# jhuldr/BrainFM

Measured on AMD Instinct MI355X. Metric: voxels/sec whole-volume multi-task inference, 256^3 tiled, higher is better.
Workload: dtype f16x3-split (fp32-grade); 1 GPU; 256^3 volume, reference tiling win160/stride80 -> 27 tiles, UNet3D f64 x6 levels, 9 heads (69 ch), fused tail + deformed atlas + on-device stitch of 17 keys; stitched_keys=17, mfma_passes=3, submission=hipGraph replay per tile shape, parallelism=tiles sharded over 1 rank(s), gather to rank 0, tiles_in_flight_per_gpu=2

## Files before the change

brainfm_amd/_lib.py:

```python
import ctypes as C
import os

_HERE = os.path.dirname(os.path.abspath(__file__))
LIB_PATH = os.path.join(_HERE, "libbrainfm_hip.so")

ERR = {0: "BFM_OK", -1: "BFM_E_ARG", -2: "BFM_E_SHAPE", -3: "BFM_E_WORKSPACE", -4: "BFM_E_LAUNCH"}

ROLE_PLAIN, ROLE_CT, ROLE_BIAS_LOG, ROLE_SEG, ROLE_DIST, ROLE_SR, ROLE_PATHOL = range(7)
(EW_EXP, EW_AFFINE, EW_CLAMP, EW_CLAMP_MIN, EW_GAMMA, EW_SIGMOID, EW_DIV, EW_NONZERO, EW_SUB_DIV, EW_GE,
 EW_NAN_TO_NUM) = range(11)
(EW_ADD, EW_MUL, EW_MUL_EXP, EW_AXPY_CLAMP0, EW_AXPY, EW_DIV2, EW_ZERO_WHERE_ZERO) = range(7)


class BfmError(RuntimeError):
    pass


class Upsample(C.Structure):
    _fields_ = [("d", C.c_int), ("h", C.c_int), ("w", C.c_int),
                ("mapD", C.c_void_p), ("mapH", C.c_void_p), ("mapW", C.c_void_p),
                ("repD", C.c_void_p), ("repH", C.c_void_p), ("repW", C.c_void_p)]


CLASS_STATS_BLOCKS = 1024


class TailDesc(C.Structure):
    _fields_ = [("n_out", C.c_int), ("c_feat", C.c_int),
                ("head_w", C.c_void_p), ("head_b", C.c_void_p), ("roles", C.c_void_p), ("out_slot", C.c_void_p),
                ("seg_first", C.c_int), ("n_seg", C.c_int), ("seg_lut", C.c_void_p),
                ("n_dist", C.c_int), ("dist_first", C.c_int), ("max_dist", C.c_float),
                ("unit_feat", C.c_int), ("slot_high_res", C.c_int), ("slot_fake_cortical", C.c_int),
                ("n_maps", C.c_int), ("head_wmax", C.c_float), ("skip_zero_input", C.c_int)]


class ZoomAxis(C.Structure):
    _fields_ = [("f", C.c_void_p), ("c", C.c_void_p), ("wf", C.c_void_p), ("wc", C.c_void_p)]


class KSet(C.Structure):
    _fields_ = [("k", C.c_void_p * 7), ("coef", C.c_float * 7), ("nk", C.c_int)]


class Dopri5Advect(C.Structure):
    _fields_ = [("y", C.c_void_p * 2), ("f", C.c_void_p * 2), ("k", C.c_void_p * 5),
                ("Vx", C.c_void_p), ("Vy", C.c_void_p), ("Vz", C.c_void_p),
                ("sx", C.c_int), ("sy", C.c_int), ("sz", C.c_int), ("neumann_bc", C.c_int), ("is_f64", C.c_int),
                ("atol", C.c_double), ("rtol", C.c_double), ("tol_min_dt", C.c_double), ("dt_max", C.c_double),
                ("safety", C.c_double), ("ifactor", C.c_double), ("dfactor", C.c_double),
                ("t_out", C.c_void_p), ("nt", C.c_int), ("sol", C.c_void_p), ("state", C.c_void_p),
                ("workspace", C.c_void_p)]


class AgeParams(C.Structure):
    _fields_ = [(n, C.c_void_p) for n in ("c1w", "c1b", "c2w", "c2b", "l1w", "l1b", "l2w", "l2b", "l3w", "l3b")]


class AgeGrads(C.Structure):
    _fields_ = [(n, C.c_void_p) for n in ("c1w", "c1b", "c2w", "c2b", "l1w", "l1b", "l2w", "l2b", "l3w", "l3b")]


GATHER_MAX_JOBS = 12


VERTEX_SETS_MAX = 4


class VertexSet(C.Structure):
    _fields_ = [("V", C.c_void_p), ("n", C.c_int64)]


class GatherJob(C.Structure):
    _fields_ = [("src", C.c_void_p), ("out", C.c_void_p), ("mean", C.c_float), ("scale", C.c_float), ("pre", C.c_int),
                ("default_max", C.c_int), ("post_div", C.c_float), ("clamp", C.c_int), ("clamp_lo", C.c_float),
                ("clamp_hi", C.c_float), ("sign", C.c_float), ("want_minmax", C.c_int)]


_P = C.c_void_p
_I = C.c_int
_F = C.c_float
_L = C.c_int64
_Z = C.c_size_t
_UP = C.POINTER(Upsample)

SIGNATURES = {
    "bfm_version": (C.c_char_p, []),
    "bfm_gn_stats_workspace": (_Z, [_I, _I, _I, _I, _I, _UP]),
    "bfm_gn_stats": (_I, [_P, _I, _P, _I, _I, _I, _I, _UP, _P, _P, _I, _F, _P, _P, _P, _P, _Z, _P]),
    "bfm_pack_conv_weights_direct": (_I, [_P, _I, _I, _P, _P]),
    "bfm_pack_conv_weights_mfma_bytes": (_Z, [_I, _I]),
    "bfm_pack_conv_weights_mfma": (_I, [_P, _I, _I, _F, _P, C.POINTER(_I), _P]),
    "bfm_pack_conv_weights_mfma16_bytes": (_Z, [_I, _I]),
    "bfm_pack_conv_weights_mfma16": (_I, [_P, _I, _I, _F, _P, C.POINTER(_I), _P]),
    "bfm_conv3x3x3_direct": (_I, [_P, _I, _P, _I, _I, _I, _I, _UP, _P, _P, _P, _I, _F, _P, _P]),
    "bfm_pack_conv_weights_upfold_bytes": (C.c_size_t, [_I, _I, _I]),
    "bfm_pack_conv_weights_upfold": (_I, [_P, _I, _I, _I, _F, _I, _P, _P, _P]),
    "bfm_conv3x3x3_upfold": (_I, [_P, _I, _I, _I, _I, _P, _P, _P, _I, _P, _I, _I, _I, _P, _P]),
    "bfm_conv3x3x3_upfold_workspace": (_Z, [_I, _I, _I, _I, _I]),
    "bfm_conv3x3x3_upfold_ex": (_I, [_P, _I, _I, _I, _I, _P, _P, _P, _I, _P, _I, _I, _I, _P, _P, _Z, _P]),
    "bfm_conv3x3x3_upfold_batch_workspace": (_Z, [_I, _I, _I, _I, _I, _I]),
    "bfm_conv3x3x3_upfold_batch": (_I, [_P, _I, _I, _I, _I, _I, _P, _P, _P, _I, _P, _I, _I, _I, _P, _P, _Z, _I, _P]),
    "bfm_conv3x3x3_tap_batch_workspace": (_Z, [_I, _I, _I, _I]),
    "bfm_conv3x3x3_tap_batch": (_I, [_P, _I, _I, _I, _P, _P, _P, _I, _P, _I, _I, _I, _I, _I, _P, _Z, _I, _P]),
    "bfm_tap_sum_rows": (_I, [_I, _I]),
    "bfm_tap_sum_batch": (_I, [_P, _I, _I, _I, _I, _P, _I, _F, _I, _I, _P, _P, _P]),
    "bfm_moment_rows_bytes": (_Z, [_I, _I]),
    "bfm_conv3x3x3_mfma_rows": (_I, [_I, _I, _I, _I, _I, C.POINTER(_I)]),
    "bfm_conv3x3x3_mfma_ex": (_I, [_P, _I, _P, _I, _I, _I, _I, _UP, _P, _P, _P, _I, _P, _I, _I, _F, _I,
                                   C.POINTER(_I), _P, _P, _Z, _P, _P]),
    "bfm_conv3x3x3_mfma_batch_workspace": (_Z, [_I, _I, _I, _I, _I, _I, _I]),
    "bfm_conv3x3x3_mfma_batch": (_I, [_P, _I, _P, _I, _I, _I, _I, _I, _UP, _P, _P, _P, _I, _P, _I, _I, _F, _I,
                                      C.POINTER(_I), _P, _P, _Z, _P, _I, _P]),
    "bfm_gn_stats_batch_workspace": (_Z, [_I, _I, _I, _I, _I, _I, _UP]),
    "bfm_gn_stats_batch": (_I, [_P, _I, _P, _I, _I, _I, _I, _I, _UP, _P, _P, _I, _F, _P, _P, _P, _P, _Z, _P]),
    "bfm_gn_stats_rows_batch": (_I, [_P, _I, _I, _P, _I, _I, C.c_double, _L, _I, _P, _P, _I, _F, _P, _P, _P, _P]),
    "bfm_conv3x3x3_stem_rows": (_I, [_I, _I, _I]),
    "bfm_conv3x3x3_stem_ex": (_I, [_P, _I, _I, _I, _P, _P, _P, _P, _I, _F, _P, _P, _P]),
    "bfm_conv3x3x3_stem_mc_ex": (_I, [_P, _I, _I, _I, _I, _P, _P, _P, _P, _I, _F, _P, _P, _P]),
    "bfm_gn_stats_rows_workspace": (_Z, [_I, _I, _I, _I]),
    "bfm_gn_stats_rows": (_I, [_P, _I, _I, _P, _I, _I, C.c_double, _L, _P, _P, _I, _F, _P, _P, _P, _P, _Z, _P, _P]),
    "bfm_gn_stats_rows_sliced": (_I, [_P, _I, _I, _I, _I, _P, _I, _I, _I, _I, C.c_double, _L, _P, _P, _I, _F, _P, _P, _P, _P, _Z,
                                      _P, _P]),
    "bfm_gn_stats_rows_train": (_I, [_P, _I, _I, _P, _I, _I, C.c_double, _L, _P, _P, _I, _F, _P, _P, _P, _P, _P, _P, _Z, _P, _P]),
    "bfm_crop3d": (_I, [_P, _I, _I, _I, _I, _I, _I, _I, _I, _I, _P, _P]),
    "bfm_pack_conv_weights_wino4_bytes": (_Z, [_I, _I, _I]),
    "bfm_pack_conv_weights_wino4": (_I, [_P, _I, _I, _F, _I, _P, C.POINTER(_I), _P]),
    "bfm_conv3x3x3_wino4_rows": (_I, [_I, _I, _I, _I]),
    "bfm_conv3x3x3_wino4_box": (_I, [_I, _I, _I, _I, _P]),
    "bfm_conv3x3x3_wino4_masked_workspace": (_Z, [_I, _I, _I, _I]),
    "bfm_conv3x3x3_wino4_uniform_scratch": (_Z, [_I]),
    "bfm_conv3x3x3_wino4_uniform": (_I, [_P, _I, _I, _I, _I, _P, _P, _P, _I, _P, _I, _I, _F, _I, _I, _P, _P, _P, _P, _P]),
    "bfm_conv3x3x3_wino4": (_I, [_P, _I, _I, _I, _I, _P, _P, _P, _I, _P, _I, _I, _F, _I, _I, _P, _P, _P]),
    "bfm_conv3x3x3_wino4_batch": (_I, [_P, _I, _I, _I, _I, _I, _P, _P, _P, _I, _P, _I, _I, _F, _I, _I, _P, _P, _I, _P]),
    "bfm_conv3x3x3_wino4_masked": (_I, [_P, _I, _I, _I, _I, _P, _P, _P, _I, _P, _I, _I, _F, _I, _I, _P, _P, _P, _Z, _P]),
    "bfm_permute_flip3d": (_I, [_P, _I, _I, _I, C.POINTER(_I), C.POINTER(_I), _P, _P]),
    "bfm_bbox_nonzero": (_I, [_P, _I, _I, _I, _F, _P, _P]),
    "bfm_mean_lastdim": (_I, [_P, _L, _I, _P, _P]),
    "bfm_pack_conv_weights_wino_bytes": (_Z, [_I, _I, _I]),
    "bfm_pack_conv_weights_wino": (_I, [_P, _I, _I, _F, _I, _P, C.POINTER(_I), _P]),
    "bfm_bspline3_prefilter_axis": (_I, [_P, _I, _I, _I, _I, _I, _F, _F, _P, _F, _F, _F, _P]),
    "bfm_bspline3_resample_axis": (_I, [_P, _I, _I, _I, _I, _P, _I, _I, _P, _P]),
    "bfm_conv3x3x3_wino_rows": (_I, [_I, _I, _I, _I]),
    "bfm_conv3x3x3_wino_ex": (_I, [_P, _I, _I, _I, _I, _P, _P, _P, _I, _P, _I, _I, _F, _I, _I, _P, _P, _P]),
    "bfm_conv3x3x3_wino_box": (_I, [_I, _I, _I, _I, _P]),
    "bfm_uniform_boxes": (_I, [_P, _I, _I, _I, _I, _I, _P, _P]),
    "bfm_uniform_boxes_level": (_I, [_P, _I, _I, _I, _I, _I, _I, _P, _P]),
    "bfm_uniform_boxes_levels": (_I, [_P, _I, _I, _I, _I, C.POINTER(_I), C.POINTER(_I), _I, C.POINTER(_P), _P, _P]),
    "bfm_uniform_boxes_bytes": (_Z, [_I, _I, _I, _I]),
    "bfm_conv3x3x3_wino_uniform_scratch": (_Z, [_I]),
    "bfm_conv3x3x3_wino_uniform": (_I, [_P, _I, _I, _I, _I, _P, _P, _P, _I, _P, _I, _I, _F, _I, _I, _P, _P, _P, _P, _P]),
    "bfm_conv3x3x3_wino_pool_ok": (_I, [_I, _I, _I, _I]),
    "bfm_conv3x3x3_wino_pool": (_I, [_P, _I, _I, _I, _I, _P, _P, _P, _I, _P, _I, _I, _F, _I, _I, _P, _P, _P, _P, _P]),
    "bfm_conv3x3x3_wino_uniform_pool": (_I, [_P, _I, _I, _I, _I, _P, _P, _P, _I, _P, _I, _I, _F, _I, _I, _P, _P, _P, _P, _P, _P,
                                             _P]),
    "bfm_conv3x3x3_wino_masked_workspace": (_Z, [_I, _I, _I, _I]),
    "bfm_conv3x3x3_wino_masked": (_I, [_P, _I, _I, _I, _I, _P, _P, _P, _I, _P, _I, _I, _F, _I, _I, _P, _P, _P, _Z, _P]),
    "bfm_maxpool2_rows": (_I, [_I, _I, _I, _I]),
    "bfm_maxpool2_ex": (_I, [_P, _I, _I, _I, _I, _P, _P, _P]),
    "bfm_maxpool2_batch_rows": (_I, [_I, _I, _I, _I]),
    "bfm_maxpool2_batch": (_I, [_P, _I, _I, _I, _I, _I, _P, _P, _P]),
    "bfm_grid_push3d_linear": (_I, [_P, _I, _I, _I, _I, _I, _P, _I, _I, _I, _I, C.POINTER(_I), _I, _P, _P]),
    "bfm_grid_grad3d_linear": (_I, [_P, _I, _I, _I, _I, _I, _P, _I, _I, _I, _I, C.POINTER(_I), _I, _P, _P]),
    "bfm_gn_stats_train": (_I, [_P, _I, _P, _I, _I, _I, _I, _UP, _P, _P, _I, _F, _P, _P, _P, _P, _P, _P, _Z, _P]),
    "bfm_lrelu_bwd": (_I, [_P, _P, _L, _F, _P, _P]),
    "bfm_lrelu_bwd_ex": (_I, [_P, _P, _L, _F, _P, _P, _P]),
    "bfm_conv3x3x3_wgrad_workspace": (_Z, [_I, _I, _I, _I, _I]),
    "bfm_conv3x3x3_wgrad": (_I, [_P, _I, _P, _I, _P, _I, _I, _I, _I, _UP, _P, _P, _P, _P, _Z, _P]),
    "bfm_conv3x3x3_wgrad_ex": (_I, [_P, _I, _P, _I, _P, _I, _I, _I, _I, _UP, _P, _P, _P, _P, _I, _I, _P, _P, _Z, _P]),
    "bfm_stem_mc_bwd_workspace": (_Z, [_I, _I, _I, _I, _I]),
    "bfm_stem_mc_bwd": (_I, [_P, _I, _P, _I, _I, _I, _I, _P, _P, _P, _P, _P, _P, _P, _P, _P, _Z, _P]),
    "bfm_stem_mc_dgrad": (_I, [_P, _I, _P, _I, _I, _I, _I, _P, _P, _P, _P, _P, _P, _I, _P, _P, _P, _P, _L, _L, _P]),
    "bfm_mask_chain_bwd": (_I, [_P, _L, _P, _P, _L, _P, _L, _L, _P]),
    "bfm_gn_bwd_workspace": (_Z, [_I, _I, _I, _I]),
    "bfm_gn_bwd": (_I, [_P, _P, _I, _P, _I, _I, _I, _I, _UP, _P, _P, _P, _P, _P, _P, _I, _P, _P, _P, _P, _P, _Z, _P]),
    "bfm_maxpool2_bwd": (_I, [_P, _P, _I, _I, _I, _I, _P, _P]),
    "bfm_transpose_mirror_weights": (_I, [_P, _I, _I, _I, _P, _P]),
    "bfm_loss_workspace": (_Z, [_I]),
    "bfm_loss_l1": (_I, [_P, _I, _I, _P, _P, _P, _L, _F, _I, _F, _P, _P, _P, _Z, _P]),
    "bfm_loss_l1_multi_workspace": (_Z, []),
    "bfm_loss_l1_multi": (_I, [_P, _I, _L, _I, _P, _P, _P, _P, _P, _P, _P, _P, _P, _P, _Z, _P]),
    "bfm_loss_grad_l1_multi": (_I, [_P, _I, _I, _P, _P, _P, _P, _I, _I, _I, _P, _P, _P, _Z, _P]),
    "bfm_loss_grad_l1": (_I, [_P, _I, _I, _P, _P, _I, _I, _I, _F, _P, _P, _P, _Z, _P]),
    "bfm_loss_seg": (_I, [_P, _I, _I, _I, _P, _P, _P, _L, _F, _F, _P, _P, _P, _P, _Z, _P]),
    "bfm_loss_pathol_workspace": (_Z, []),
    "bfm_loss_pathol": (_I, [_P, _L, _L, _P, _L, _F, _F, _P, _P, _P, _P, _Z, _P]),
    "bfm_loss_reg_workspace": (_Z, [_I, _I, _I, _I]),
    "bfm_loss_reg_smooth": (_I, [_P, _L, _L, _L, _I, _I, _I, _I, _F, _P, _P, _P, _Z, _P]),
    "bfm_loss_reg_hessian": (_I, [_P, _L, _L, _L, _I, _I, _I, _I, _F, _P, _P, _P, _Z, _P]),
    "bfm_loss_contrastive_workspace": (_Z, []),
    "bfm_loss_contrastive": (_I, [_P, _P, _I, _L, _I, _F, _F, _F, _F, _F, _P, _P, _P, _P, _P, _P, _Z, _P]),
    "bfm_head_bwd_workspace": (_Z, [_I, _I, _L]),
    "bfm_head_bwd": (_I, [_P, _P, _P, _I, _I, _L, _P, _P, _P, _P, _Z, _P]),
    "bfm_tail_raw_rows": (_I, [_P, _L, C.POINTER(TailDesc), _P, _P, _L, _P]),
    "bfm_loss_l1_multi_rows": (_I, [_P, _L, _I, _L, _I, _P, _P, _P, _P, _P, _P, _P, _P, _P, _P, _Z, _P]),
    "bfm_loss_grad_l1_multi_rows": (_I, [_P, _L, _I, _I, _P, _P, _P, _P, _I, _I, _I, _P, _P, _P, _Z, _P]),
    "bfm_loss_seg_rows": (_I, [_P, _L, _I, _I, _I, _P, _P, _P, _L, _F, _F, _P, _P, _P, _P, _Z, _P]),
    "bfm_head_bwd_rows": (_I, [_P, _L, _P, _P, _I, _I, _L, _P, _P, _P, _P, _Z, _P]),
    "bfm_normalize_bwd": (_I, [_P, _P, _I, _L, _F, _P, _P]),
    "bfm_adamw_step": (_I, [_P, _P, _P, _P, _L, _F, _F, _F, _F, _F, _I, _F, _P]),
    "bfm_grad_sumsq": (_I, [_P, _L, _P, _P, _P, _Z, _P]),
    "bfm_grad_sumsq_multi": (_I, [_P, _I, _P, _I, _L, _P, _P, _P, _Z, _P]),
    "bfm_adamw_step_multi": (_I, [_P, _I, _P, _I, _L, _F, _F, _F, _F, _F, _P]),
    "bfm_conv3x3x3_mfma_workspace": (_Z, [_I, _I, _I, _I, _I, _I]),
    "bfm_conv3x3x3_mfma_plan": (_I, [_I, _I, _I, _I, _I, C.POINTER(_I)]),
    "bfm_conv3x3x3_mfma": (_I, [_P, _I, _P, _I, _I, _I, _I, _UP, _P, _P, _P, _I, _P, _I, _I, _F, _I,
                                C.POINTER(_I), _P, _P, _Z, _P]),
    "bfm_maxpool2": (_I, [_P, _I, _I, _I, _I, _P, _P]),
    "bfm_tail_heads": (_I, [_P, _P, _L, C.POINTER(TailDesc), _P, _P, _P, _P, _P, _P]),
    "bfm_tail_heads_rows": (_I, [_P, _P, _L, C.POINTER(TailDesc), _P, _P, _L, _P, _P, _I, _P]),
    "bfm_ew_unary": (_I, [_I, _P, _L, _P, _L, _L, _F, _F, _P]),
    "bfm_ew_binary": (_I, [_I, _P, _L, _P, _L, _P, _L, _L, _F, _P]),
    "bfm_absmax_f32": (_I, [_P, _L, _L, _L, _P, _P]),
    "bfm_softmax_cl": (_I, [_P, _L, _I, _P, _L, _L, _P]),
    "bfm_argmax_lut_cl": (_I, [_P, _L, _I, _P, _P, _L, _P]),
    "bfm_fake_cortical": (_I, [_P, _L, _I, _P, _L, _P]),
    "bfm_mask_concat2": (_I, [_P, _P, _L, _P, _P]),
    "bfm_condition_input": (_I, [_P, _P, _I, _I, _I, _I, _P, _P, _P, _P]),
    "bfm_twostage_train_input": (_I, [_P, _P, _L, _L, _P, _L, _P, _P, _P, _P]),
    "bfm_interp3d_linear": (_I, [_P, _I, _I, _I, _I, _P, _P, _P, _L, _F, _P, _P]),
    "bfm_interp3d_nearest": (_I, [_P, _I, _I, _I, _I, _P, _P, _P, _L, _P, _P]),
    "bfm_deformed_atlas": (_I, [_P, _P, _P, _P, _P, _I, _I, _I, C.POINTER(_F), _L, _P, _P]),
    "bfm_deformed_atlas_tile": (_I, [_P, _P, _P, _P, _P, _I, _I, _I, C.POINTER(_F), _L, _P, _P]),
    "bfm_zoom_linear": (_I, [_P, _I, _I, _I, _I, C.POINTER(ZoomAxis), _I, _I, _I, _P, _P]),
    "bfm_conv1d_axis": (_I, [_P, _I, _I, _I, _I, _P, _I, _P, _P]),
    "bfm_grid_pull3d_linear": (_I, [_P, _I, _I, _I, _I, _I, _P, _I, _I, _I, _I, C.POINTER(_I), _I, _P, _P]),
    "bfm_deform_grid_workspace": (_Z, [_I, _I, _I]),
    "bfm_deform_grid": (_I, [_P, _I, _I, _I, C.POINTER(_F), C.POINTER(_F), C.POINTER(_I), _P, _P, _P, _P, _P, _Z, _P]),
    "bfm_label_gauss": (_I, [_P, _P, _P, _P, _L, _I, _P, _P]),
    "bfm_label_class_stats": (_I, [_P, _P, _L, _P, _P, _P, _P]),
    "bfm_onehot_lut": (_I, [_P, _P, _I, _I, _L, _P, _P]),
    "bfm_perlin3d": (_I, [_P, _I, _I, _I, _I, _I, _I, _P, _P]),
    "bfm_radix_hist_f64": (_I, [_P, _L, C.c_uint64, _I, _P, _P]),
    "bfm_threshold_mask_f64": (_I, [_P, _L, C.c_double, _P, _P, _P]),
    "bfm_curl3d": (_I, [_P, _P, _P, _I, _I, _I, _F, _P, _P, _P, _P]),
    "bfm_advect_upwind_rhs": (_I, [_P, _I, _P, _P, _P, _I, _I, _I, _I, _P, _P]),
    "bfm_rk_combine": (_I, [_P, _I, C.POINTER(KSet), _P, _L, _P]),
    "bfm_reduce_workspace": (_Z, []),
    "bfm_rk_error_sumsq": (_I, [C.POINTER(KSet), _P, _P, _I, C.c_double, C.c_double, _L, _P, _P, _Z, _P]),
    "bfm_scaled_sumsq": (_I, [_P, _P, _I, _P, _I, C.c_double, C.c_double, _L, _P, _P, _Z, _P]),
    "bfm_dopri5_dense_eval": (_I, [_P, _P, _I, C.POINTER(KSet), C.c_double, C.c_double, _P, _L, _P]),
    "bfm_reduce_f32": (_I, [_I, _P, _P, _L, _P, _P, _Z, _P]),
    "bfm_reduce_f64": (_I, [_I, _P, _P, _L, _P, _P, _Z, _P]),
    "bfm_dopri5_advect_state_bytes": (_Z, []),
    "bfm_dopri5_advect_workspace": (_Z, [_I, _I, _I]),
    "bfm_dopri5_advect_init": (_I, [C.POINTER(Dopri5Advect), C.c_double, C.c_double, _P]),
    "bfm_dopri5_advect_steps": (_I, [C.POINTER(Dopri5Advect), _I, _P]),
    "bfm_randn_philox": (_I, [_P, _L, C.c_uint64, C.c_uint64, _F, _P]),
    "bfm_svf_integrate_workspace": (_Z, [_I, _I, _I]),
    "bfm_svf_integrate": (_I, [_P, _I, _I, _I, _I, _P, _P, _P, _Z, _P]),
    "bfm_deform_vertices": (_I, [_P, _I, _I, _I, C.POINTER(VertexSet), _I, C.POINTER(_F), C.POINTER(_F), _I, _I, _P]),
    "bfm_deform_zoom_workspace": (_Z, []),
    "bfm_deform_zoom_minmax": (_I, [_P, _I, _I, _I, C.POINTER(ZoomAxis), _I, _I, _I, _I, C.POINTER(_F), C.POINTER(_F),
                                    C.POINTER(_I), _P, _P, _Z, _P]),
    "bfm_deform_zoom_write": (_I, [_P, _I, _I, _I, C.POINTER(ZoomAxis), _I, _I, _I, _I, C.POINTER(_F), C.POINTER(_F),
                                   C.POINTER(_I), C.POINTER(_F), _P, _P, _P, _P, _P]),
    "bfm_gather_targets_workspace": (_Z, []),
    "bfm_gather_targets": (_I, [C.POINTER(GatherJob), _I, _I, _I, _I, C.POINTER(_I), _P, _P, _P, _I, _I, _I, _I, _P, _P,
                                _Z, _P]),
    "bfm_minmax_normalise": (_I, [_P, _L, _P, _P]),
    "bfm_gather_onehot": (_I, [_P, _I, _I, _I, C.POINTER(_I), _P, _P, _P, _I, _I, _I, _I, _P, _I, _I, _P, _P, _P]),
    "bfm_gather_onehot_rows": (_I, [_P, _I, _I, _I, C.POINTER(_I), _P, _P, _P, _I, _I, _I, _I, _P, _I, _I, _P, _P, _P]),
    "bfm_percentile_workspace": (_Z, []),
    "bfm_percentile_f64": (_I, [_P, _L, _L, _I, C.c_double, _P, _P, _Z, _P]),
    "bfm_shape_workspace": (_Z, []),
    "bfm_shape_threshold_f64": (_I, [_P, _L, _P, _P, _P, _P, _P, _Z, _P]),
    "bfm_shape_binarize": (_I, [_P, _I, _L, _P, C.c_double, _P, _P, _P, _Z, _P]),
    "bfm_pathology_mask": (_I, [_P, _P, _I, _P, _L, _P, _P, _Z, _P]),
    "bfm_pathology_encode_workspace": (_Z, []),
    "bfm_pathology_encode_dev": (_I, [_P, _P, _P, _I, _P, C.POINTER(_F), _I, _P, _L, _P, _P, _P, _Z, _P]),
    "bfm_interp3d_linear_axes": (_I, [_P, _I, _I, _I, _P, _P, _P, _I, _I, _I, _F, _P, _P]),
    "bfm_sample_finalize": (_I, [_P, _P, _I, _I, _I, _P, _I, _P, _P, _P]),
    "bfm_stitch_accumulate": (_I, [_P, _P, _P, _I, _I, _I, _P, _I, _I, _I, _I, _I, _I, _P]),
    "bfm_stitch_accumulate_multi": (_I, [_P, _L, _P, _I, _P, _P, _I, _I, _I, _P, _I, _I, _I, _I, _I, _I, _P]),
    "bfm_tile_count_add": (_I, [_P, _I, _I, _I, _I, _I, _I, _I, _I, _I, _P]),
    "bfm_pack_tile_multi": (_I, [_P, _L, _P, _I, _P, _P, _L, _P, _P]),
    "bfm_divide_by_count_multi": (_I, [_P, _P, _L, _I, _P]),
    "bfm_stitch_gather_multi": (_I, [_P, _I, _I, _P, _I, _I, _I, _P]),
    "bfm_tile_mask_blocks": (_I, [_L]),
    "bfm_tile_mask_index": (_I, [_P, _I, _I, _I, _P, _I, _I, _P, _P, _P, _P]),
    "bfm_pack_tile_compact": (_I, [_P, _L, _P, _I, _P, _P, _L, _P, _L, _P, _P]),
    "bfm_stitch_gather_compact": (_I, [_P, _I, _I, _P, _P, _I, _I, _I, _P]),
    "bfm_maxpool4": (_I, [_P, _I, _I, _I, _I, _P, _P, _P]),
    "bfm_maxpool4_bwd": (_I, [_P, _P, _I, _I, _I, _I, _P, _I, _P]),
    "bfm_age_conv_fwd": (_I, [_P, _I, _I, _I, _I, _P, _P, _I, _P, _P]),
# ... 92 lines not shown
```

brainfm_amd/csrc/conv3d_upfold.hip:

```cpp
#include "conv_shared.h"
#include <type_traits>

namespace {

typedef _Float16 half8 __attribute__((ext_vector_type(8)));
typedef _Float16 half4 __attribute__((ext_vector_type(4)));
typedef float floatx16 __attribute__((ext_vector_type(16)));

constexpr int KC = 16;
constexpr int NTHR = 512;

struct UpParams {
    const float* B;
    int CB, d, h, w;
    const float *scale, *shift;
    int saff;
    const float* bound;
    int G;
    const uint4* wp;
    int wexp, Cout;
    float* out;
    int BD, BH, BW, HT, WT;
    int BHW, BVOX;
    int nTy, nTx, nMt, NT, KCB;
    int nvox_lds, plane_stride;
    int rowoff_lds;
    int kc_per_split;
    float* slab;
    int64_t slab_stride;
    int64_t sB, sO;
    int dbg_sleep;
};

__device__ __forceinline__ void box_coords(const UpParams& p, int q, int& bd, int& bh, int& bw) {
    bd = q / p.BHW;
    const int rem = q - bd * p.BHW;
    bh = rem / p.BW;
    bw = rem - bh * p.BW;
}

template <int NPASS, int ABL = 0, int NW = 8>
__device__ __forceinline__ void conv_upfold_body(const UpParams& p) {
    constexpr int NTHRV = NW * 64;
    constexpr int NPL = (NPASS == 3) ? 2 : 1;
    constexpr int NF = 2 * NPL;
    extern __shared__ __attribute__((aligned(16))) unsigned char lds[];
    const int tid = threadIdx.x;
    const int lane = tid & 63;
    int xcd_ = blockIdx.x & 7, idx_ = blockIdx.x >> 3, half_ = 0;
    if constexpr (NW == 4) {
        half_ = idx_ & 1;
        idx_ >>= 1;
        const int nblk = p.nMt * p.NT;
        if (idx_ >= (nblk >> 3) + (xcd_ < (nblk & 7) ? 1 : 0)) return;
    }
    const int cls = __builtin_amdgcn_readfirstlane(tid >> 6) + half_ * 4;
    const int pz = cls >> 2, py = (cls >> 1) & 1, px = cls & 1;
    const int l32 = lane & 31, khalf = lane >> 5;
#ifdef BFM_UP_ABLATE
    if (p.dbg_sleep > 0 && blockIdx.x < 256 && ((blockIdx.x >> 3) & 1))
        for (int i = 0; i < p.dbg_sleep; ++i) __builtin_amdgcn_s_sleep(16);
#endif

    int bid;
    {
        const int nblk = p.nMt * p.NT;
        const int q = nblk >> 3, r = nblk & 7;
        const int xcd = xcd_, idx = idx_;
        bid = (xcd < r ? xcd * (q + 1) : r * (q + 1) + (xcd - r) * q) + idx;
    }
    const int mt = bid / p.NT, nt = bid - mt * p.NT;
    const int tx = mt % p.nTx;
    const int ty = (mt / p.nTx) % p.nTy;
    const int tz = mt / (p.nTx * p.nTy);
    const int z0 = tz * p.BD, y0 = ty * p.BH, x0 = tx * p.BW;
    const int smp = blockIdx.z;
    const float* const pB = p.B + smp * p.sB;
    const float* const pscale = p.scale + smp * p.saff;
    const float* const pshift = p.shift + smp * p.saff;
    const float* const pbound = p.bound + smp * p.G;

    float bmax = 0.f;
    for (int g = 0; g < p.G; ++g) bmax = fmaxf(bmax, pbound[g]);
    int aexp = 0;
    if (bmax > 0.f && bmax < INFINITY) {
        int ex;
        (void)frexpf(bmax, &ex);
        aexp = 14 - ex;
        aexp = aexp > 60 ? 60 : (aexp < -60 ? -60 : aexp);
    }
    const float a_scale = ldexpf(1.0f, aexp);
    const float dq = ldexpf(1.0f, -(aexp + p.wexp));

    int a_off[4];
#pragma unroll
    for (int mb = 0; mb < 4; ++mb) {
        int bd, bh, bw;
        const int q = mb * 32 + row_perm(l32);
        box_coords(p, q < p.BVOX ? q : 0, bd, bh, bw);
        a_off[mb] = (khalf * NPL) * p.plane_stride + (((bd + pz) * p.HT + (bh + py)) * p.WT + (bw + px)) * 16;
    }

    int* const rowoff = reinterpret_cast<int*>(lds + p.rowoff_lds);
    if (tid < 128) {
        int bd, bh, bw;
        box_coords(p, tid < p.BVOX ? tid : 0, bd, bh, bw);
        const bool ok = tid < p.BVOX && z0 + bd < p.d && y0 + bh < p.h && x0 + bw < p.w;
        rowoff[tid] = ok ? (((2 * bd) * (2 * p.h) + 2 * bh) * (2 * p.w) + 2 * bw) * p.Cout : -1;
    }

    constexpr int MAX_IT = 2048 / NTHRV;
    const int n_el = p.nvox_lds * 4;
    const int q4 = tid & 3;
    int off[MAX_IT];
#pragma unroll
    for (int it = 0; it < MAX_IT; ++it) {
        const int e = tid + it * NTHRV;
        off[it] = -2;
        if (e < n_el) {
            const int vox = e >> 2;
            const int hz = vox / (p.HT * p.WT);
            const int rem = vox - hz * (p.HT * p.WT);
            const int hy = rem / p.WT;
            const int hx = rem - hy * p.WT;
            const int gz = z0 + hz - 1, gy = y0 + hy - 1, gx = x0 + hx - 1;
            off[it] = -1;
            if (gz >= 0 && gz < p.d && gy >= 0 && gy < p.h && gx >= 0 && gx < p.w)
                off[it] = ((gz * p.h + gy) * p.w + gx) * p.CB;
        }
    }
    const int st_plane = ((q4 >> 1) * NPL) * p.plane_stride + (q4 & 1) * 8;

    floatx16 acc[4][2];
#pragma unroll
    for (int mb = 0; mb < 4; ++mb)
#pragma unroll
        for (int nb = 0; nb < 2; ++nb)
#pragma unroll
            for (int i = 0; i < 16; ++i) acc[mb][nb][i] = 0.f;

    const int S = p.KCB * 8;
    const uint4* wbase = p.wp + (size_t)(nt * 8 + cls) * S * (NF * 64) + lane;
    uint4 wq[3][NF];
    const int kc0_ = blockIdx.y * p.kc_per_split * 8;
    half8 a_abl[4][NPL];
    if constexpr ((ABL & 2) != 0) {
#pragma unroll
        for (int u = 0; u < 4; ++u)
#pragma unroll
            for (int hl = 0; hl < NPL; ++hl)
#pragma unroll
                for (int j = 0; j < 8; ++j) a_abl[u][hl][j] = (_Float16)(0.01f * (float)((lane * 7 + u * 3 + hl * 5 + j) % 61) - 0.3f);
    }
    auto fetch = [&](int s, uint4 (&dst)[NF]) __attribute__((always_inline)) {
        if constexpr ((ABL & 1) != 0) { if (s > kc0_ + 1) return; }
        const int sc = s < S ? s : S - 1;
#pragma unroll
        for (int f = 0; f < NF; ++f) dst[f] = wbase[(size_t)sc * (NF * 64) + f * 64];
    };
    const int kc0 = blockIdx.y * p.kc_per_split;
    const int kc1 = min(p.KCB, kc0 + p.kc_per_split);
    fetch(kc0 * 8, wq[0]);
    fetch(kc0 * 8 + 1, wq[1]);

    auto do_chunk = [&](int kc, auto ph_tag) __attribute__((always_inline)) {
        constexpr int PH = decltype(ph_tag)::value;
        const int c0 = kc * KC;
        const float* src = pB + c0 + q4 * 4;
        const float4 sc4 = *reinterpret_cast<const float4*>(pscale + c0 + q4 * 4);
        const float4 sh4 = *reinterpret_cast<const float4*>(pshift + c0 + q4 * 4);
        const float sc[4] = {sc4.x * a_scale, sc4.y * a_scale, sc4.z * a_scale, sc4.w * a_scale};
        const float sh[4] = {sh4.x * a_scale, sh4.y * a_scale, sh4.z * a_scale, sh4.w * a_scale};
        __syncthreads();
#pragma unroll
        for (int u0 = 0; u0 < MAX_IT; u0 += 2) {
            if constexpr ((ABL & 4) != 0) continue;
            float4 v[2];
#pragma unroll
            for (int u = 0; u < 2; ++u) {
                v[u] = make_float4(0.f, 0.f, 0.f, 0.f);
                if constexpr ((ABL & 8) != 0) v[u] = make_float4(0.1f * lane, 0.2f, 0.3f * kc, 0.4f);
                else
                if (off[u0 + u] >= 0) v[u] = *reinterpret_cast<const float4*>(src + off[u0 + u]);
            }
#pragma unroll
            for (int u = 0; u < 2; ++u) {
                const int e = tid + (u0 + u) * NTHRV;
                if (off[u0 + u] != -2) {
                    const bool ok = off[u0 + u] >= 0;
                    float y[4] = {v[u].x, v[u].y, v[u].z, v[u].w};
                    half4 hi, lo;
#pragma unroll
                    for (int i = 0; i < 4; ++i) {
                        float t = ok ? fmaf(y[i], sc[i], sh[i]) : 0.f;
                        _Float16 hh = (_Float16)t;
                        hi[i] = hh;
                        lo[i] = (_Float16)(t - (float)hh);
                    }
                    unsigned char* dst = lds + st_plane + (e >> 2) * 16;
                    *reinterpret_cast<half4*>(dst) = hi;
                    if constexpr (NPASS == 3) *reinterpret_cast<half4*>(dst + p.plane_stride) = lo;
                }
            }
        }
        __syncthreads();

#pragma unroll
        for (int t = 0; t < 8; ++t) {
            const int s = kc * 8 + t;
            const int ta = t >> 2, tb = (t >> 1) & 1, tc = t & 1;
            const int toff = ((ta * p.HT + tb) * p.WT + tc) * 16;
            const int cur = (PH + t) % 3;
            uint4 bw[NF];
#pragma unroll
            for (int f = 0; f < NF; ++f) bw[f] = wq[cur][f];
            fetch(s + 2, wq[(cur + 2) % 3]);
            __builtin_amdgcn_sched_barrier(0);
#pragma unroll
            for (int mb = 0; mb < 4; ++mb) {
                half8 a[NPL];
#pragma unroll
                for (int hl = 0; hl < NPL; ++hl) {
                    if constexpr ((ABL & 2) != 0) a[hl] = a_abl[mb][hl];
                    else a[hl] = *reinterpret_cast<const half8*>(lds + a_off[mb] + hl * p.plane_stride + toff);
                }
                if constexpr ((ABL & 64) != 0) {
                    float ss = 0.f;
#pragma unroll
                    for (int hl = 0; hl < NPL; ++hl) ss += (float)a[hl][0] + (float)a[hl][7];
                    ss += __builtin_bit_cast(float, bw[0].x) + __builtin_bit_cast(float, bw[NF - 1].w);
                    acc[mb][0][0] += ss;
                    continue;
                }
#pragma unroll
                for (int nb = 0; nb < 2; ++nb) {
                    const half8 bhi = __builtin_bit_cast(half8, bw[nb * NPL]);
                    if constexpr (NPASS == 3) {
                        const half8 blo = __builtin_bit_cast(half8, bw[nb * NPL + 1]);
                        acc[mb][nb] = __builtin_amdgcn_mfma_f32_32x32x16_f16(bhi, a[1], acc[mb][nb], 0, 0, 0);
                        acc[mb][nb] = __builtin_amdgcn_mfma_f32_32x32x16_f16(blo, a[0], acc[mb][nb], 0, 0, 0);
                    }
                    acc[mb][nb] = __builtin_amdgcn_mfma_f32_32x32x16_f16(bhi, a[0], acc[mb][nb], 0, 0, 0);
                }
            }
        }
    };
    for (int kc = kc0; kc < kc1; kc += 3) {
        do_chunk(kc, std::integral_constant<int, 0>{});
        if (kc + 1 < kc1) do_chunk(kc + 1, std::integral_constant<int, 2>{});
        if (kc + 2 < kc1) do_chunk(kc + 2, std::integral_constant<int, 1>{});
    }

    if constexpr ((ABL & 16) != 0) {
        float sm = 0.f;
#pragma unroll
        for (int mb = 0; mb < 4; ++mb)
#pragma unroll
            for (int i = 0; i < 16; ++i) sm += acc[mb][0][i] + acc[mb][1][i];
        if (sm == 12345.678f) p.out[tid] = sm;
        return;
    }
    const int H2 = 2 * p.h, W2 = 2 * p.w;
    float* const obase = p.slab ? p.slab + ((int64_t)smp * gridDim.y + blockIdx.y) * p.slab_stride : p.out + smp * p.sO;
    float* const ob = obase + (((int64_t)(2 * z0 + pz) * H2 + (2 * y0 + py)) * W2 + (2 * x0 + px)) * p.Cout + nt * 64 + khalf * 4;
#pragma unroll
    for (int mb = 0; mb < 4; ++mb) {
        const int rel = rowoff[mb * 32 + row_perm(l32)];
        if (rel < 0) continue;
        float* const o = ob + (unsigned)rel;
#pragma unroll
        for (int nb = 0; nb < 2; ++nb)
#pragma unroll
            for (int g = 0; g < 4; ++g)
                *reinterpret_cast<float4*>(o + nb * 32 + g * 8) =
                    make_float4(acc[mb][nb][4 * g] * dq, acc[mb][nb][4 * g + 1] * dq, acc[mb][nb][4 * g + 2] * dq,
                                acc[mb][nb][4 * g + 3] * dq);
    }
}

template <int NPASS>
__global__ void __launch_bounds__(NTHR, 1) conv_upfold(const UpParams p) { conv_upfold_body<NPASS, 0>(p); }
template <int NPASS>
__global__ void __launch_bounds__(NTHR / 2, 2) conv_upfold_h(const UpParams p) { conv_upfold_body<NPASS, 0, 4>(p); }
#ifdef BFM_UP_ABLATE
template <int ABL>
__global__ void __launch_bounds__(NTHR, 1) conv_upfold_abl(const UpParams p) { conv_upfold_body<3, ABL>(p); }
#endif

__global__ void upfold_reduce(const float4* __restrict__ slab, int nsplit, int64_t n4, float4* __restrict__ out) {
    slab += (int64_t)blockIdx.y * nsplit * n4;
    out += (int64_t)blockIdx.y * n4;
    for (int64_t i = (int64_t)blockIdx.x * blockDim.x + threadIdx.x; i < n4; i += (int64_t)gridDim.x * blockDim.x) {
        float4 a = slab[i];
        for (int k = 1; k < nsplit; ++k) {
            const float4 b = slab[i + (int64_t)k * n4];
            a.x += b.x; a.y += b.y; a.z += b.z; a.w += b.w;
        }
        out[i] = a;
    }
}

__global__ void pack_upfold(const float* __restrict__ w, int Cin, int CA, int CB, int Cout, int wexp, int npl,
                            uint4* __restrict__ out) {
    const int KCB = CB / KC;
    const int nf = 2 * npl;
    const int64_t n = (int64_t)(Cout / 64) * 8 * KCB * 8 * nf * 64;
    const float s = ldexpf(1.0f, wexp);
    for (int64_t i = (int64_t)blockIdx.x * blockDim.x + threadIdx.x; i < n; i += (int64_t)gridDim.x * blockDim.x) {
        const int lane = (int)(i & 63);
        int64_t r = i >> 6;
        const int f = (int)(r % nf); r /= nf;
        const int t = (int)(r & 7); r >>= 3;
        const int kc = (int)(r % KCB); r /= KCB;
        const int cls = (int)(r & 7); r >>= 3;
        const int ntile = (int)r;
        const int nb = f / npl, hl = f - nb * npl;
        const int co = ntile * 64 + nb * 32 + (lane & 31);
        const int ci0 = CA + kc * KC + 8 * (lane >> 5);
        const int pz = cls >> 2, py = (cls >> 1) & 1, px = cls & 1;
        const int ta = t >> 2, tb = (t >> 1) & 1, tc = t & 1;
        const int zlo = pz == 0 ? (ta == 0 ? 0 : 1) : (ta == 0 ? 0 : 2), zhi = pz == 0 ? (ta == 0 ? 0 : 2) : (ta == 0 ? 1 : 2);
        const int ylo = py == 0 ? (tb == 0 ? 0 : 1) : (tb == 0 ? 0 : 2), yhi = py == 0 ? (tb == 0 ? 0 : 2) : (tb == 0 ? 1 : 2);
        const int xlo = px == 0 ? (tc == 0 ? 0 : 1) : (tc == 0 ? 0 : 2), xhi = px == 0 ? (tc == 0 ? 0 : 2) : (tc == 0 ? 1 : 2);
        half8 v;
#pragma unroll
        for (int j = 0; j < 8; ++j) {
            const float* wc = w + ((size_t)co * Cin + ci0 + j) * 27;
            float sum = 0.f;
            for (int kd = zlo; kd <= zhi; ++kd)
                for (int kh = ylo; kh <= yhi; ++kh)
                    for (int kw = xlo; kw <= xhi; ++kw) sum += wc[kd * 9 + kh * 3 + kw];
            const float x = sum * s;
            const _Float16 hh = (_Float16)x;
            v[j] = hl == 0 ? hh : (_Float16)(x - (float)hh);
        }
        out[i] = __builtin_bit_cast(uint4, v);
    }
}

constexpr int PKU_ROW = KC * 27 + 1;
__global__ void __launch_bounds__(256) pack_upfold_tiled(const float* __restrict__ w, int Cin, int CA, int CB, int Cout,
                                                         int wexp, int npl, uint4* __restrict__ out) {
    extern __shared__ float pku_lds[];
    const int KCB = CB / KC;
    const int nf = 2 * npl;
    const int kc = blockIdx.x % KCB, ntile = blockIdx.x / KCB;
    const float s = ldexpf(1.0f, wexp);
    const float* src0 = w + ((int64_t)(ntile * 64) * Cin + CA + kc * KC) * 27;
    bfm_stage_rows<64, KC * 27, PKU_ROW, 256>(src0, (int64_t)Cin * 27, pku_lds, 1.0f,
                                              ((reinterpret_cast<uintptr_t>(w) & 15) == 0) && (Cin & 3) == 0 && (CA & 3) == 0);
    __syncthreads();
    const int lane = threadIdx.x & 63, wave = threadIdx.x >> 6;
    for (int q = wave; q < 8 * 8 * 2; q += 4) {
        const int nb = q & 1;
        const int t = (q >> 1) & 7;
        const int cls = q >> 4;
        const int pz = cls >> 2, py = (cls >> 1) & 1, px = cls & 1;
        const int ta = t >> 2, tb = (t >> 1) & 1, tc = t & 1;
        const int zlo = pz == 0 ? (ta == 0 ? 0 : 1) : (ta == 0 ? 0 : 2), zhi = pz == 0 ? (ta == 0 ? 0 : 2) : (ta == 0 ? 1 : 2);
        const int ylo = py == 0 ? (tb == 0 ? 0 : 1) : (tb == 0 ? 0 : 2), yhi = py == 0 ? (tb == 0 ? 0 : 2) : (tb == 0 ? 1 : 2);
        const int xlo = px == 0 ? (tc == 0 ? 0 : 1) : (tc == 0 ? 0 : 2), xhi = px == 0 ? (tc == 0 ? 0 : 2) : (tc == 0 ? 1 : 2);
        const float* src = pku_lds + (nb * 32 + (lane & 31)) * PKU_ROW + (8 * (lane >> 5)) * 27;
        half8 vh, vl;
#pragma unroll
        for (int j = 0; j < 8; ++j) {
            const float* wc = src + j * 27;
            float sum = 0.f;
            for (int kd = zlo; kd <= zhi; ++kd)
                for (int kh = ylo; kh <= yhi; ++kh)
                    for (int kw = xlo; kw <= xhi; ++kw) sum += wc[kd * 9 + kh * 3 + kw];
            const float x = sum * s;
            const _Float16 hh = (_Float16)x;
            vh[j] = hh;
            vl[j] = (_Float16)(x - (float)hh);
        }
        uint4* dst = out + ((((int64_t)(ntile * 8 + cls) * KCB + kc) * 8 + t) * nf + nb * npl) * 64 + lane;
        dst[0] = __builtin_bit_cast(uint4, vh);
        if (npl == 2) dst[64] = __builtin_bit_cast(uint4, vl);
    }
}

void choose_box(int d, int h, int w, int& BD, int& BH, int& BW) {
    static const int opts[][3] = {{2, 4, 16}, {4, 2, 16}, {4, 4, 8}, {2, 8, 8}, {8, 2, 8}, {8, 4, 4}, {4, 8, 4},
                                  {1, 8, 16}, {8, 1, 16}, {2, 2, 32}, {1, 4, 32}, {4, 1, 32},
                                  {5, 5, 5}, {2, 5, 10}, {5, 2, 10}};
    int64_t best = -1;
    for (auto& o : opts) {
        if ((o[0] + 2) * (o[1] + 2) * (o[2] + 2) * 4 > 4 * NTHR) continue;
        int64_t cost = (int64_t)bfm_cdiv(d, o[0]) * bfm_cdiv(h, o[1]) * bfm_cdiv(w, o[2]);
        cost = cost * 64 - (o[2] > 32 ? 32 : o[2]);
        if (best < 0 || cost < best) { best = cost; BD = o[0]; BH = o[1]; BW = o[2]; }
    }
}

}

extern "C" size_t bfm_pack_conv_weights_upfold_bytes(int CB, int Cout, int passes) {
    if (CB <= 0 || Cout <= 0 || CB % KC || Cout % 64) return 0;
    const int npl = passes == 3 ? 2 : 1;
    return (size_t)(Cout / 64) * 8 * (CB / KC) * 8 * 2 * npl * 64 * sizeof(uint4);
}

extern "C" int bfm_pack_conv_weights_upfold(const float* w_oidhw, int CA, int CB, int Cout, float wmax_abs_host,
                                            int passes, void* wpacked, int* wexp_host, bfm_stream_t stream) {
    if (!w_oidhw || !wpacked || !wexp_host || CA < 0 || CB <= 0 || Cout <= 0) return BFM_E_ARG;
    if (CB % KC || Cout % 64 || (passes != 1 && passes != 3)) return BFM_E_SHAPE;
    int wexp = 0;
    if (wmax_abs_host > 0.f && wmax_abs_host < INFINITY) {
        int ex;
        (void)frexpf(8.f * wmax_abs_host, &ex);
        wexp = 14 - ex;
        wexp = wexp > 60 ? 60 : (wexp < -60 ? -60 : wexp);
    }
    *wexp_host = wexp;
    const int npl = passes == 3 ? 2 : 1;
    const int64_t nblk = (int64_t)(Cout / 64) * (CB / KC);
    const size_t smem = (size_t)64 * PKU_ROW * sizeof(float);
    static bool attr = false;
    if (const int rc = bfm_raise_lds_limit(attr, {bfm_kernel(&pack_upfold_tiled)}, (int)smem)) return rc;
    if (nblk <= 0x7fffffff) {
        hipLaunchKernelGGL(pack_upfold_tiled, dim3((unsigned)nblk), dim3(256), smem, bfm_s(stream), w_oidhw, CA + CB, CA, CB,
                           Cout, wexp, npl, static_cast<uint4*>(wpacked));
    } else {
        const int64_t n = nblk * 8 * 8 * 2 * npl * 64;
        int nb = (int)std::min<int64_t>(4096, bfm_cdiv64(n, 256));
        hipLaunchKernelGGL(pack_upfold, dim3(nb), dim3(256), 0, bfm_s(stream), w_oidhw, CA + CB, CA, CB, Cout, wexp, npl,
                           static_cast<uint4*>(wpacked));
    }
    return bfm_launch_status();
}

namespace {
void upfold_split(int CB, int d, int h, int w, int Cout, int& nsplit, int& per) {
    int BD, BH, BW;
    choose_box(d, h, w, BD, BH, BW);
    const int64_t wgs = (int64_t)bfm_cdiv(d, BD) * bfm_cdiv(h, BH) * bfm_cdiv(w, BW) * (Cout / 64);
    const int KCB = CB / KC;
    nsplit = 1;
    per = KCB;
    if (wgs >= 192 || KCB < 6) return;
    int want = (int)std::min<int64_t>(KCB / 3, bfm_cdiv64(384, wgs));
    if (want < 2) return;
    per = bfm_cdiv(bfm_cdiv(KCB, want), 3) * 3;
    nsplit = bfm_cdiv(KCB, per);
    if (nsplit < 2) { nsplit = 1; per = KCB; }
}
}

extern "C" size_t bfm_conv3x3x3_upfold_workspace(int CB, int d, int h, int w, int Cout) {
    if (CB <= 0 || d <= 0 || h <= 0 || w <= 0 || Cout <= 0 || CB % KC || Cout % 64) return 0;
    int nsplit, per;
    upfold_split(CB, d, h, w, Cout, nsplit, per);
    return nsplit > 1 ? (size_t)nsplit * 8 * d * h * w * Cout * sizeof(float) : 0;
}

static int upfold_launch(const float* B, int CB, int S, int d, int h, int w, const float* scale_b, const float* shift_b,
                         const float* bound, int G, const void* wpacked, int wexp, int Cout, int passes, float* out,
                         void* workspace, size_t workspace_bytes, bool strict, int affine_stride, bfm_stream_t stream);

extern "C" int bfm_conv3x3x3_upfold_ex(const float* B, int CB, int d, int h, int w, const float* scale_b,
                                       const float* shift_b, const float* bound, int G, const void* wpacked, int wexp,
                                       int Cout, int passes, float* out, void* workspace, size_t workspace_bytes,
                                       bfm_stream_t stream) {
    return upfold_launch(B, CB, 1, d, h, w, scale_b, shift_b, bound, G, wpacked, wexp, Cout, passes, out, workspace,
                         workspace_bytes, false, 0, stream);
}

extern "C" size_t bfm_conv3x3x3_upfold_batch_workspace(int CB, int S, int d, int h, int w, int Cout) {
    return S > 0 ? (size_t)S * bfm_conv3x3x3_upfold_workspace(CB, d, h, w, Cout) : 0;
}

extern "C" int bfm_conv3x3x3_upfold_batch(const float* B, int CB, int S, int d, int h, int w, const float* scale_b,
                                          const float* shift_b, const float* bound, int G, const void* wpacked, int wexp,
                                          int Cout, int passes, float* out, void* workspace, size_t workspace_bytes,
                                          int affine_stride, bfm_stream_t stream) {
    if (S <= 0 || S > 65535) return BFM_E_ARG;
    if (affine_stride != 0 && (affine_stride < CB || (affine_stride & 3))) return BFM_E_ARG;
    return upfold_launch(B, CB, S, d, h, w, scale_b, shift_b, bound, G, wpacked, wexp, Cout, passes, out, workspace,
                         workspace_bytes, true, affine_stride, stream);
}

static int upfold_launch(const float* B, int CB, int S, int d, int h, int w, const float* scale_b, const float* shift_b,
                         const float* bound, int G, const void* wpacked, int wexp, int Cout, int passes, float* out,
                         void* workspace, size_t workspace_bytes, bool strict, int affine_stride, bfm_stream_t stream) {
    if (!B || CB <= 0 || d <= 0 || h <= 0 || w <= 0 || !scale_b || !shift_b || !bound || G <= 0 || !wpacked || !out)
        return BFM_E_ARG;
    if (CB % KC || Cout % 64 || Cout <= 0) return BFM_E_SHAPE;
    if (passes != 1 && passes != 3) return BFM_E_ARG;
    if ((reinterpret_cast<uintptr_t>(B) & 15) || (reinterpret_cast<uintptr_t>(scale_b) & 15) ||
        (reinterpret_cast<uintptr_t>(shift_b) & 15) || (reinterpret_cast<uintptr_t>(wpacked) & 15) ||
        (reinterpret_cast<uintptr_t>(out) & 15))
        return BFM_E_ARG;
    if ((int64_t)d * h * w * CB > 0x7fffffffLL) return BFM_E_SHAPE;
    UpParams p{};
    p.B = B; p.CB = CB; p.d = d; p.h = h; p.w = w;
    p.scale = scale_b; p.shift = shift_b; p.bound = bound; p.G = G;
    p.saff = affine_stride > 0 ? affine_stride : CB;
    p.wp = static_cast<const uint4*>(wpacked);
    p.wexp = wexp; p.Cout = Cout; p.out = out;
    choose_box(d, h, w, p.BD, p.BH, p.BW);
    p.HT = p.BH + 2; p.WT = p.BW + 2;
    p.BHW = p.BH * p.BW; p.BVOX = p.BD * p.BHW;
    const int nTz = bfm_cdiv(d, p.BD);
    p.nTy = bfm_cdiv(h, p.BH); p.nTx = bfm_cdiv(w, p.BW);
    p.nMt = nTz * p.nTy * p.nTx;
    p.NT = Cout / 64;
    p.KCB = CB / KC;
    p.nvox_lds = (p.BD + 2) * p.HT * p.WT;
    if (p.nvox_lds * 4 > 4 * NTHR) return BFM_E_SHAPE;
    p.plane_stride = ((p.nvox_lds * 16 + 255) / 256) * 256 + 16;
    const int npl = passes == 3 ? 2 : 1;
    p.rowoff_lds = ((2 * npl * p.plane_stride + 64 + 15) / 16) * 16;
    const size_t smem = (size_t)p.rowoff_lds + 128 * sizeof(int);
    if ((int64_t)(2 * p.BD) * (2 * h) * (2 * w) * Cout > 0x7fffffffLL) return BFM_E_SHAPE;
    if ((int64_t)p.nMt * p.NT > 0x7fffffff) return BFM_E_SHAPE;
    int nsplit = 1, per = p.KCB;
    const int64_t nout = (int64_t)8 * d * h * w * Cout;
    p.sB = (int64_t)d * h * w * CB;
    p.sO = nout;
    if (workspace || strict) {
        upfold_split(CB, d, h, w, Cout, nsplit, per);
        if (nsplit > 1 && (!workspace || workspace_bytes < (size_t)S * nsplit * nout * sizeof(float) ||
                           (reinterpret_cast<uintptr_t>(workspace) & 15))) {
            if (strict) return BFM_E_ARG;
            nsplit = 1;
            per = p.KCB;
        }
    }
    p.kc_per_split = per;
    p.slab = nsplit > 1 ? static_cast<float*>(workspace) : nullptr;
    p.slab_stride = nout;
    dim3 grid((unsigned)(p.nMt * p.NT), (unsigned)nsplit, (unsigned)S);
#ifdef BFM_UP_ABLATE
    if (const char* e = getenv("BFM_UP_SLEEP")) p.dbg_sleep = atoi(e);
    if (const char* e = getenv("BFM_UP_ABL")) {
        const int a = atoi(e);
        hipStream_t st = bfm_s(stream);
#define UPA(n) case n: hipLaunchKernelGGL(conv_upfold_abl<n>, grid, dim3(NTHR), smem, st, p); break;
        switch (a) {
            UPA(0) UPA(1) UPA(2) UPA(4) UPA(8) UPA(16) UPA(64) UPA(3) UPA(5) UPA(7) UPA(23) UPA(68) UPA(71) UPA(87) UPA(80) UPA(20) UPA(12)
            default: return BFM_E_ARG;
        }
#undef UPA
        return bfm_launch_status();
    }
#endif
    static const int waves_env = [] { const char* e = getenv("BFM_UPFOLD_WAVES"); return e ? atoi(e) : 0; }();
    const int waves = waves_env ? waves_env : ((nsplit > 1 || (int64_t)p.nMt * p.NT * S <= 128) ? 4 : 8);
    if (waves == 4) {
        const int64_t nblk = (int64_t)p.nMt * p.NT;
        const int64_t gx = 16 * bfm_cdiv64(nblk, 8);
        if (gx > 0x7fffffff) return BFM_E_SHAPE;
        dim3 gridh((unsigned)gx, (unsigned)nsplit, (unsigned)S);
        bfm_launch_by_passes(passes, conv_upfold_h<3>, conv_upfold_h<1>, gridh, dim3(NTHR / 2), smem, bfm_s(stream), p);
    } else bfm_launch_by_passes(passes, conv_upfold<3>, conv_upfold<1>, grid, dim3(NTHR), smem, bfm_s(stream), p);
    if (nsplit > 1) {
        const int64_t n4 = nout / 4;
        const int nb = (int)std::min<int64_t>(4096, bfm_cdiv64(n4, 256));
        hipLaunchKernelGGL(upfold_reduce, dim3(nb, S), dim3(256), 0, bfm_s(stream), reinterpret_cast<const float4*>(p.slab), nsplit,
                           n4, reinterpret_cast<float4*>(out));
    }
    return bfm_launch_status();
}

extern "C" int bfm_conv3x3x3_upfold(const float* B, int CB, int d, int h, int w, const float* scale_b,
                                    const float* shift_b, const float* bound, int G, const void* wpacked, int wexp,
                                    int Cout, int passes, float* out, bfm_stream_t stream) {
    return bfm_conv3x3x3_upfold_ex(B, CB, d, h, w, scale_b, shift_b, bound, G, wpacked, wexp, Cout, passes, out, nullptr, 0,
                                   stream);
}
```

brainfm_amd/csrc/conv3d_wino4.hip:

```cpp
#include "wino_shared.h"
#include <cstdlib>
#include <type_traits>

namespace {

typedef _Float16 half8 __attribute__((ext_vector_type(8)));
typedef float floatx16 __attribute__((ext_vector_type(16)));
typedef __fp16 fp16x2_t __attribute__((ext_vector_type(2)));

constexpr int KC = 16;
constexpr int NPOS = 6;
constexpr int NTHR = 256;
constexpr int NRG = NTHR / 32;
constexpr int MLD = 33;

struct W4Params {
    const float* A;
    int CA, D, H, W;
    const float *scale, *shift, *bound;
    int G;
    const uint4* wp;
    int wexp, Cout;
    float slope;
    float* out;
// ... 260 lines not shown
#pragma unroll
                for (int i = 0; i < 16; ++i) sm += acc[u][nb][i];
        if (sm == 12345.678f) p.out[tid] = sm;
        return;
    }
    float* m = reinterpret_cast<float*>(lds);
    const int col = tid & 31, rg = tid >> 5;
    const bool interior = z0 + p.TD <= p.D && y0 + p.TH <= p.H && x0 + p.TW <= p.W;
    unsigned off_t = 0;
    int un[4] = {0, 0, 0, 0};
    if (interior) {
        int d_t, h_t, j_t;
        quad_coords(p, rg, d_t, h_t, j_t);
        off_t = (unsigned)(((d_t * p.H + h_t) * p.W + 4 * j_t) * p.Cout + col);
#pragma unroll
        for (int s2 = 0; s2 < 4; ++s2) un[s2] = row_unperm(rg + 8 * s2);
    }
#pragma unroll
    for (int nb = 0; nb < 2; ++nb) {
        __syncthreads();
#pragma unroll
        for (int u = 0; u < 3; ++u) {
            const int pos = u < 2 ? posA : posB, mb = u < 2 ? u : mbB;
            float* mw = m + (pos * 64 + mb * 32 + khalf * 4) * MLD + l32;
#pragma unroll
            for (int i = 0; i < 16; ++i)
                mw[((i >> 2) * 8 + (i & 3)) * MLD] = acc[u][nb][i];
        }
        __syncthreads();
        float fs = 0.f, fq = 0.f, fmn = INFINITY, fmx = -INFINITY;
        if (interior) {
            float* ob = p.out + nt * 64 + nb * 32;
            float prev[8][4];
            if (p.accum) {
#pragma unroll
                for (int it = 0; it < 8; ++it) {
                    int d_u, h_u, j_u;
                    quad_coords(p, 8 * it, d_u, h_u, j_u);
                    const float* o = ob + (((int64_t)(z0 + d_u) * p.H + (y0 + h_u)) * p.W + x0 + 4 * j_u) * p.Cout;
#pragma unroll
                    for (int k = 0; k < 4; ++k) prev[it][k] = o[off_t + (unsigned)(k * p.Cout)];
                }
            }
            const float* mc = m + col;
#pragma unroll
            for (int it = 0; it < 8; ++it) {
                int d_u, h_u, j_u;
                quad_coords(p, 8 * it, d_u, h_u, j_u);
                float* o = ob + (((int64_t)(z0 + d_u) * p.H + (y0 + h_u)) * p.W + x0 + 4 * j_u) * p.Cout;
                const int qr = 32 * (it >> 2) + un[it & 3];
                const float* mr = mc + qr * MLD;
                const float m0 = mr[0 * 64 * MLD], m1 = mr[1 * 64 * MLD], m2 = mr[2 * 64 * MLD];
                const float m3 = mr[3 * 64 * MLD], m4 = mr[4 * 64 * MLD], m5 = mr[5 * 64 * MLD];
                const float s1 = m1 + m2, d1 = m1 - m2, s2 = m3 + m4, d2 = m3 - m4;
                float y[4];
                y[0] = ((m0 + s1) + s2) * dq;
                y[1] = fmaf(2.f, d2, d1) * dq;
                y[2] = fmaf(4.f, s2, s1) * dq;
                y[3] = (fmaf(8.f, d2, d1) + m5) * dq;
#pragma unroll
                for (int k = 0; k < 4; ++k) {
                    float r = y[k];
                    if (p.accum) r = r + prev[it][k];
                    r = r >= 0.f ? r : r * p.slope;
                    o[off_t + (unsigned)(k * p.Cout)] = r;
                    fs += r; fq = fmaf(r, r, fq); fmn = fminf(fmn, r); fmx = fmaxf(fmx, r);
                }
            }
        } else
#pragma unroll 2
        for (int q = rg; q < 64; q += NRG) {
            int d, h, j;
            quad_coords(p, q, d, h, j);
            const int gz = z0 + d, gy = y0 + h, gx = x0 + 4 * j;
            if (gz >= p.D || gy >= p.H || gx >= p.W) continue;
            const int qr = (q & ~31) + row_unperm(q & 31);
            const float* mr = m + qr * MLD + col;
            const float m0 = mr[0 * 64 * MLD], m1 = mr[1 * 64 * MLD], m2 = mr[2 * 64 * MLD];
            const float m3 = mr[3 * 64 * MLD], m4 = mr[4 * 64 * MLD], m5 = mr[5 * 64 * MLD];
            const float s1 = m1 + m2, d1 = m1 - m2, s2 = m3 + m4, d2 = m3 - m4;
            float y[4];
            y[0] = ((m0 + s1) + s2) * dq;
            y[1] = fmaf(2.f, d2, d1) * dq;
            y[2] = fmaf(4.f, s2, s1) * dq;
            y[3] = (fmaf(8.f, d2, d1) + m5) * dq;
            float* o = p.out + (((int64_t)gz * p.H + gy) * p.W + gx) * p.Cout + nt * 64 + nb * 32 + col;
#pragma unroll
            for (int k = 0; k < 4; ++k) {
                if (gx + k < p.W) {
                    float r = y[k];
                    if (p.accum) r = r + o[(size_t)k * p.Cout];
                    r = r >= 0.f ? r : r * p.slope;
                    o[(size_t)k * p.Cout] = r;
                    fs += r; fq = fmaf(r, r, fq); fmn = fminf(fmn, r); fmx = fmaxf(fmx, r);
                }
            }
        }
        if (p.rsum != nullptr) {
            double* ls = reinterpret_cast<double*>(lds + (size_t)NPOS * 64 * MLD * sizeof(float));
            double* lq = ls + NRG * 32;
            float* lmn = reinterpret_cast<float*>(lq + NRG * 32);
            float* lmx = lmn + NRG * 32;
            ls[rg * 32 + col] = (double)fs; lq[rg * 32 + col] = (double)fq;
            lmn[rg * 32 + col] = fmn; lmx[rg * 32 + col] = fmx;
            __syncthreads();
            if (tid < 32) {
                double Ssum = 0.0, Q = 0.0;
                float MN = INFINITY, MX = -INFINITY;
#pragma unroll
                for (int r = 0; r < NRG; ++r) {
                    Ssum += ls[r * 32 + tid]; Q += lq[r * 32 + tid];
                    MN = fminf(MN, lmn[r * 32 + tid]); MX = fmaxf(MX, lmx[r * 32 + tid]);
                }
                const size_t o = (size_t)mt * p.Cout + nt * 64 + nb * 32 + tid;
                p.rsum[o] = Ssum; p.rsq[o] = Q; p.rmn[o] = MN; p.rmx[o] = MX;
            }
        }
    }
}

template <int NPASS>
__global__ void __launch_bounds__(NTHR, 2) conv_wino4(const W4Params p) { conv_wino4_body<NPASS, 0>(p); }
template <int NPASS>
__global__ void __launch_bounds__(NTHR, 2) conv_wino4_masked(const W4Params p) { conv_wino4_body<NPASS, 1>(p); }

constexpr int DB_TD = 8, DB_TH = 8, DB_HT = 10, DB_NROW = 100;
constexpr int DB_PLANE = DB_NROW * 16;
constexpr int DB_RAWROW = 6 * 64;
constexpr int DB_RAW = DB_NROW * DB_RAWROW;
constexpr int DB_NDMA = DB_NROW / 2;
constexpr int DB_NDMA_WAVE = (DB_NDMA + 3) / 4;

template <bool LO>
__device__ __forceinline__ void split_store4_mix(const float (&t)[4], unsigned char* dp, int plane_stride) {
    const fp16x2_t h01 = __builtin_amdgcn_cvt_pkrtz(t[0], t[1]);
    const fp16x2_t h23 = __builtin_amdgcn_cvt_pkrtz(t[2], t[3]);
    uint2 hv;
    hv.x = __builtin_bit_cast(unsigned, h01);
    hv.y = __builtin_bit_cast(unsigned, h23);
    *reinterpret_cast<uint2*>(dp) = hv;
    if constexpr (LO) {
        uint2 lv;
        asm("v_fma_mixlo_f16 %0, %1, -1.0, %2 op_sel_hi:[1,0,0]" : "=v"(lv.x) : "v"(hv.x), "v"(t[0]));
        asm("v_fma_mixhi_f16 %0, %1, -1.0, %2 op_sel:[1,0,0] op_sel_hi:[1,0,0]" : "+v"(lv.x) : "v"(hv.x), "v"(t[1]));
        asm("v_fma_mixlo_f16 %0, %1, -1.0, %2 op_sel_hi:[1,0,0]" : "=v"(lv.y) : "v"(hv.y), "v"(t[2]));
        asm("v_fma_mixhi_f16 %0, %1, -1.0, %2 op_sel:[1,0,0] op_sel_hi:[1,0,0]" : "+v"(lv.y) : "v"(hv.y), "v"(t[3]));
        *reinterpret_cast<uint2*>(dp + plane_stride) = lv;
    }
}

template <int NPASS, int MODE, int ABL = 0>
__device__ __forceinline__ void conv_wino4d_body(const W4Params& pin) {
    W4Params p = pin;
    constexpr bool LIST = MODE != 0;
    constexpr bool UNI = MODE == 3;
    constexpr bool BY_FLAG = MODE == 2 || MODE == 3;
    constexpr int NPL = (NPASS == 3) ? 2 : 1;
    constexpr int NF = 2 * NPL;
    constexpr int NWF = 3 * NPL;
    constexpr int RAW_OFF = 2 * NPOS * NPL * DB_PLANE;
    extern __shared__ __attribute__((aligned(16))) unsigned char lds[];

    const int tid = threadIdx.x;
    const int lane = tid & 63;
    const int wv = __builtin_amdgcn_readfirstlane(tid >> 6);
    const int posA = wv;
    const int posB = 4 + (wv >> 1), nbB = wv & 1;
    const int l32 = lane & 31, khalf = lane >> 5;
#ifdef BFM_W4_ABLATE
    if (p.dbg_sleep > 0 && blockIdx.x < 512) {
        unsigned hwid;
        asm volatile("s_getreg_b32 %0, hwreg(HW_REG_HW_ID)" : "=s"(hwid));
        if (hwid & 1)
            for (int i = 0; i < p.dbg_sleep; ++i) __builtin_amdgcn_s_sleep(16);
    }
#endif
    int item;
    {
        const int nblk = LIST ? p.list_n[0] * p.NT : p.nMt * p.NT;
        const int bid = blockIdx.x;
        if (LIST && bid >= nblk) return;
        const int q = nblk >> 3, r = nblk & 7;
        const int xcd = bid & 7, idx = bid >> 3;
        item = (xcd < r ? xcd * (q + 1) : r * (q + 1) + (xcd - r) * q) + idx;
    }
    const int mt = LIST ? p.list[item / p.NT] : item / p.NT;
    const int nt = item % p.NT;
    int mtl = mt;
    if (!LIST && p.nMtS > 0) {
        const int smp = mt / p.nMtS;
        mtl = mt - smp * p.nMtS;
        p.A += smp * p.sA;
        p.out += smp * p.sO;
        p.scale += smp * p.saff;
        p.shift += smp * p.saff;
        p.bound += smp * p.G;
    }
    const int tx = mtl % p.nTx;
    const int ty = (mtl / p.nTx) % p.nTy;
    const int tz = mtl / (p.nTx * p.nTy);
    const int z0 = tz * DB_TD, y0 = ty * DB_TH, x0 = tx * 4;
    int cls = 0;
    if constexpr (BY_FLAG) cls = __builtin_amdgcn_readfirstlane((int)p.uni_flags[mt]);
    const bool rep = MODE == 2 && cls != 0;
    float4* const ybuf = BY_FLAG && cls ? reinterpret_cast<float4*>(p.uni_acc) + ((size_t)(cls - 1) * p.NT + nt) * (2 * 8 * NTHR) + tid
                                        : nullptr;

    float bmax = 0.f;
    for (int g = 0; g < p.G; ++g) bmax = fmaxf(bmax, p.bound[g]);
    int aexp = 0;
    if (bmax > 0.f && bmax < INFINITY) {
        int ex;
        (void)frexpf(bmax, &ex);
        aexp = 10 - ex;
        aexp = aexp > 60 ? 60 : (aexp < -60 ? -60 : aexp);
    }
    const float a_scale = ldexpf(1.0f, aexp);
    const float dq = ldexpf(1.0f, -(aexp + p.wexp));

    floatx16 acc[2][2];
    floatx16 accB[2];
    if constexpr (!UNI) {
    int a_off[4];
#pragma unroll
    for (int u = 0; u < 4; ++u) {
        const int pos = u < 2 ? posA : posB, mb = u & 1;
        const int pr = row_perm(l32);
        const int d = mb * 2 + (pr >> 4) + 4 * ((pr & 15) >> 3), h = pr & 7;
        a_off[u] = ((pos * 2 + khalf) * NPL) * DB_PLANE + (d * DB_HT + h) * 16;
    }

    const int q4 = tid & 3;
    int msk[2];
#pragma unroll
    for (int it = 0; it < 2; ++it) {
        const int r = (tid >> 2) + 64 * it;
        msk[it] = -1;
        if (r < DB_NROW) {
            const int hz = r / DB_HT, hy = r - hz * DB_HT;
            const int gz = z0 + hz - 1, gy = y0 + hy - 1;
            int m = 0;
            if (gz >= 0 && gz < p.D && gy >= 0 && gy < p.H) {
#pragma unroll
                for (int i = 0; i < 6; ++i)
                    if (x0 - 1 + i >= 0 && x0 - 1 + i < p.W) m |= 1 << i;
            }
            msk[it] = m;
        }
    }
    const bool inner = z0 >= 1 && z0 + DB_TD < p.D && y0 >= 1 && y0 + DB_TH < p.H && x0 >= 1 && x0 + 4 < p.W;
    const int st_plane = ((q4 >> 1) * NPL) * DB_PLANE + (q4 & 1) * 8;

    const int slot = lane >> 2;
    const int sb = slot >= 6 ? 1 : 0;
    int gxc = x0 + (slot - 6 * sb) - 1;
    gxc = gxc < 0 ? 0 : (gxc > p.W - 1 ? p.W - 1 : gxc);
    const int lane_el = gxc * p.CA + (lane & 3) * 4;
    const bool dma_lane = slot < 12;
    const unsigned raw_lds = (unsigned)(__UINTPTR_TYPE__)((__attribute__((address_space(3))) unsigned char*)(lds + RAW_OFF));
    const int zs = z0 > 0 ? z0 - 1 : 0;
    const float* slab = p.A + (int64_t)zs * p.H * p.W * p.CA;
    auto issue_dma = [&](int kc) __attribute__((always_inline)) {
        if constexpr ((ABL & 8) != 0) return;
        if (dma_lane) {
            int wvo = wv;
            asm volatile("" : "+s"(wvo));
#pragma unroll
            for (int n = 0; n < DB_NDMA_WAVE; ++n) {
                const int i = wvo + 4 * n;
                if (n < DB_NDMA_WAVE - 1 || i < DB_NDMA) {
                    const int hz = i / 5, hp = i - 5 * hz;
                    int gz = z0 + hz - 1;
                    gz = gz < 0 ? 0 : (gz > p.D - 1 ? p.D - 1 : gz);
                    int gy0 = y0 + 2 * hp - 1, gy1 = gy0 + 1;
                    gy0 = gy0 < 0 ? 0 : (gy0 > p.H - 1 ? p.H - 1 : gy0);
                    gy1 = gy1 > p.H - 1 ? p.H - 1 : gy1;
                    const unsigned ro0 = (unsigned)((((gz - zs) * p.H + gy0) * p.W) * p.CA);
                    const unsigned ro1 = (unsigned)((((gz - zs) * p.H + gy1) * p.W) * p.CA);
                    const unsigned vo = ((sb ? ro1 : ro0) + (unsigned)lane_el) * 4u;
                    const unsigned la = raw_lds + (unsigned)(i * (2 * DB_RAWROW));
                    asm volatile("s_mov_b32 m0, %2\n\ts_nop 0\n\tglobal_load_lds_dwordx4 %0, %1" ::"v"(vo), "s"(slab + kc * KC), "s"(la)
                                 : "memory");
                }
            }
        }
    };

#pragma unroll
    for (int u = 0; u < 2; ++u) {
#pragma unroll
        for (int i = 0; i < 16; ++i) { acc[u][0][i] = 0.f; acc[u][1][i] = 0.f; accB[u][i] = 0.f; }
    }

    const int S = p.KCN * 9;
    const uint4* wbA = p.wp + (size_t)(nt * NPOS + posA) * S * (NF * 64) + lane;
    const uint4* wbB = p.wp + (size_t)(nt * NPOS + posB) * S * (NF * 64) + nbB * (NPL * 64) + lane;
    uint4 wq[3][NWF];
    auto fetch = [&](int s, uint4 (&dst)[NWF]) __attribute__((always_inline)) {
        if constexpr ((ABL & 1) != 0) { if (s > 2) return; }
        const int sc = s < S ? s : S - 1;
#pragma unroll
        for (int f = 0; f < NF; ++f) dst[f] = wbA[(size_t)sc * (NF * 64) + f * 64];
#pragma unroll
        for (int f = 0; f < NPL; ++f) dst[NF + f] = wbB[(size_t)sc * (NF * 64) + f * 64];
    };
    issue_dma(0);
    fetch(0, wq[0]);
    fetch(1, wq[1]);
    half8 a_abl[4][NPL];
    if constexpr ((ABL & 2) != 0) {
#pragma unroll
        for (int u = 0; u < 4; ++u)
#pragma unroll
            for (int hl = 0; hl < NPL; ++hl)
#pragma unroll
                for (int j = 0; j < 8; ++j) a_abl[u][hl][j] = (_Float16)(0.01f * (float)((lane * 7 + u * 3 + hl * 5 + j) % 61) - 0.3f);
    }

    for (int kc = 0; kc < p.KCN; ++kc) {
        const int c0 = kc * KC;
        const float4 sc4 = *reinterpret_cast<const float4*>(p.scale + c0 + q4 * 4);
        const float4 sh4 = *reinterpret_cast<const float4*>(p.shift + c0 + q4 * 4);
        const float sc[4] = {sc4.x * a_scale, sc4.y * a_scale, sc4.z * a_scale, sc4.w * a_scale};
        const float sh[4] = {sh4.x * a_scale, sh4.y * a_scale, sh4.z * a_scale, sh4.w * a_scale};
        __builtin_amdgcn_s_waitcnt(0x0F70);
        __syncthreads();
#pragma unroll
        for (int it = 0; it < 2; ++it) {
            if (msk[it] < 0) continue;
            if constexpr ((ABL & 4) != 0) continue;
            const int r = (tid >> 2) + 64 * it;
            const float4* rp = reinterpret_cast<const float4*>(
                __builtin_assume_aligned(lds + RAW_OFF + r * DB_RAWROW + q4 * 16, 16));
            float4 v[6];
#pragma unroll
            for (int i = 0; i < 6; ++i) v[i] = rp[i * 4];
            float dd[6][4];
            if (inner) {
#pragma unroll
                for (int i = 0; i < 6; ++i) {
                    const float y[4] = {v[i].x, v[i].y, v[i].z, v[i].w};
#pragma unroll
                    for (int c = 0; c < 4; ++c) dd[i][c] = fmaf(y[c], sc[c], sh[c]);
                }
            } else {
#pragma unroll
                for (int i = 0; i < 6; ++i) {
                    const bool ok = msk[it] & (1 << i);
                    const float y[4] = {v[i].x, v[i].y, v[i].z, v[i].w};
#pragma unroll
                    for (int c = 0; c < 4; ++c) {
                        const float a = fmaf(y[c], sc[c], sh[c]);
                        dd[i][c] = ok ? a : 0.f;
                    }
                }
            }
            unsigned char* dst = lds + st_plane + r * 16;
            float t[6][4];
#pragma unroll
            for (int c = 0; c < 4; ++c) {
                const float d0 = dd[0][c], d1 = dd[1][c], d2 = dd[2][c], d3 = dd[3][c], d4 = dd[4][c], d5 = dd[5][c];
                const float a = fmaf(-4.f, d2, d4);
                const float b = fmaf(-4.f, d1, d3);
                const float cc = d4 - d2;
                const float ee = 2.f * (d3 - d1);
                t[0][c] = fmaf(4.f, d0, fmaf(-5.f, d2, d4));
                t[1][c] = a + b;
                t[2][c] = a - b;
                t[3][c] = cc + ee;
                t[4][c] = cc - ee;
                t[5][c] = fmaf(4.f, d1, fmaf(-5.f, d3, d5));
            }
#pragma unroll
            for (int ps = 0; ps < NPOS; ++ps)
                split_store4_mix<NPASS == 3>(t[ps], dst + (ps * 2 * NPL) * DB_PLANE, DB_PLANE);
        }
        __syncthreads();
        fetch(kc * 9 + 2, wq[2]);
        if (kc + 1 < p.KCN) issue_dma(kc + 1);

#pragma unroll
        for (int t = 0; t < 9; ++t) {
            const int s = kc * 9 + t;
            const int kd = t / 3, kh = t - kd * 3;
            const int toff = (kd * DB_HT + kh) * 16;
            constexpr int dummy = 0; (void)dummy;
            const int cur = t % 3;
            if (t >= 1) fetch(s + 2, wq[(t + 2) % 3]);
            __builtin_amdgcn_sched_barrier(0);
#pragma unroll
            for (int u = 0; u < 4; ++u) {
                half8 a[NPL];
#pragma unroll
                for (int hl = 0; hl < NPL; ++hl) {
                    if constexpr ((ABL & 2) != 0) a[hl] = a_abl[u][hl];
                    else a[hl] = *reinterpret_cast<const half8*>(lds + a_off[u] + hl * DB_PLANE + toff);
                }
                if constexpr ((ABL & 64) != 0) {
                    float ss = 0.f;
#pragma unroll
                    for (int hl = 0; hl < NPL; ++hl) ss += (float)a[hl][0] + (float)a[hl][7];
                    ss += __builtin_bit_cast(float, wq[cur][0].x) + __builtin_bit_cast(float, wq[cur][NWF - 1].w);
                    if (u < 2) acc[u][0][0] += ss; else accB[u - 2][0] += ss;
                    continue;
                }
                if (u < 2) {
#pragma unroll
                    for (int nb = 0; nb < 2; ++nb) {
                        const half8 bhi = __builtin_bit_cast(half8, wq[cur][nb * NPL]);
                        if constexpr (NPASS == 3) {
                            const half8 blo = __builtin_bit_cast(half8, wq[cur][nb * NPL + 1]);
                            acc[u][nb] = __builtin_amdgcn_mfma_f32_32x32x16_f16(a[1], bhi, acc[u][nb], 0, 0, 0);
                            acc[u][nb] = __builtin_amdgcn_mfma_f32_32x32x16_f16(a[0], blo, acc[u][nb], 0, 0, 0);
                        }
                        acc[u][nb] = __builtin_amdgcn_mfma_f32_32x32x16_f16(a[0], bhi, acc[u][nb], 0, 0, 0);
                    }
                } else {
                    const half8 bhi = __builtin_bit_cast(half8, wq[cur][NF]);
                    if constexpr (NPASS == 3) {
                        const half8 blo = __builtin_bit_cast(half8, wq[cur][NF + 1]);
                        accB[u - 2] = __builtin_amdgcn_mfma_f32_32x32x16_f16(a[1], bhi, accB[u - 2], 0, 0, 0);
                        accB[u - 2] = __builtin_amdgcn_mfma_f32_32x32x16_f16(a[0], blo, accB[u - 2], 0, 0, 0);
                    }
                    accB[u - 2] = __builtin_amdgcn_mfma_f32_32x32x16_f16(a[0], bhi, accB[u - 2], 0, 0, 0);
                }
            }
        }
    }

    }

    if constexpr ((ABL & 16) != 0) {
        float sm = 0.f;
#pragma unroll
        for (int u = 0; u < 2; ++u)
#pragma unroll
            for (int i = 0; i < 16; ++i) sm += acc[u][0][i] + acc[u][1][i] + accB[u][i];
        if (sm == 12345.678f) p.out[tid] = sm;
        return;
    }
    float* m = reinterpret_cast<float*>(lds);
    const int col = tid & 31, rg = tid >> 5;
    const bool interior = z0 + DB_TD <= p.D && y0 + DB_TH <= p.H && x0 + 4 <= p.W;
    int un[4];
#pragma unroll
    for (int c = 0; c < 4; ++c) un[c] = row_unperm(16 * (c >> 1) + 8 * (c & 1) + rg);
    const unsigned off_t = (unsigned)((rg * p.W) * p.Cout + col);
#pragma unroll
    for (int nb = 0; nb < 2; ++nb) {
        if constexpr (!UNI && (ABL & 256) == 0) {
        __syncthreads();
#pragma unroll
        for (int u = 0; u < 2; ++u) {
            float* mw = m + (posA * 64 + u * 32 + khalf * 4) * MLD + l32;
#pragma unroll
            for (int i = 0; i < 16; ++i)
                mw[((i >> 2) * 8 + (i & 3)) * MLD] = acc[u][nb][i];
        }
        if (nbB == nb) {
#pragma unroll
            for (int u = 0; u < 2; ++u) {
                float* mw = m + (posB * 64 + u * 32 + khalf * 4) * MLD + l32;
#pragma unroll
                for (int i = 0; i < 16; ++i)
                    mw[((i >> 2) * 8 + (i & 3)) * MLD] = accB[u][i];
            }
        }
        __syncthreads();
        } else if (nb == 1 && p.rsum != nullptr) __syncthreads();
        float fs = 0.f, fq = 0.f, fmn = INFINITY, fmx = -INFINITY;
        float* ob = p.out + nt * 64 + nb * 32 + ((int64_t)(z0 * p.H + y0) * p.W + x0) * p.Cout;
        if constexpr ((ABL & 512) != 0) ob = p.out + nt * 64 + nb * 32 + (mt & 127) * 16384;
        const float* mc = m + col;
        if (interior) {
            float prev[8][4];
            if (p.accum) {
#pragma unroll
                for (int it = 0; it < 8; ++it) {
                    const float* o = ob + (int64_t)it * p.H * p.W * p.Cout;
#pragma unroll
                    for (int k = 0; k < 4; ++k) prev[it][k] = o[off_t + (unsigned)(k * p.Cout)];
                }
            }
#pragma unroll
            for (int it = 0; it < 8; ++it) {
                float* o = ob + (int64_t)it * p.H * p.W * p.Cout;
                if constexpr ((ABL & 512) != 0) o = ob + it * 2048 - (int)off_t + (rg * 256 + col);
                float y[4];
                if constexpr (UNI) {
                    const float4 yy = ybuf[(nb * 8 + it) * NTHR];
                    y[0] = yy.x; y[1] = yy.y; y[2] = yy.z; y[3] = yy.w;
                } else {
                    const int qr = 32 * ((it & 3) >> 1) + un[2 * (it & 1) + (it >> 2)];
                    const float* mr = mc + qr * MLD;
                    float m0, m1, m2, m3, m4, m5;
                    if constexpr ((ABL & 256) != 0) {
                        m0 = acc[0][nb][it]; m1 = acc[1][nb][it]; m2 = accB[0][it]; m3 = accB[1][it];
                        m4 = acc[0][nb][it + 8]; m5 = acc[1][nb][it + 8];
                    } else {
                        m0 = mr[0 * 64 * MLD]; m1 = mr[1 * 64 * MLD]; m2 = mr[2 * 64 * MLD];
                        m3 = mr[3 * 64 * MLD]; m4 = mr[4 * 64 * MLD]; m5 = mr[5 * 64 * MLD];
                    }
                    const float s1 = m1 + m2, d1 = m1 - m2, s2 = m3 + m4, d2 = m3 - m4;
                    y[0] = ((m0 + s1) + s2) * dq;
                    y[1] = fmaf(2.f, d2, d1) * dq;
                    y[2] = fmaf(4.f, s2, s1) * dq;
                    y[3] = (fmaf(8.f, d2, d1) + m5) * dq;
                    if (MODE == 2 && rep) ybuf[(nb * 8 + it) * NTHR] = make_float4(y[0], y[1], y[2], y[3]);
                }
#pragma unroll
                for (int k = 0; k < 4; ++k) {
                    float r = y[k];
                    if (p.accum) r = r + prev[it][k];
                    r = r >= 0.f ? r : r * p.slope;
                    if constexpr ((ABL & 128) == 0) o[off_t + (unsigned)(k * p.Cout)] = r;
                    fs += r; fq = fmaf(r, r, fq); fmn = fminf(fmn, r); fmx = fmaxf(fmx, r);
                }
            }
            if constexpr ((ABL & 128) != 0) { if (fs == 12345.678f) p.out[tid] = fs + fq + fmn + fmx; }
        } else if (y0 + rg < p.H) {
#pragma unroll 2
            for (int it = 0; it < 8; ++it) {
                if (z0 + it >= p.D) break;
                float* o = ob + (int64_t)it * p.H * p.W * p.Cout;
                float y[4];
                if constexpr (UNI) {
                    const float4 yy = ybuf[(nb * 8 + it) * NTHR];
                    y[0] = yy.x; y[1] = yy.y; y[2] = yy.z; y[3] = yy.w;
                } else {
                    const int qr = 32 * ((it & 3) >> 1) + row_unperm(16 * (it & 1) + 8 * (it >> 2) + rg);
                    const float* mr = mc + qr * MLD;
                    const float m0 = mr[0 * 64 * MLD], m1 = mr[1 * 64 * MLD], m2 = mr[2 * 64 * MLD];
                    const float m3 = mr[3 * 64 * MLD], m4 = mr[4 * 64 * MLD], m5 = mr[5 * 64 * MLD];
                    const float s1 = m1 + m2, d1 = m1 - m2, s2 = m3 + m4, d2 = m3 - m4;
                    y[0] = ((m0 + s1) + s2) * dq;
                    y[1] = fmaf(2.f, d2, d1) * dq;
                    y[2] = fmaf(4.f, s2, s1) * dq;
                    y[3] = (fmaf(8.f, d2, d1) + m5) * dq;
                    if (MODE == 2 && rep) ybuf[(nb * 8 + it) * NTHR] = make_float4(y[0], y[1], y[2], y[3]);
                }
#pragma unroll
                for (int k = 0; k < 4; ++k) {
                    if (x0 + k < p.W) {
                        float r = y[k];
                        if (p.accum) r = r + o[off_t + (unsigned)(k * p.Cout)];
                        r = r >= 0.f ? r : r * p.slope;
                        o[off_t + (unsigned)(k * p.Cout)] = r;
                        fs += r; fq = fmaf(r, r, fq); fmn = fminf(fmn, r); fmx = fmaxf(fmx, r);
                    }
                }
            }
        }
        if (p.rsum != nullptr) {
            double* ls = reinterpret_cast<double*>(lds + (UNI ? (size_t)0 : (size_t)NPOS * 64 * MLD * sizeof(float)));
            double* lq = ls + NRG * 32;
            float* lmn = reinterpret_cast<float*>(lq + NRG * 32);
            float* lmx = lmn + NRG * 32;
            ls[rg * 32 + col] = (double)fs; lq[rg * 32 + col] = (double)fq;
            lmn[rg * 32 + col] = fmn; lmx[rg * 32 + col] = fmx;
            __syncthreads();
            if (tid < 32) {
                double Ssum = 0.0, Q = 0.0;
                float MN = INFINITY, MX = -INFINITY;
#pragma unroll
                for (int r = 0; r < NRG; ++r) {
                    Ssum += ls[r * 32 + tid]; Q += lq[r * 32 + tid];
                    MN = fminf(MN, lmn[r * 32 + tid]); MX = fmaxf(MX, lmx[r * 32 + tid]);
                }
                const size_t o = (size_t)mt * p.Cout + nt * 64 + nb * 32 + tid;
                p.rsum[o] = Ssum; p.rsq[o] = Q; p.rmn[o] = MN; p.rmx[o] = MX;
            }
        }
    }
}

template <int NPASS>
__global__ void __launch_bounds__(NTHR, 2) conv_wino4d(const W4Params p) { conv_wino4d_body<NPASS, 0>(p); }
template <int NPASS>
__global__ void __launch_bounds__(NTHR, 2) conv_wino4d_masked(const W4Params p) { conv_wino4d_body<NPASS, 1>(p); }
template <int NPASS>
__global__ void __launch_bounds__(NTHR, 2) conv_wino4d_rest(const W4Params p) { conv_wino4d_body<NPASS, 2>(p); }
template <int NPASS>
__global__ void __launch_bounds__(NTHR, 2) conv_wino4d_uniform(const W4Params p) { conv_wino4d_body<NPASS, 3>(p); }
#ifdef BFM_W4_ABLATE
template <int ABL>
__global__ void __launch_bounds__(NTHR, 2) conv_wino4d_abl(const W4Params p) { conv_wino4d_body<3, 0, ABL>(p); }
#endif

__global__ void pack_wino4(const float* __restrict__ w, int Cin, int Cout, int wexp, int npl, uint4* __restrict__ out) {
    const int KCN = Cin / KC;
    const int nf = 2 * npl;
    const int64_t n = (int64_t)(Cout / 64) * NPOS * KCN * 9 * nf * 64;
    const double s = ldexp(1.0, wexp);
    for (int64_t i = (int64_t)blockIdx.x * blockDim.x + threadIdx.x; i < n; i += (int64_t)gridDim.x * blockDim.x) {
        const int lane = (int)(i & 63);
        int64_t r = i >> 6;
        const int f = (int)(r % nf); r /= nf;
        const int t = (int)(r % 9); r /= 9;
        const int kc = (int)(r % KCN); r /= KCN;
        const int ps = (int)(r % NPOS); r /= NPOS;
        const int ntile = (int)r;
        const int nb = f / npl, hl = f - nb * npl;
        const int co = ntile * 64 + nb * 32 + (lane & 31);
        const int ci0 = kc * KC + 8 * (lane >> 5);
        half8 v;
#pragma unroll
        for (int j = 0; j < 8; ++j) {
            const float* g = w + ((size_t)co * Cin + ci0 + j) * 27 + t * 3;
            const double g0 = g[0], g1 = g[1], g2 = g[2];
            const double u = ps == 0 ? g0 / 4.0
                           : ps == 1 ? -((g0 + g1) + g2) / 6.0
                           : ps == 2 ? -((g0 - g1) + g2) / 6.0
                           : ps == 3 ? g0 / 24.0 + g1 / 12.0 + g2 / 6.0
                           : ps == 4 ? g0 / 24.0 - g1 / 12.0 + g2 / 6.0
                                     : g2;
            const float x = (float)(u * s);
            const _Float16 hh = (_Float16)x;
            v[j] = hl == 0 ? hh : (_Float16)(x - (float)hh);
        }
        out[i] = __builtin_bit_cast(uint4, v);
    }
}

int ilog2i(int v) { int r = 0; while ((1 << r) < v) ++r; return r; }

bool choose_box4(int D, int H, int W, int npl, int& TD, int& TH, int& TW) {
    if (!bfm_wino_choose_box(D, H, W, npl, TD, TH, TW)) return false;
    if (TW % 4 || TD * TH * (TW / 4) != 64) return false;
    const int64_t npos = (int64_t)(TD + 2) * (TH + 2) * (TW / 4);
    if (npos * 4 > 3 * NTHR) return false;
    const int64_t plane = ((npos * 16 + 255) / 256) * 256 + 16;
    return 2 * NPOS * npl * plane <= 62 * 1024;
}

bool use_dma_kernel(int D, int H, int W) {
#ifdef BFM_W4_ABLATE
    if (getenv("BFM_W4_OLD")) return false;
#endif
    return D >= DB_TD && H >= DB_TH && W >= 4;
}

bool choose_box_any(int D, int H, int W, int npl, int& TD, int& TH, int& TW) {
    if (use_dma_kernel(D, H, W)) { TD = DB_TD; TH = DB_TH; TW = 4; return true; }
    return choose_box4(D, H, W, npl, TD, TH, TW);
}

}

extern "C" size_t bfm_pack_conv_weights_wino4_bytes(int Cin, int Cout, int passes) {
    if (Cin <= 0 || Cout <= 0 || Cin % KC || Cout % 64) return 0;
    const int npl = passes == 3 ? 2 : 1;
    return (size_t)(Cout / 64) * NPOS * (Cin / KC) * 9 * 2 * npl * 64 * sizeof(uint4);
}

extern "C" int bfm_pack_conv_weights_wino4(const float* w_oidhw, int Cin, int Cout, float wmax_abs_host, int passes,
                                           void* wpacked, int* wexp_host, bfm_stream_t stream) {
    if (!w_oidhw || !wpacked || !wexp_host || Cin <= 0 || Cout <= 0) return BFM_E_ARG;
    if (Cin % KC || Cout % 64 || (passes != 1 && passes != 3)) return BFM_E_SHAPE;
    int wexp = 0;
    if (wmax_abs_host > 0.f && wmax_abs_host < INFINITY) {
        int ex;
        (void)frexpf(wmax_abs_host, &ex);
        wexp = 14 - ex;
        wexp = wexp > 60 ? 60 : (wexp < -60 ? -60 : wexp);
    }
    *wexp_host = wexp;
    const int npl = passes == 3 ? 2 : 1;
    const int64_t n = (int64_t)(Cout / 64) * NPOS * (Cin / KC) * 9 * 2 * npl * 64;
    const int nb = (int)std::min<int64_t>(8192, bfm_cdiv64(n, 256));
    hipLaunchKernelGGL(pack_wino4, dim3(nb), dim3(256), 0, bfm_s(stream), w_oidhw, Cin, Cout, wexp, npl,
                       static_cast<uint4*>(wpacked));
    return bfm_launch_status();
}

extern "C" int bfm_conv3x3x3_wino4_rows(int D, int H, int W, int passes) {
    int TD, TH, TW;
    if (D <= 0 || H <= 0 || W <= 0 || !choose_box_any(D, H, W, passes == 3 ? 2 : 1, TD, TH, TW)) return 0;
    return (int)bfm_box_count(D, H, W, TD, TH, TW);
}

extern "C" int bfm_conv3x3x3_wino4_box(int D, int H, int W, int passes, int* box) {
    int TD, TH, TW;
    if (!box || D <= 0 || H <= 0 || W <= 0 || !choose_box_any(D, H, W, passes == 3 ? 2 : 1, TD, TH, TW)) return BFM_E_ARG;
    box[0] = TD; box[1] = TH; box[2] = TW;
    return BFM_OK;
}

extern "C" size_t bfm_conv3x3x3_wino4_masked_workspace(int D, int H, int W, int passes) {
    const int n = bfm_conv3x3x3_wino4_rows(D, H, W, passes);
    if (n <= 0) return 0;
    return MaskListBuf::bytes((size_t)n);
}

static int w4_launch(const WinoLaunch& a) {
    if (const int rc = bfm_wino_check(a, KC)) return rc;
    const int D = a.D, H = a.H, W = a.W, CA = a.CA, Cout = a.Cout, passes = a.passes;
    const int S = a.batch.S, affine_stride = a.batch.affine_stride;
    const int npl = passes == 3 ? 2 : 1;
    W4Params p{};
    p.A = a.A; p.CA = CA; p.D = D; p.H = H; p.W = W;
    p.scale = a.scale; p.shift = a.shift; p.bound = a.bound; p.G = a.G;
    p.wp = static_cast<const uint4*>(a.wpacked);
    p.wexp = a.wexp; p.Cout = Cout; p.slope = a.slope; p.out = a.out; p.accum = a.flags & 1;
    if (!choose_box_any(D, H, W, npl, p.TD, p.TH, p.TW)) return BFM_E_SHAPE;
    const bool dma = use_dma_kernel(D, H, W);
    if (dma && (int64_t)(DB_TD + 2) * H * W * CA >= (int64_t)1 << 30) return BFM_E_SHAPE;
    p.HT = p.TH + 2; p.QW = p.TW / 4;
    p.qw_shift = ilog2i(p.QW); p.thq_shift = ilog2i(p.TH * p.QW);
    const int nTz = bfm_cdiv(D, p.TD);
    p.nTy = bfm_cdiv(H, p.TH); p.nTx = bfm_cdiv(W, p.TW);
    p.nMt = nTz * p.nTy * p.nTx;
    if (S > 1 || affine_stride > 0) {
        if (a.mask.img || S < 1 || (affine_stride != 0 && (affine_stride < CA || (affine_stride & 3)))) return BFM_E_ARG;
        p.nMtS = p.nMt;
        p.nMt = S * p.nMtS;
        p.saff = affine_stride > 0 ? affine_stride : CA;
        p.sA = (int64_t)D * H * W * CA;
        p.sO = (int64_t)D * H * W * Cout;
    }
    p.NT = Cout / 64;
    p.KCN = CA / KC;
    p.npos_lds = (p.TD + 2) * p.HT * p.QW;
    p.plane_stride = ((p.npos_lds * 16 + 255) / 256) * 256 + 16;
    size_t smem = dma ? (size_t)2 * NPOS * npl * DB_PLANE + DB_RAW : (size_t)2 * NPOS * npl * p.plane_stride;
    const size_t epi = (size_t)NPOS * 64 * MLD * sizeof(float) + (size_t)NRG * 32 * 24;
    if (smem < epi) smem = epi;
    if (smem > (dma ? 80u : 64u) * 1024) return BFM_E_SHAPE;
    const UniformFlagBuf fb{a.uniform.flags, (size_t)p.nMt};
    if (fb.flags) {
        int bd, bh, bw;
        if (!dma || a.mask.img || S > 1 || affine_stride > 0 || !a.uniform.scratch) return BFM_E_ARG;
        if (!bfm_wino_choose_box(D, H, W, npl, bd, bh, bw) || bd != p.TD || bh != p.TH || bw != p.TW) return BFM_E_SHAPE;
        p.uni_flags = fb.flags;
        p.uni_acc = a.uniform.scratch;
    }
    if (dma) {
        static bool attr = false;
        if (const int rc = bfm_raise_lds_limit(
                attr,
                {bfm_kernel(&conv_wino4d_rest<3>), bfm_kernel(&conv_wino4d_rest<1>), bfm_kernel(&conv_wino4d<3>),
                 bfm_kernel(&conv_wino4d<1>), bfm_kernel(&conv_wino4d_masked<3>), bfm_kernel(&conv_wino4d_masked<1>)},
                80 * 1024))
            return rc;
    }
    MomentRows rows;
    if (a.moment_rows && !rows.carve(a.moment_rows, (size_t)p.nMt * Cout)) return BFM_E_ARG;
    rows.into(p);
    if ((int64_t)p.nMt * p.NT > 0x7fffffff) return BFM_E_SHAPE;
    const dim3 grid((unsigned)(p.nMt * p.NT)), block(NTHR);
    hipStream_t st = bfm_s(a.stream);
    if (a.mask.img) {
        if (!a.mask.ws) return BFM_E_ARG;
        const MaskListBuf mb{a.mask.ws, (size_t)p.nMt};
        if (const int rc = bfm_wino_mask_list(a.mask.img, D, H, W, p.TD, p.TH, p.TW, p.nTy, p.nTx, p.nMt, a.mask.ws, a.stream))
            return rc;
        p.list = mb.list(); p.list_n = mb.count();
        if (dma) bfm_launch_by_passes(passes, conv_wino4d_masked<3>, conv_wino4d_masked<1>, grid, block, smem, st, p);
        else bfm_launch_by_passes(passes, conv_wino4_masked<3>, conv_wino4_masked<1>, grid, block, smem, st, p);
        return bfm_launch_status();
    }
    if (fb.flags) {
        p.list = fb.rest_list(); p.list_n = fb.counts();
        bfm_launch_by_passes(passes, conv_wino4d_rest<3>, conv_wino4d_rest<1>, grid, block, smem, st, p);
        p.list = fb.uniform_list(); p.list_n = fb.counts() + 1;
        bfm_launch_by_passes(passes, conv_wino4d_uniform<3>, conv_wino4d_uniform<1>, grid, block, 6144, st, p);
        return bfm_launch_status();
    }
#ifdef BFM_W4_ABLATE
    if (const char* e = getenv("BFM_W4_SLEEP")) p.dbg_sleep = atoi(e);
    if (const char* e = getenv("BFM_W4_ABL")) {
        const int abl = atoi(e);
        if (dma) {
#define W4D_ATTR(N) (void)hipFuncSetAttribute(reinterpret_cast<const void*>(&conv_wino4d_abl<N>), hipFuncAttributeMaxDynamicSharedMemorySize, 80 * 1024)
            W4D_ATTR(0); W4D_ATTR(1); W4D_ATTR(2); W4D_ATTR(3); W4D_ATTR(4); W4D_ATTR(8); W4D_ATTR(12); W4D_ATTR(15); W4D_ATTR(16); W4D_ATTR(31); W4D_ATTR(64); W4D_ATTR(28); W4D_ATTR(128); W4D_ATTR(256); W4D_ATTR(384); W4D_ATTR(512);
            switch (abl) {
#define W4D_CASE(N) case N: hipLaunchKernelGGL(conv_wino4d_abl<N>, grid, dim3(NTHR), smem, st, p); return bfm_launch_status()
                W4D_CASE(0); W4D_CASE(1); W4D_CASE(2); W4D_CASE(3); W4D_CASE(4); W4D_CASE(8); W4D_CASE(12); W4D_CASE(15); W4D_CASE(16); W4D_CASE(31); W4D_CASE(64); W4D_CASE(28); W4D_CASE(128); W4D_CASE(256); W4D_CASE(384); W4D_CASE(512);
                default: return BFM_E_ARG;
            }
        }
    }
#endif
    if (dma) bfm_launch_by_passes(passes, conv_wino4d<3>, conv_wino4d<1>, grid, block, smem, st, p);
    else bfm_launch_by_passes(passes, conv_wino4<3>, conv_wino4<1>, grid, block, smem, st, p);
    return bfm_launch_status();
}

extern "C" int bfm_conv3x3x3_wino4(const float* A, int CA, int D, int H, int W, const float* scale, const float* shift,
                                   const float* bound, int G, const void* wpacked, int wexp, int Cout, float slope,
                                   int passes, int flags, float* out, void* moment_rows, bfm_stream_t stream) {
    return w4_launch({A, CA, D, H, W, scale, shift, bound, G, wpacked, wexp, Cout, slope, passes, flags, out, moment_rows, stream});
}

extern "C" int bfm_conv3x3x3_wino4_batch(const float* A, int CA, int S, int D, int H, int W, const float* scale,
                                         const float* shift, const float* bound, int G, const void* wpacked, int wexp,
                                         int Cout, float slope, int passes, int flags, float* out, void* moment_rows,
                                         int affine_stride, bfm_stream_t stream) {
    if (S < 1) return BFM_E_ARG;
    WinoLaunch a{A, CA, D, H, W, scale, shift, bound, G, wpacked, wexp, Cout, slope, passes, flags, out, moment_rows, stream};
    a.batch = {S, affine_stride > 0 ? affine_stride : CA};
    return w4_launch(a);
}

extern "C" int bfm_conv3x3x3_wino4_masked(const float* A, int CA, int D, int H, int W, const float* scale, const float* shift,
                                          const float* bound, int G, const void* wpacked, int wexp, int Cout, float slope,
                                          int passes, int flags, float* out, const float* mask_image, void* workspace,
                                          size_t workspace_bytes, bfm_stream_t stream) {
    if (!mask_image || (flags & ~1)) return BFM_E_ARG;
    if (!workspace || (reinterpret_cast<uintptr_t>(workspace) & 3) ||
        workspace_bytes < bfm_conv3x3x3_wino4_masked_workspace(D, H, W, passes))
        return BFM_E_ARG;
    WinoLaunch a{A, CA, D, H, W, scale, shift, bound, G, wpacked, wexp, Cout, slope, passes, flags, out, nullptr, stream};
    a.mask = {mask_image, workspace};
    return w4_launch(a);
}

extern "C" size_t bfm_conv3x3x3_wino4_uniform_scratch(int Cout) {
    if (Cout <= 0 || Cout % 64) return 0;
    return (size_t)27 * (Cout / 64) * 2 * 8 * NTHR * sizeof(float4);
}

extern "C" int bfm_conv3x3x3_wino4_uniform(const float* A, int CA, int D, int H, int W, const float* scale, const float* shift,
                                           const float* bound, int G, const void* wpacked, int wexp, int Cout, float slope,
                                           int passes, int flags, float* out, void* moment_rows,
                                           const unsigned char* uniform_flags, void* scratch, bfm_stream_t stream) {
    if (!uniform_flags || !scratch || (reinterpret_cast<uintptr_t>(uniform_flags) & 3) || (reinterpret_cast<uintptr_t>(scratch) & 15))
        return BFM_E_ARG;
    WinoLaunch a{A, CA, D, H, W, scale, shift, bound, G, wpacked, wexp, Cout, slope, passes, flags, out, moment_rows, stream};
    a.uniform = {uniform_flags, static_cast<float*>(scratch)};
    return w4_launch(a);
}
```

brainfm_amd/csrc/wino_shared.h:

```cpp
#pragma once
#include "conv_shared.h"

bool bfm_wino_choose_box(int D, int H, int W, int npl, int& TD, int& TH, int& TW);

static inline size_t bfm_pad4(size_t n) { return (n + 3) & ~(size_t)3; }

struct MaskListBuf {
    void* ws;
    size_t n;
    static size_t bytes(size_t n) { return bfm_pad4(n) + 4 + n * 4; }
    unsigned char* act() const { return static_cast<unsigned char*>(ws); }
    int* count() const { return reinterpret_cast<int*>(act() + bfm_pad4(n)); }
    int* list() const { return count() + 1; }
};

struct UniformFlagBuf {
    const unsigned char* flags;
    size_t n;
    static size_t bytes(size_t n) { return bfm_pad4(n) + 27 * 4 + 2 * 4 + 2 * n * 4; }
    int* first() const { return reinterpret_cast<int*>(const_cast<unsigned char*>(flags) + bfm_pad4(n)); }
    int* counts() const { return first() + 27; }
    int* rest_list() const { return counts() + 2; }
    int* uniform_list() const { return rest_list() + n; }
};

int bfm_wino_mask_list(const float* mask_img, int D, int H, int W, int TD, int TH, int TW, int nTy, int nTx, int nMt, void* ws,
                       bfm_stream_t stream);

struct WinoLaunch {
    const float* A;
    int CA, D, H, W;
    const float *scale, *shift, *bound;
    int G;
    const void* wpacked;
    int wexp, Cout;
    float slope;
    int passes, flags;
    float* out;
    void* moment_rows;
    bfm_stream_t stream;
    struct { const float* img = nullptr; void* ws = nullptr; } mask;
    struct { const unsigned char* flags = nullptr; float* scratch = nullptr; } uniform;
    struct { float* out = nullptr; void* rows = nullptr; } pool;
    struct { int S = 1, affine_stride = 0; } batch;
};

static inline int bfm_wino_check(const WinoLaunch& a, int KC) {
    if (a.flags & ~1) return BFM_E_ARG;
    if (!a.A || a.CA <= 0 || a.D <= 0 || a.H <= 0 || a.W <= 0 || !a.scale || !a.shift || !a.bound || a.G <= 0 || !a.wpacked ||
        !a.out)
        return BFM_E_ARG;
    if (a.CA % KC || a.Cout % 64 || a.Cout <= 0) return BFM_E_SHAPE;
    if (a.passes != 1 && a.passes != 3) return BFM_E_ARG;
    if ((reinterpret_cast<uintptr_t>(a.A) & 15) || (reinterpret_cast<uintptr_t>(a.scale) & 15) ||
        (reinterpret_cast<uintptr_t>(a.shift) & 15) || (reinterpret_cast<uintptr_t>(a.wpacked) & 15) ||
        (reinterpret_cast<uintptr_t>(a.out) & 15))
        return BFM_E_ARG;
    if ((int64_t)a.D * a.H * a.W * a.CA > 0x7fffffffLL) return BFM_E_SHAPE;
    return BFM_OK;
}
```

brainfm_amd/engine.py:

```python
import ctypes as C
import os
from collections import OrderedDict, namedtuple

import numpy as np
import torch

from . import _lib as L

LABELS_LEFT = [0, 1, 2, 3, 4, 7, 8, 9, 10, 14, 15, 17, 31, 34, 36, 38, 40, 42]
LABELS_FULL = [0, 11, 12, 13, 16, 31, 32, 33, 34, 35, 36, 37, 38, 39, 40, 41, 42, 43, 44, 46,
               1, 2, 3, 4, 5, 6, 7, 8, 9, 10, 14, 15, 17, 47, 49, 51, 53, 55,
               18, 19, 20, 21, 22, 23, 24, 25, 26, 27, 28, 29, 30, 48, 50, 52, 54, 56]


def features_per_level(f_maps, num_levels):
    return [f_maps * 2 ** k for k in range(num_levels)]


def nearest_index_map(n_in, n_out):
    scale = np.float32(n_in) / np.float32(n_out)
    idx = np.floor(np.arange(n_out, dtype=np.float32) * scale).astype(np.int64)
    return np.minimum(idx, n_in - 1).astype(np.int32)


def tap_row_table(lo, hi):
    maps = [nearest_index_map(lo[a], hi[a]).astype(np.int64) for a in range(3)]
    z, y, x = np.meshgrid(*[np.arange(hi[a]) for a in range(3)], indexing="ij")
    tab = np.full(tuple(hi) + (27,), -1, dtype=np.int32)
    for kd in range(3):
        for kh in range(3):
            for kw in range(3):
                zz, yy, xx = z + kd - 1, y + kh - 1, x + kw - 1
                ok = (zz >= 0) & (zz < hi[0]) & (yy >= 0) & (yy < hi[1]) & (xx >= 0) & (xx < hi[2])
                row = (maps[0][zz.clip(0, hi[0] - 1)] * lo[1] + maps[1][yy.clip(0, hi[1] - 1)]) * lo[2] \
                    + maps[2][xx.clip(0, hi[2] - 1)]
                tab[..., (kd * 3 + kh) * 3 + kw] = np.where(ok, row, -1)
    return np.ascontiguousarray(tab.reshape(-1, 27))


_TUNE_CHOICES = {}

_Variant = namedtuple("_Variant", "layout pack_bytes pack rows box dense masked_workspace masked uniform_scratch uniform",
                      defaults=(None,) * 7)
_MFMA = _Variant("mfma", "bfm_pack_conv_weights_mfma_bytes", "bfm_pack_conv_weights_mfma")
_CONV_VARIANTS = (
    _MFMA,
    _MFMA,
    _Variant("mfma16", "bfm_pack_conv_weights_mfma16_bytes", "bfm_pack_conv_weights_mfma16"),
    _Variant("wino", "bfm_pack_conv_weights_wino_bytes", "bfm_pack_conv_weights_wino", "bfm_conv3x3x3_wino_rows",
             "bfm_conv3x3x3_wino_box", "bfm_conv3x3x3_wino_ex", "bfm_conv3x3x3_wino_masked_workspace",
             "bfm_conv3x3x3_wino_masked", "bfm_conv3x3x3_wino_uniform_scratch", "bfm_conv3x3x3_wino_uniform"),
    _Variant("wino4", "bfm_pack_conv_weights_wino4_bytes", "bfm_pack_conv_weights_wino4", "bfm_conv3x3x3_wino4_rows",
             "bfm_conv3x3x3_wino4_box", "bfm_conv3x3x3_wino4", "bfm_conv3x3x3_wino4_masked_workspace",
             "bfm_conv3x3x3_wino4_masked", "bfm_conv3x3x3_wino4_uniform_scratch", "bfm_conv3x3x3_wino4_uniform"),
)
_VARIANT_OF = {v.layout: ver for ver, v in enumerate(_CONV_VARIANTS)}

TUNE_FILE = os.environ.get("BFM_CONV_TUNE_FILE") or os.path.join(os.path.dirname(os.path.abspath(__file__)),
                                                                  "conv_tune_gfx950.json")
_TUNE_TABLE = None
_ARCH = {}


def _tune_key_str(key):
    cin, cout, dims, two, acc = key[:5]
    return ",".join(str(int(v)) for v in (cin, cout) + tuple(dims) + (two, acc) + tuple(key[5:]))


def _arch_of(dev_index):
    if dev_index not in _ARCH:
        name = getattr(torch.cuda.get_device_properties(dev_index), "gcnArchName", "") or "gpu"
        _ARCH[dev_index] = name.split(":")[0]
    return _ARCH[dev_index]


def _tune_table():
    global _TUNE_TABLE
    if _TUNE_TABLE is None:
        _TUNE_TABLE = {}
        mode = os.environ.get("BFM_CONV_TUNE", "1")
        if mode not in ("0", "retune") and os.path.exists(TUNE_FILE):
            import json
            try:
                _TUNE_TABLE = json.load(open(TUNE_FILE)).get("choices", {})
            except Exception as e:
                raise L.BfmError("cannot read the conv tune table %s: %r" % (TUNE_FILE, e))
    return _TUNE_TABLE


def _tune_lookup(dev_index, passes, key):
    return _tune_table().get("%s/%s" % (_arch_of(dev_index), passes), {}).get(_tune_key_str(key))


def _tune_store(dev_index, passes, key, ver):
    sect = "%s/%s" % (_arch_of(dev_index), passes)
    _tune_table().setdefault(sect, {})[_tune_key_str(key)] = int(ver)
    if os.environ.get("BFM_CONV_TUNE_SAVE") == "1":
        import json
        disk = {}
        if os.path.exists(TUNE_FILE) and os.environ.get("BFM_CONV_TUNE", "1") != "retune":
            try:
                disk = json.load(open(TUNE_FILE)).get("choices", {})
            except Exception:
                disk = {}
        for sct, tab in _tune_table().items():
            disk.setdefault(sct, {}).update(tab)
        doc = {"about": "conv variant per layer shape (0 conv_mfma, 1 conv_mfma_ws, 2 conv_mfma16, 3 conv_wino, 4 conv_wino4); key = "
                        "cin,cout,D,H,W,two_sources,accumulate[,samples]; written by UNetEngine._autotune under "
                        "BFM_CONV_TUNE_SAVE=1 (scripts/make_tune_table.py)",
               "choices": {k: dict(sorted(v.items())) for k, v in sorted(disk.items())}}
        tmp = "%s.%d.tmp" % (TUNE_FILE, os.getpid())
        with open(tmp, "w") as f:
            json.dump(doc, f, indent=0, sort_keys=False)
        os.replace(tmp, TUNE_FILE)


TRAIN_F43 = os.environ.get("BFM_TRAIN_F43", "1") != "0"


class _Layer:
    __slots__ = ("name", "cin", "cout", "groups", "gamma", "beta", "kind", "wpacked", "wexp", "w_raw", "packs", "skip",
                 "used")

    def touch(self, layout):
        u = getattr(self, "used", None)
        if u is None:
            u = self.used = set()
        u.add(layout)


HEAD_SLOPE = 0.2


class _HeadLayer(_Layer):
    __slots__ = ("bias",)


class UNetEngine:
    prof = None
    lane = 0
    weights_epoch = 0
    pack_count = 0
    _ws_lanes = None
    _variants = None
    _f23_ids = None
    _same_box_cache = None
    _uf_cache = None
    _deep_ok = None
    _tap_cache = None
    _head_layers = None
    _unit_bound = None
    _no_heads = None
    dense_last = False
    tape = None
    grad_sink = None
    prof_reps = 1
    use_upfold = False
    upfold_min = 250
    fuse_stats = False

    def __init__(self, state_dict, in_channels=1, f_maps=64, num_levels=6, num_groups=8, unit_feat=True,
                 device="cuda", passes=3, eps=1e-5, slope=0.01):
        self.lib = L.load()
        self.device = torch.device(device)
        if self.device.type != "cuda":
            raise L.BfmError("UNetEngine needs a HIP device; the product path has no CPU fallback")
        self.fm = features_per_level(f_maps, num_levels) if isinstance(f_maps, int) else list(f_maps)
        self.in_channels = in_channels
        self.num_groups = num_groups
        self.unit_feat = bool(unit_feat)
        self.passes = int(passes)
        self.eps = float(eps)
        self.slope = float(slope)
        self._up_cache = {}
        self._ws_lanes = {}
        self._ws_retired = []
        self.lane = 0
        self._gn_tickets = {ln: torch.zeros(16, dtype=torch.int32, device=self.device) for ln in range(4)}
        self._uf_tickets = {ln: torch.zeros(1, dtype=torch.int32, device=self.device) for ln in range(4)}
        self.gn_one_launch = os.environ.get("BFM_GN_ONE_LAUNCH", "1") != "0"
        self._plan_cache = {}
        self._tuned = set()
        self.force_direct = False
        self.use_upfold = os.environ.get("BFM_UPFOLD", "1") != "0"
        self.upfold_min = int(os.environ.get("BFM_UPFOLD_MIN", "250"))
        self.fuse_stats = os.environ.get("BFM_FUSE_STATS", "1") != "0"
        self.fuse_pool = os.environ.get("BFM_FUSE_POOL", "1") != "0"
        self.stem_mc = os.environ.get("BFM_STEM_MC", "1") != "0"
        self.prof_reps = 1
        self.prof = None
        sd = self._normalise_keys(state_dict)
        self.enc = []
        for i, co in enumerate(self.fm):
            ci = in_channels if i == 0 else self.fm[i - 1]
            c1 = max(co // 2, ci)
            self.enc.append([self._make_layer(sd, "backbone.encoders.%d.basic_module.SingleConv1" % i, ci, c1),
                             self._make_layer(sd, "backbone.encoders.%d.basic_module.SingleConv2" % i, c1, co)])
        rev = list(reversed(self.fm))
        self.dec = []
        for i in range(len(rev) - 1):
            ci, co = rev[i] + rev[i + 1], rev[i + 1]
            self.dec.append([self._make_layer(sd, "backbone.decoders.%d.basic_module.SingleConv1" % i, ci, co),
                             self._make_layer(sd, "backbone.decoders.%d.basic_module.SingleConv2" % i, co, co)])
        self.sd = sd
        self.dense_last = any(k.startswith("head.layers.") for k in sd)

    @staticmethod
    def _normalise_keys(state_dict):
        out = {}
        for k, v in state_dict.items():
            for marker in ("backbone.", "head."):
                j = k.find(marker)
                if j >= 0:
                    out[k[j:]] = v
                    break
            else:
                out[k] = v
        return out

    def _dev(self, t, dtype=torch.float32):
        return torch.as_tensor(t).to(device=self.device, dtype=dtype).contiguous()

    def _make_layer(self, sd, name, cin, cout):
        ly = _Layer()
        ly.name, ly.cin, ly.cout = name, cin, cout
        ly.groups = self.num_groups if cin >= self.num_groups else 1
        ly.gamma = self._dev(sd[name + ".groupnorm.weight"])
        ly.beta = self._dev(sd[name + ".groupnorm.bias"])
        w = self._dev(sd[name + ".conv.weight"])
        if tuple(w.shape) != (cout, cin, 3, 3, 3):
            raise L.BfmError("%s.conv.weight has shape %s, expected %s" % (name, tuple(w.shape), (cout, cin, 3, 3, 3)))
        ly.w_raw = w
        ly.kind = None
        ly.wpacked = None
        ly.wexp = 0
        ly.packs = {}
        ly.skip = None
        return ly

    def _mfma_ok(self, ly, ca, cb):
        return (not self.force_direct) and ca % 16 == 0 and cb % 16 == 0 and ly.cout % 64 == 0

    def _variant(self, ver):
        if self._variants is None:
            self._variants = tuple(_Variant(v.layout, *[fn and getattr(self.lib, fn) for fn in v[1:]])
                                   for v in _CONV_VARIANTS)
        return self._variants[ver if 0 <= ver < len(self._variants) else 0]

    def _make_pack(self, ly, layout, wmax=None):
        st = L.stream_ptr()
        prev = ly.packs.get(layout)
        self.pack_count += 1
        if layout in _VARIANT_OF:
            v = self._variant(_VARIANT_OF[layout])
            ps = (self.passes,) if v.dense is not None else ()
            nbytes = v.pack_bytes(ly.cin, ly.cout, *ps)
            buf = prev[0] if prev is not None else torch.empty(nbytes, dtype=torch.uint8, device=self.device)
            wexp = C.c_int(0)
            wmax = float(ly.w_raw.abs().max().item()) if wmax is None else wmax
            L.check(v.pack(L.ptr(ly.w_raw), ly.cin, ly.cout, wmax, *ps, L.ptr(buf), C.byref(wexp), st),
                    "pack_%s %s" % (layout, ly.name))
            ly.packs[layout] = (buf, wexp.value)
        elif layout == "direct":
            buf = prev[0] if prev is not None else torch.empty(27 * ly.cin * ly.cout, dtype=torch.float32, device=self.device)
            L.check(self.lib.bfm_pack_conv_weights_direct(L.ptr(ly.w_raw), ly.cin, ly.cout, L.ptr(buf), st),
                    "pack_direct " + ly.name)
            ly.packs[layout] = (buf, 0)
        else:
            raise L.BfmError("unknown weight layout '%s'" % layout)

    def _pack(self, ly, mfma, ver=0):
        layout = self._variant(ver).layout if mfma else "direct"
        if layout not in ly.packs:
            self._make_pack(ly, layout)
        ly.touch(layout)
        ly.wpacked, ly.wexp = ly.packs[layout]
        ly.kind = "mfma" if mfma else "direct"

    def _make_upfold_pack(self, ly, ca, cb, wmax=None):
        st = L.stream_ptr()
        self.pack_count += 1
        prev = ly.packs.get("upfold")
        nbytes = self.lib.bfm_pack_conv_weights_upfold_bytes(cb, ly.cout, self.passes)
        buf = prev[0] if prev is not None else torch.empty(nbytes, dtype=torch.uint8, device=self.device)
        wexp = C.c_int(0)
        wmax = float(ly.w_raw[:, ca:].abs().max().item()) if wmax is None else wmax
        L.check(self.lib.bfm_pack_conv_weights_upfold(L.ptr(ly.w_raw), ca, cb, ly.cout, wmax, self.passes,
                                                      L.ptr(buf), C.byref(wexp), st), "pack_upfold " + ly.name)
        ly.packs["upfold"] = (buf, wexp.value)

    def repack_all(self, refresh=None):
        jobs = []
        self.weights_epoch += 1

        hidden = self._head_layers[1] if self._head_layers is not None else []
        slots = torch.zeros(4 * (len(self.enc) + len(self.dec) + len(hidden)) * 4 + 16, dtype=torch.float32,
                            device=self.device)
        nslot = [0]

        def absmax(t):
            i = nslot[0]
            nslot[0] += 1
            if t.is_contiguous():
                rows, ln, stride = 1, t.numel(), t.numel()
            else:
                rows, ln, stride = t.shape[0], t[0].numel(), t.stride(0)
                if not t[0].is_contiguous():
                    raise L.BfmError("absmax: unsupported layout")
            L.check(self.lib.bfm_absmax_f32(L.ptr(t), rows, ln, stride, C.c_void_p(slots.data_ptr() + 4 * i),
                                            L.stream_ptr()), "absmax")
            return i

        def visit(ly, wm=None):
            used = getattr(ly, "used", None) or set()
            for layout in list(ly.packs.keys()):
                if layout not in used:
                    del ly.packs[layout]
                elif layout == "dgrad_layer":
                    dg = ly.packs[layout]
                    if refresh is not None:
                        refresh(ly, dg)
                    if wm is None:
                        wm = absmax(ly.w_raw)
                    visit(dg, wm)
                elif layout == "upfold":
                    jobs.append((ly, layout, absmax(ly.w_raw[:, ly.skip.cin:])))
                elif layout == "direct":
                    jobs.append((ly, layout, None))
                else:
                    if wm is None:
                        wm = absmax(ly.w_raw)
                    jobs.append((ly, layout, wm))
            ly.used = set()
            ly.wpacked, ly.kind = None, None
            if ly.skip is not None:
                ly.skip.w_raw.copy_(ly.w_raw[:, :ly.skip.cin])
                visit(ly.skip)

# ... 297 lines not shown
        mfma = self._mfma_ok(ly, ca, cb)
        if (mfma and B is not None and self.use_upfold and tuple(dims) == tuple(2 * v for v in lo_dims)
                and lo_dims[0] * lo_dims[1] * lo_dims[2] >= self.upfold_min):
            return self._single_conv_upfold(ly, A, dims, B, lo_dims, upp, scale, shift, bound, uni_flags=uni_flags)
        cfg = None
        wsc = 0
        if mfma:
            cfg = self._plan(ly.cin, ly.cout, dims, B is not None)
            wsc = self.lib.bfm_conv3x3x3_mfma_workspace(ly.cin, ly.cout, D, H, W, cfg[5])
        ws = self._gn_stats(ly, A, ca, B, cb, dims, lo_dims, upp, scale, shift, bound, wsc)
        out = torch.empty((D, H, W, ly.cout), dtype=torch.float32, device=self.device)
        if mfma:
            def _launch(c):
                self._conv_launch(ly, A, ca, B, cb, dims, upp, scale, shift, bound, ly.groups, c, out, ws)
            cfg = self._f23_cfg(ly, self._autotune(ly, (ly.cin, ly.cout, tuple(dims), B is not None, False), _launch))
        self._pack(ly, mfma, cfg[6] if cfg is not None else 0)
        if mfma:
            if mask_img is not None and not (cfg[6] in (3, 4) and B is None and self.tape is None):
                mask_img = None
            if uni_flags is not None and not (cfg[6] in (3, 4) and B is None and mask_img is None):
                uni_flags = None
            rows = self._rows_for(ly.cin, ly.cout, dims, cfg) if mask_img is None else None
            pl = None
            if (pool and cfg[6] == 3 and B is None and mask_img is None and self.tape is None and self.fuse_pool
                    and min(dims) >= 2 and self.lib.bfm_conv3x3x3_wino_pool_ok(D, H, W, self.passes)):
                pooled = torch.empty((D // 2, H // 2, W // 2, ly.cout), dtype=torch.float32, device=self.device)
                pl = (pooled, self._rows_buf(ly.cout, 1, self.lib.bfm_conv3x3x3_wino_rows, D, H, W, self.passes))

            def _record():
                nv = D * H * W
                if mask_img is not None:
                    nv = self.masked_voxels(mask_img, dims, cfg[6])
                if uni_flags is not None:
                    nv = self.uniform_voxels(uni_flags, dims)
                lo = 0 if B is None else lo_dims[0] * lo_dims[1] * lo_dims[2]
                return (2.0 * 27 * ly.cin * ly.cout * nv, 4.0 * (nv * ca + lo * cb + nv * ly.cout + 27 * ly.cin * ly.cout),
                        self._tag(ly) + ("[masked]" if mask_img is not None else "[uniform]" if uni_flags is not None else ""),
                        ly.cin, ly.cout, dims, cfg)
            self._bracket(lambda: self._conv_launch(ly, A, ca, B, cb, dims, upp, scale, shift, bound, ly.groups, cfg, out, ws,
                                                    rows, mask_img=mask_img, uni_flags=uni_flags, pool=pl), _record)
            if rows is not None:
                out._bfm_rows = rows
            if pl is not None:
                if pl[1] is not None:
                    pl[0]._bfm_rows = pl[1]
                out._bfm_pooled = (pl[0], (D // 2, H // 2, W // 2))
        elif ca == 1 and cb == 0 and ly.cout in (32, 64) and not self.force_direct:
            rows = self._rows_buf(ly.cout, 1, self.lib.bfm_conv3x3x3_stem_rows, D, H, W)
            L.check(self.lib.bfm_conv3x3x3_stem_ex(L.ptr(A), D, H, W, L.ptr(scale), L.ptr(shift), L.ptr(bound),
                                                   L.ptr(ly.wpacked), ly.cout, self.slope, L.ptr(out),
                                                   L.ptr(rows[0]) if rows is not None else None, st),
                    "conv_stem " + ly.name)
            if rows is not None:
                out._bfm_rows = rows
        elif ca in (2, 3, 4) and cb == 0 and ly.cout in (32, 64) and not self.force_direct and self.stem_mc:
            rows = self._rows_buf(ly.cout, 1, self.lib.bfm_conv3x3x3_stem_rows, D, H, W)
            L.check(self.lib.bfm_conv3x3x3_stem_mc_ex(L.ptr(A), ca, D, H, W, L.ptr(scale), L.ptr(shift), L.ptr(bound),
                                                      L.ptr(ly.wpacked), ly.cout, self.slope, L.ptr(out),
                                                      L.ptr(rows[0]) if rows is not None else None, st),
                    "conv_stem_mc " + ly.name)
            ly.kind = "stem_mc"
            if rows is not None:
                out._bfm_rows = rows
        else:
            L.check(self.lib.bfm_conv3x3x3_direct(L.ptr(A), ca, L.ptr(B), cb, D, H, W, upp, L.ptr(scale),
                                                  L.ptr(shift), L.ptr(ly.wpacked), ly.cout, self.slope, L.ptr(out),
                                                  st), "conv_direct " + ly.name)
        self._record(ly, A, B, dims, lo_dims, scale, shift, bound, out)
        return out

    def masked_voxels(self, mask_img, dims, ver=None):
        D, H, W = dims
        if ver is None:
            ly = self.dec[-1][-1] if self.dec else self.enc[0][-1]
            key = (ly.cin, ly.cout, tuple(dims), False, False)
            ver = _TUNE_CHOICES.get((torch.cuda.current_device(), getattr(self, "passes", None), key))
            if ver is None:
                ver = _tune_lookup(torch.cuda.current_device(), getattr(self, "passes", None), key)
            if os.environ.get("BFM_CONV_VER"):
                ver = int(os.environ["BFM_CONV_VER"])
        box = (C.c_int * 3)()
        L.check(self._variant(4 if ver == 4 else 3).box(D, H, W, self.passes, box), "wino_box")
        td, th, tw = box[0], box[1], box[2]
        m = (mask_img.reshape(D, H, W) != 0)
        m = torch.nn.functional.pad(m, (0, -W % tw, 0, -H % th, 0, -D % td))
        m = m.reshape(m.shape[0] // td, td, m.shape[1] // th, th, m.shape[2] // tw, tw)
        act = m.any(dim=5, keepdim=True).any(dim=3, keepdim=True).any(dim=1, keepdim=True).expand_as(m)
        act = act.reshape(m.shape[0] * td, m.shape[2] * th, m.shape[4] * tw)[:D, :H, :W]
        n = int(act.sum().item())
        self.last_mask_fraction = n / float(D * H * W)
        return n

    def uniform_flags(self, x_cl, dims, radius, level=0):
        if not self.uniform_skip or x_cl is None or x_cl.shape[-1] != 1 or self.tape is not None:
            return None
        radius = max([radius] + [r for k, r in self.UNIFORM_RADIUS.items() if k[1] == level])
        ckey = (x_cl.data_ptr(), tuple(dims), int(level), int(radius), torch.cuda.current_stream(self.device).cuda_stream)
        if self._uf_cache is None:
            self._uf_cache = {}
        cache = self._uf_cache
        if ckey in cache:
            return cache[ckey]
        D, H, W = dims
        lv = sorted({k[1] for k in self.UNIFORM_RADIUS})
        rad = [max(r for k, r in self.UNIFORM_RADIUS.items() if k[1] == l) for l in lv]
        if level in lv and radius == rad[lv.index(level)]:
            nb = [self.lib.bfm_uniform_boxes_bytes(D >> l, H >> l, W >> l, self.passes) for l in lv]
            if min(nb) > 0:
                bufs = [torch.empty(n, dtype=torch.uint8, device=self.device) for n in nb]
                rc = self.lib.bfm_uniform_boxes_levels(L.ptr(x_cl), D, H, W, len(lv), (C.c_int * len(lv))(*lv),
                                                       (C.c_int * len(lv))(*rad), self.passes,
                                                       (C.c_void_p * len(lv))(*[b.data_ptr() for b in bufs]),
                                                       L.ptr(self._uf_ticket()), L.stream_ptr())
                if rc != -2:
                    L.check(rc, "uniform_boxes_levels")
                    for l, r, b in zip(lv, rad, bufs):
                        cache[ckey[:2] + (int(l), int(r)) + ckey[4:]] = b
                    return cache[ckey]
        n = self.lib.bfm_uniform_boxes_bytes(D >> level, H >> level, W >> level, self.passes)
        if n <= 0:
            return None
        flags = torch.empty(n, dtype=torch.uint8, device=self.device)
        rc = self.lib.bfm_uniform_boxes_level(L.ptr(x_cl), D, H, W, int(level), int(radius), self.passes, L.ptr(flags),
                                              L.stream_ptr())
        if rc == -2:
            flags = None
        else:
            L.check(rc, "uniform_boxes")
        cache[ckey] = flags
        return flags

    UNIFORM_RADIUS = {("enc", 0, 1): 2, ("dec", 0): 3}
    if os.environ.get("BFM_UNIFORM_LEVELS", "1") != "0":
        UNIFORM_RADIUS.update({("enc", 1, 0): 4, ("enc", 1, 1): 6, ("dec", 1): 8})

    def uniform_voxels(self, flags, dims):
        nb = self.lib.bfm_conv3x3x3_wino_rows(dims[0], dims[1], dims[2], self.passes)
        f = flags[:nb]
        k = int((f != 0).sum().item())
        reused = k - int(torch.unique(f[f != 0]).numel())
        self.last_uniform_fraction = k / float(nb)
        return int(round(dims[0] * dims[1] * dims[2] * (1.0 - max(reused, 0) / float(nb))))

    def _skip_layer(self, ly, ca):
        if ly.skip is None:
            sk = _Layer()
            sk.name, sk.cin, sk.cout, sk.groups = ly.name + "[skip]", ca, ly.cout, ly.groups
            sk.gamma, sk.beta = ly.gamma, ly.beta
            sk.w_raw = ly.w_raw[:, :ca].contiguous()
            sk.kind, sk.wpacked, sk.wexp, sk.packs, sk.skip = None, None, 0, {}, None
            ly.skip = sk
        return ly.skip

    def _single_conv_upfold(self, ly, A, dims, B, lo_dims, upp, scale, shift, bound, uni_flags=None):
        D, H, W = dims
        ca, cb = A.shape[-1], B.shape[-1]
        st = L.stream_ptr()
        sk = self._skip_layer(ly, ca)
        key = (ca, ly.cout, tuple(dims), False, True)
        cfg0 = self._plan(ca, ly.cout, dims, False, True)
        cfg0[7] = 1
        wsc = self.lib.bfm_conv3x3x3_mfma_workspace(ca, ly.cout, D, H, W, cfg0[5])
        wsu = self.lib.bfm_conv3x3x3_upfold_workspace(cb, lo_dims[0], lo_dims[1], lo_dims[2], ly.cout)
        ws = self._gn_stats(ly, A, ca, B, cb, dims, lo_dims, upp, scale, shift, bound, max(wsc, wsu))
        out = torch.empty((D, H, W, ly.cout), dtype=torch.float32, device=self.device)
        if "upfold" not in ly.packs:
            self._make_upfold_pack(ly, ca, cb)
        ly.touch("upfold")
        wup, wexp_up = ly.packs["upfold"]

        def _launch_skip(c):
            self._conv_launch(sk, A, ca, None, 0, dims, None, scale, shift, bound, ly.groups, c, out, ws)
        cfg = self._f23_cfg(ly, self._autotune(sk, key, _launch_skip))
        self._pack(sk, True, cfg[6])
        sc_b, sh_b = scale[ca:], shift[ca:]
        nv = D * H * W
        lo = lo_dims[0] * lo_dims[1] * lo_dims[2]

        def _launch_up():
            L.check(self.lib.bfm_conv3x3x3_upfold_ex(L.ptr(B), cb, lo_dims[0], lo_dims[1], lo_dims[2], L.ptr(sc_b),
                                                     L.ptr(sh_b), L.ptr(bound), ly.groups, L.ptr(wup), wexp_up, ly.cout,
                                                     self.passes, L.ptr(out), L.ptr(ws) if wsu else None, ws.numel(), st),
                    "conv_upfold " + ly.name)
        self._bracket(_launch_up, lambda: (2.0 * 27 * cb * ly.cout * nv, 4.0 * (lo * cb + nv * ly.cout),
                                           self._tag(ly) + "up", cb, ly.cout, dims, (0,) * 8))
        rows = self._rows_for(ca, ly.cout, dims, cfg)
        if uni_flags is not None and (cfg[6] not in (3, 4) or (cfg[6] == 4 and not self._same_boxes(dims))):
            uni_flags = None
        self._bracket(lambda: self._conv_launch(sk, A, ca, None, 0, dims, None, scale, shift, bound, ly.groups, cfg, out, ws,
                                                rows, uni_flags=uni_flags),
                      lambda: (2.0 * 27 * ca * ly.cout * (nv if uni_flags is None else self.uniform_voxels(uni_flags, dims)),
                               4.0 * (nv * ca + 2 * nv * ly.cout),
                               self._tag(ly) + ("sk[uniform]" if uni_flags is not None else "sk"), ca, ly.cout, dims, cfg))
        if rows is not None:
            out._bfm_rows = rows
        self._record(ly, A, B, dims, lo_dims, scale, shift, bound, out)
        return out

    def maxpool(self, X, dims, out=None):
        D, H, W = dims
        c = X.shape[-1]
        fused = getattr(X, "_bfm_pooled", None)
        if fused is not None and out is None and self.tape is None:
            return fused
        if out is None:
            out = torch.empty((D // 2, H // 2, W // 2, c), dtype=torch.float32, device=self.device)
        rows = self._rows_buf(c, 1, self.lib.bfm_maxpool2_rows, c, D, H, W)
        L.check(self.lib.bfm_maxpool2_ex(L.ptr(X), c, D, H, W, L.ptr(out), L.ptr(rows[0]) if rows is not None else None,
                                         L.stream_ptr()), "maxpool2")
        if rows is not None:
            out._bfm_rows = rows
        if self.tape is not None:
            self.tape.append(dict(pool_in=X, pool_dims=tuple(dims)))
        return out, (D // 2, H // 2, W // 2)

    def maxpool_batch(self, X, dims):
        S, (D, H, W), c = X.shape[0], dims, X.shape[-1]
        out = torch.empty((S, D // 2, H // 2, W // 2, c), dtype=torch.float32, device=self.device)
        if c % 4 or self.tape is not None:
            for s_ in range(S):
                self.maxpool(X[s_], dims, out=out[s_])
            return out
        rows = self._rows_buf(c, S, self.lib.bfm_maxpool2_batch_rows, c, D, H, W)
        L.check(self.lib.bfm_maxpool2_batch(L.ptr(X), c, S, D, H, W, L.ptr(out), L.ptr(rows[0]) if rows is not None else None,
                                            L.stream_ptr()), "maxpool2_batch")
        if rows is not None:
            out._bfm_rows = rows
        return out

    deep_from = int(os.environ.get("BFM_DEEP_FROM", "3"))
    deep_batch = os.environ.get("BFM_DEEP_BATCH", "1") != "0"
    DEEP_VERS = (0, 2)
    DEEP_VERS_1SRC = (0, 2, 4)
    deep_upfold = os.environ.get("BFM_DEEP_UPFOLD", "1") != "0"
    deep_upfold_min = int(os.environ.get("BFM_DEEP_UPFOLD_MIN", "100"))
    use_tap = os.environ.get("BFM_TAP", "1") != "0"
    tap_max = 64
    mask_skip = os.environ.get("BFM_MASK_SKIP", "1") != "0"
    uniform_skip = os.environ.get("BFM_UNIFORM_SKIP", "1") != "0"

    deep_vox = int(os.environ.get("BFM_DEEP_VOX", "16000"))

    def _region_ok(self, df):
        if self._deep_ok is None:
            self._deep_ok = {}
        cache = self._deep_ok
        if df not in cache:
            ndeep = len(self.enc) - 1 - df
            layers = [ly for pair in self.enc[df:] + self.dec[:ndeep] for ly in pair]
            cache[df] = all(ly.cin % 16 == 0 and ly.cout % 64 == 0 for ly in layers) and \
                self.enc[df - 1][1].cout % 16 == 0
        return cache[df]

    def has_deep_region(self):
        if not (self.deep_batch and self.tape is None and not self.force_direct and len(self.fm) > self.deep_from >= 1):
            return False
        return self._region_ok(self.deep_from)

    def region_start(self, dims):
        df = self.deep_from
        while df - 1 >= 2:
            lv = [v >> (df - 1) for v in dims]
            if min(lv) < 1 or lv[0] * lv[1] * lv[2] > self.deep_vox or not self._region_ok(df - 1):
                break
            df -= 1
        return df

    def _batch_stats(self, ly, A, ca, B, cb, S, dims, lo_dims, upp, scale, shift, bound):
        D, H, W = dims
        st = L.stream_ptr()
        ra = getattr(A, "_bfm_rows", None) if self.fuse_stats else None
        rb = getattr(B, "_bfm_rows", None) if (self.fuse_stats and B is not None) else None
        exact2 = B is None or tuple(dims) == tuple(2 * v for v in lo_dims)
        if ra is not None and ra[1] <= 128 and (B is None or (rb is not None and exact2 and rb[1] <= 128)):
            L.check(self.lib.bfm_gn_stats_rows_batch(L.ptr(ra[0]), ra[1], ca, L.ptr(rb[0]) if rb is not None else None,
                                                     rb[1] if rb is not None else 0, cb, 8.0, D * H * W, S,
                                                     L.ptr(ly.gamma), L.ptr(ly.beta), ly.groups, self.eps, L.ptr(scale),
                                                     L.ptr(shift), L.ptr(bound), st), "gn_stats_rows_batch " + ly.name)
            return
        need = self.lib.bfm_gn_stats_batch_workspace(ca, cb, S, D, H, W, upp)
        ws = self._workspace(need)
        L.check(self.lib.bfm_gn_stats_batch(L.ptr(A), ca, L.ptr(B), cb, S, D, H, W, upp, L.ptr(ly.gamma), L.ptr(ly.beta),
                                            ly.groups, self.eps, L.ptr(scale), L.ptr(shift), L.ptr(bound), L.ptr(ws),
                                            ws.numel(), st), "gn_stats_batch " + ly.name)

    def batch_conv(self, ly, A, dims, B=None, lo_dims=None, stats=None):
        S = A.shape[0]
        D, H, W = dims
        ca = A.shape[-1]
        cb = 0 if B is None else B.shape[-1]
        assert ca + cb == ly.cin, (ly.name, ca, cb, ly.cin)
        if not self._mfma_ok(ly, ca, cb):
            raise L.BfmError("%s: the batched levels need channel counts that are multiples of 16 / 64" % ly.name)
        up = self._upsample_desc(lo_dims, dims) if B is not None else None
        upp = C.byref(up) if up is not None else None
        if stats is None:
            scale = torch.empty((S, ly.cin), dtype=torch.float32, device=self.device)
            shift = torch.empty((S, ly.cin), dtype=torch.float32, device=self.device)
            bound = torch.empty((S, ly.groups), dtype=torch.float32, device=self.device)
            self._batch_stats(ly, A, ca, B, cb, S, dims, lo_dims, upp, scale, shift, bound)
        else:
            scale, shift, bound = stats
        if self.use_tap and (lo_dims[0] * lo_dims[1] * lo_dims[2] if B is not None else D * H * W) <= self.tap_max:
            return self._batch_conv_tap(ly, A, dims, B, lo_dims, scale, shift, bound)
        if (B is not None and self.use_upfold and self.deep_upfold and tuple(dims) == tuple(2 * v for v in lo_dims)
                and lo_dims[0] * lo_dims[1] * lo_dims[2] >= self.deep_upfold_min):
            return self._batch_conv_upfold(ly, A, dims, B, lo_dims, scale, shift, bound)
        key = (ly.cin, ly.cout, tuple(dims), B is not None, False, 1)
        vers = self.DEEP_VERS if B is not None else self.DEEP_VERS_1SRC
        cfg = self._batch_plan(key, vers)
        out = torch.empty((S, D, H, W, ly.cout), dtype=torch.float32, device=self.device)
        if key not in self._tuned:
            cfg = self._autotune(ly, key, lambda c: self._batch_launch(ly, c, A[0:1], B[0:1] if B is not None else None, upp, dims,
                                                                       scale[0:1], shift[0:1], bound[0:1], out[0:1]),
                                 vers=vers)
        self._pack(ly, True, cfg[6])
        rows = self._rows_for(ly.cin, ly.cout, dims, cfg, S)
        nv = D * H * W
        lo = 0 if B is None else lo_dims[0] * lo_dims[1] * lo_dims[2]
        self._bracket(lambda: self._batch_launch(ly, cfg, A, B, upp, dims, scale, shift, bound, out, rows),
                      lambda: (2.0 * 27 * ly.cin * ly.cout * nv * S,
                               4.0 * (S * (nv * ca + lo * cb + nv * ly.cout) + 27 * ly.cin * ly.cout),
                               self._tag(ly) + ("x%d" % S), ly.cin, ly.cout, dims, cfg))
        if rows is not None:
            out._bfm_rows = rows
        return out

    def _batch_plan(self, key, vers):
        if key not in self._plan_cache:
            cfg = (C.c_int * 8)()
# ... 474 lines not shown
```

include/brainfm_hip.h:

```cpp
#ifndef BRAINFM_HIP_H
#define BRAINFM_HIP_H

#include <stddef.h>
#include <stdint.h>

#ifdef __cplusplus
extern "C" {
#endif

typedef void* bfm_stream_t;

#define BFM_OK 0
#define BFM_E_ARG (-1)
#define BFM_E_SHAPE (-2)
#define BFM_E_WORKSPACE (-3)
#define BFM_E_LAUNCH (-4)

typedef struct {
    int d, h, w;
    const int32_t* mapD; const int32_t* mapH; const int32_t* mapW;
    const int32_t* repD; const int32_t* repH; const int32_t* repW;
} bfm_upsample_t;

const char* bfm_version(void);

size_t bfm_gn_stats_workspace(int CA, int CB, int D, int H, int W, const bfm_upsample_t* up);
int bfm_gn_stats(const float* A, int CA, const float* B, int CB, int D, int H, int W,
                 const bfm_upsample_t* up, const float* gamma, const float* beta, int G, float eps,
                 float* scale, float* shift, float* bound, void* workspace, size_t workspace_bytes,
                 bfm_stream_t stream);
int bfm_gn_stats_train(const float* A, int CA, const float* B, int CB, int D, int H, int W, const bfm_upsample_t* up,
                       const float* gamma, const float* beta, int G, float eps, float* scale, float* shift,
                       float* bound, float* mean_out, float* rstd_out, void* workspace, size_t workspace_bytes,
                       bfm_stream_t stream);

int bfm_pack_conv_weights_direct(const float* w_oidhw, int Cin, int Cout, float* wpacked, bfm_stream_t stream);
size_t bfm_pack_conv_weights_mfma_bytes(int Cin, int Cout);
int bfm_pack_conv_weights_mfma(const float* w_oidhw, int Cin, int Cout, float wmax_abs_host, void* wpacked,
                               int* wexp_host, bfm_stream_t stream);

size_t bfm_pack_conv_weights_mfma16_bytes(int Cin, int Cout);
int bfm_pack_conv_weights_mfma16(const float* w_oidhw, int Cin, int Cout, float wmax_abs_host, void* wpacked,
                                 int* wexp_host, bfm_stream_t stream);

int bfm_conv3x3x3_direct(const float* A, int CA, const float* B, int CB, int D, int H, int W,
                         const bfm_upsample_t* up, const float* scale, const float* shift,
                         const float* wpacked, int Cout, float slope, float* out, bfm_stream_t stream);


size_t bfm_pack_conv_weights_wino_bytes(int Cin, int Cout, int passes);
int bfm_pack_conv_weights_wino(const float* w_oidhw, int Cin, int Cout, float wmax_abs_host, int passes, void* wpacked,
                               int* wexp_host, bfm_stream_t stream);
int bfm_conv3x3x3_wino_rows(int D, int H, int W, int passes);
int bfm_conv3x3x3_wino_ex(const float* A, int CA, int D, int H, int W, const float* scale, const float* shift,
                          const float* bound, int G, const void* wpacked, int wexp, int Cout, float slope, int passes,
                          int flags, float* out, void* moment_rows , bfm_stream_t stream);

size_t bfm_uniform_boxes_bytes(int D, int H, int W, int passes);
int bfm_uniform_boxes(const float* image, int D, int H, int W, int radius, int passes, unsigned char* flags,
                      bfm_stream_t stream);
int bfm_uniform_boxes_level(const float* image, int D, int H, int W, int level, int radius, int passes, unsigned char* flags,
                            bfm_stream_t stream);
int bfm_uniform_boxes_levels(const float* image, int D, int H, int W, int nlevels, const int* levels, const int* radii,
                             int passes, unsigned char* const* flags, int* ticket, bfm_stream_t stream);
size_t bfm_conv3x3x3_wino_uniform_scratch(int Cout);
int bfm_conv3x3x3_wino_uniform(const float* A, int CA, int D, int H, int W, const float* scale, const float* shift,
                               const float* bound, int G, const void* wpacked, int wexp, int Cout, float slope, int passes,
                               int flags, float* out, void* moment_rows, const unsigned char* uniform_flags, void* scratch,
                               bfm_stream_t stream);
int bfm_conv3x3x3_wino_pool_ok(int D, int H, int W, int passes);
int bfm_conv3x3x3_wino_pool(const float* A, int CA, int D, int H, int W, const float* scale, const float* shift,
                            const float* bound, int G, const void* wpacked, int wexp, int Cout, float slope, int passes,
                            int flags, float* out, void* moment_rows, float* pooled, void* pooled_rows ,
                            bfm_stream_t stream);
int bfm_conv3x3x3_wino_uniform_pool(const float* A, int CA, int D, int H, int W, const float* scale, const float* shift,
                                    const float* bound, int G, const void* wpacked, int wexp, int Cout, float slope,
                                    int passes, int flags, float* out, void* moment_rows,
                                    const unsigned char* uniform_flags, void* scratch, float* pooled,
                                    void* pooled_rows , bfm_stream_t stream);
int bfm_conv3x3x3_wino_box(int D, int H, int W, int passes, int* box );
size_t bfm_conv3x3x3_wino_masked_workspace(int D, int H, int W, int passes);
int bfm_conv3x3x3_wino_masked(const float* A, int CA, int D, int H, int W, const float* scale, const float* shift,
                              const float* bound, int G, const void* wpacked, int wexp, int Cout, float slope, int passes,
                              int flags, float* out, const float* mask_image, void* workspace, size_t workspace_bytes,
                              bfm_stream_t stream);

size_t bfm_moment_rows_bytes(int nrows, int C);
int bfm_conv3x3x3_mfma_rows(int Cin, int Cout, int D, int H, int W, const int* cfg);
int bfm_conv3x3x3_mfma_ex(const float* A, int CA, const float* B, int CB, int D, int H, int W,
                          const bfm_upsample_t* up, const float* scale, const float* shift, const float* bound,
                          int G, const void* wpacked, int wexp, int Cout, float slope, int passes, const int* cfg,
                          float* out, void* workspace, size_t workspace_bytes, void* moment_rows ,
                          bfm_stream_t stream);
size_t bfm_conv3x3x3_mfma_batch_workspace(int Cin, int Cout, int S, int D, int H, int W, int splitk);
int bfm_conv3x3x3_mfma_batch(const float* A, int CA, const float* B, int CB, int S, int D, int H, int W,
                             const bfm_upsample_t* up, const float* scale, const float* shift, const float* bound, int G,
                             const void* wpacked, int wexp, int Cout, float slope, int passes, const int* cfg, float* out,
                             void* workspace, size_t workspace_bytes, void* moment_rows, int affine_stride,
                             bfm_stream_t stream);
size_t bfm_gn_stats_batch_workspace(int CA, int CB, int S, int D, int H, int W, const bfm_upsample_t* up);
int bfm_gn_stats_batch(const float* A, int CA, const float* B, int CB, int S, int D, int H, int W,
                       const bfm_upsample_t* up, const float* gamma, const float* beta, int G, float eps, float* scale,
                       float* shift, float* bound, void* workspace, size_t workspace_bytes, bfm_stream_t stream);
int bfm_gn_stats_rows_batch(const void* rowsA, int nrowsA_per_sample, int CA, const void* rowsB, int nrowsB_per_sample,
                            int CB, double weightB, int64_t nvox, int S, const float* gamma, const float* beta, int G,
                            float eps, float* scale, float* shift, float* bound, bfm_stream_t stream);

int bfm_maxpool2_rows(int C, int D, int H, int W);
int bfm_maxpool2_ex(const float* in, int C, int D, int H, int W, float* out, void* moment_rows ,
                    bfm_stream_t stream);
int bfm_maxpool2_batch_rows(int C, int D, int H, int W);
int bfm_maxpool2_batch(const float* in, int C, int S, int D, int H, int W, float* out, void* moment_rows ,
                       bfm_stream_t stream);
int bfm_conv3x3x3_stem_rows(int D, int H, int W);
int bfm_conv3x3x3_stem_ex(const float* A, int D, int H, int W, const float* scale, const float* shift,
                          const float* bound, const float* wpacked_direct, int Cout, float slope, float* out,
                          void* moment_rows , bfm_stream_t stream);
int bfm_conv3x3x3_stem_mc_ex(const float* A, int Cin, int D, int H, int W, const float* scale, const float* shift,
                             const float* bound, const float* wpacked_direct, int Cout, float slope, float* out,
                             void* moment_rows , bfm_stream_t stream);
size_t bfm_gn_stats_rows_workspace(int nrowsA, int CA, int nrowsB, int CB);
#define BFM_GN_TICKETS 16
int bfm_gn_stats_rows(const void* rowsA, int nrowsA, int CA, const void* rowsB, int nrowsB, int CB, double weightB,
                      int64_t nvox, const float* gamma, const float* beta, int G, float eps, float* scale,
                      float* shift, float* bound, void* workspace, size_t workspace_bytes, void* ticket,
                      bfm_stream_t stream);
int bfm_gn_stats_rows_train(const void* rowsA, int nrowsA, int CA, const void* rowsB, int nrowsB, int CB, double weightB,
                            int64_t nvox, const float* gamma, const float* beta, int G, float eps, float* scale,
                            float* shift, float* bound, float* mean_out, float* rstd_out, void* workspace,
                            size_t workspace_bytes, void* ticket, bfm_stream_t stream);

int bfm_gn_stats_rows_sliced(const void* rowsA, int totalA, int firstA, int nrowsA, int CA, const void* rowsB, int totalB,
                             int firstB, int nrowsB, int CB, double weightB, int64_t nvox, const float* gamma,
                             const float* beta, int G, float eps, float* scale, float* shift, float* bound,
                             void* workspace, size_t workspace_bytes, void* ticket, bfm_stream_t stream);

size_t bfm_pack_conv_weights_wino4_bytes(int Cin, int Cout, int passes);
int bfm_pack_conv_weights_wino4(const float* w_oidhw, int Cin, int Cout, float wmax_abs_host, int passes, void* wpacked,
                                int* wexp_host, bfm_stream_t stream);
int bfm_conv3x3x3_wino4_rows(int D, int H, int W, int passes);
int bfm_conv3x3x3_wino4_box(int D, int H, int W, int passes, int* box );
int bfm_conv3x3x3_wino4(const float* A, int CA, int D, int H, int W, const float* scale, const float* shift,
                        const float* bound, int G, const void* wpacked, int wexp, int Cout, float slope, int passes,
                        int flags, float* out, void* moment_rows , bfm_stream_t stream);
int bfm_conv3x3x3_wino4_batch(const float* A, int CA, int S, int D, int H, int W, const float* scale, const float* shift,
                              const float* bound, int G, const void* wpacked, int wexp, int Cout, float slope, int passes,
                              int flags, float* out, void* moment_rows, int affine_stride, bfm_stream_t stream);
size_t bfm_conv3x3x3_wino4_masked_workspace(int D, int H, int W, int passes);
size_t bfm_conv3x3x3_wino4_uniform_scratch(int Cout);
int bfm_conv3x3x3_wino4_uniform(const float* A, int CA, int D, int H, int W, const float* scale, const float* shift,
                                const float* bound, int G, const void* wpacked, int wexp, int Cout, float slope, int passes,
                                int flags, float* out, void* moment_rows, const unsigned char* uniform_flags, void* scratch,
                                bfm_stream_t stream);
int bfm_conv3x3x3_wino4_masked(const float* A, int CA, int D, int H, int W, const float* scale, const float* shift,
                               const float* bound, int G, const void* wpacked, int wexp, int Cout, float slope, int passes,
                               int flags, float* out, const float* mask_image, void* workspace, size_t workspace_bytes,
                               bfm_stream_t stream);

size_t bfm_conv3x3x3_mfma_workspace(int Cin, int Cout, int D, int H, int W, int splitk);
int bfm_conv3x3x3_mfma_plan(int Cin, int Cout, int D, int H, int W, int* cfg_out );

size_t bfm_pack_conv_weights_upfold_bytes(int CB, int Cout, int passes);
int bfm_pack_conv_weights_upfold(const float* w_oidhw , int CA, int CB, int Cout,
                                 float wmax_abs_host, int passes, void* wpacked, int* wexp_host, bfm_stream_t stream);
int bfm_conv3x3x3_upfold(const float* B, int CB, int d, int h, int w, const float* scale_b, const float* shift_b,
                         const float* bound, int G, const void* wpacked, int wexp, int Cout, int passes, float* out,
                         bfm_stream_t stream);
size_t bfm_conv3x3x3_upfold_workspace(int CB, int d, int h, int w, int Cout);
int bfm_conv3x3x3_upfold_ex(const float* B, int CB, int d, int h, int w, const float* scale_b, const float* shift_b,
                            const float* bound, int G, const void* wpacked, int wexp, int Cout, int passes, float* out,
                            void* workspace, size_t workspace_bytes, bfm_stream_t stream);
size_t bfm_conv3x3x3_upfold_batch_workspace(int CB, int S, int d, int h, int w, int Cout);
int bfm_conv3x3x3_upfold_batch(const float* B, int CB, int S, int d, int h, int w, const float* scale_b,
                               const float* shift_b, const float* bound, int G, const void* wpacked, int wexp, int Cout,
                               int passes, float* out, void* workspace, size_t workspace_bytes, int affine_stride,
                               bfm_stream_t stream);

size_t bfm_conv3x3x3_tap_batch_workspace(int Cin, int Cout, int S, int n_lo);
int bfm_conv3x3x3_tap_batch(const float* X, int Cin, int S, int n_lo, const float* scale, const float* shift,
                            const float* bound, int G, const void* wpacked, int wexp, int Cout, int kc_first, int kc_pack,
                            int passes, void* workspace, size_t workspace_bytes, int affine_stride, bfm_stream_t stream);
int bfm_tap_sum_rows(int n_hi, int Cout);
int bfm_tap_sum_batch(const void* workspace, int Cin, int Cout, int S, int n_lo, const int* table ,
                      int n_hi, float slope, int activation, int accumulate, float* out, void* moment_rows ,
                      bfm_stream_t stream);

int bfm_conv3x3x3_mfma(const float* A, int CA, const float* B, int CB, int D, int H, int W,
                       const bfm_upsample_t* up, const float* scale, const float* shift, const float* bound,
                       int G, const void* wpacked, int wexp, int Cout, float slope, int passes,
                       const int* cfg , float* out, void* workspace,
                       size_t workspace_bytes, bfm_stream_t stream);

int bfm_maxpool2(const float* in, int C, int D, int H, int W, float* out, bfm_stream_t stream);

enum {
    BFM_ROLE_PLAIN = 0,
    BFM_ROLE_CT = 1,
    BFM_ROLE_BIAS_LOG = 2,
    BFM_ROLE_SEG = 3,
    BFM_ROLE_DIST = 4,
    BFM_ROLE_SR = 5,
    BFM_ROLE_PATHOL = 6
};
typedef struct {
    int n_out;
    int c_feat;
    const float* head_w;
    const float* head_b;
    const int32_t* roles;
    const int32_t* out_slot;
    int seg_first, n_seg;
    const int32_t* seg_lut;
    int n_dist;
    int dist_first;
    float max_dist;
    int unit_feat;
    int slot_high_res;
    int slot_fake_cortical;
    int n_maps;
    float head_wmax;
    int skip_zero_input;
} bfm_tail_desc_t;

int bfm_tail_heads(const float* feat, const float* input , int64_t nvox,
                   const bfm_tail_desc_t* desc, float* feat_norm ,
                   float* const* maps ,
                   float* seg_prob , int64_t* label ,
                   float* raw_out ,
                   bfm_stream_t stream);
int bfm_tail_heads_rows(const float* feat, const float* input , int64_t nvox,
                        const bfm_tail_desc_t* desc, float* feat_norm , float* maps_rows, int64_t row_stride,
                        float* seg_prob , int64_t* label , int flags, bfm_stream_t stream);

int bfm_stitch_accumulate(const float* tile, const int64_t* tile_label, const float* tile_input,
                          int td, int th, int tw, float* full, int D, int H, int W,
                          int z0, int y0, int x0, bfm_stream_t stream);
int bfm_stitch_accumulate_multi(const float* maps, int64_t map_stride, const int32_t* sel, int K,
                                const int64_t* tile_label, const float* tile_input, int td, int th, int tw, float* full,
                                int D, int H, int W, int z0, int y0, int x0, bfm_stream_t stream);
int bfm_tile_count_add(float* cnt, int D, int H, int W, int z0, int z1, int y0, int y1, int x0, int x1,
                       bfm_stream_t stream);
int bfm_pack_tile_multi(const float* maps, int64_t map_stride, const int32_t* sel, int K, const int64_t* tile_label,
                        const float* tile_input, int64_t n, float* out, bfm_stream_t stream);
int bfm_divide_by_count_multi(float* full, const float* cnt, int64_t vol, int K, bfm_stream_t stream);
int bfm_stitch_gather_multi(const int64_t* tiles, int T, int K, float* full, int D, int H, int W, bfm_stream_t stream);

int bfm_tile_mask_blocks(int64_t tile_voxels);
int bfm_tile_mask_index(const float* volume, int D, int H, int W, const int64_t* tiles, int T, int total_blocks,
                        int32_t* pos, int32_t* nnz, int32_t* block_ws, bfm_stream_t stream);
int bfm_pack_tile_compact(const float* maps, int64_t map_stride, const int32_t* sel, int K, const int64_t* tile_label,
                          const float* tile_input, int64_t n, const int32_t* pos, int64_t row_stride, float* out,
                          bfm_stream_t stream);
int bfm_stitch_gather_compact(const int64_t* tiles, int T, int K, const float* volume, float* full, int D, int H, int W,
                              bfm_stream_t stream);

enum {
    BFM_EW_EXP = 0, BFM_EW_AFFINE = 1 , BFM_EW_CLAMP = 2 , BFM_EW_CLAMP_MIN = 3,
    BFM_EW_GAMMA = 4 , BFM_EW_SIGMOID = 5,
    BFM_EW_DIV = 6 , BFM_EW_NONZERO = 7 , BFM_EW_SUB_DIV = 8 ,
    BFM_EW_GE = 9 ,
    BFM_EW_NAN_TO_NUM = 10
};
enum {
    BFM_EW_ADD = 0, BFM_EW_MUL = 1, BFM_EW_MUL_EXP = 2 ,
    BFM_EW_AXPY_CLAMP0 = 3 , BFM_EW_AXPY = 4, BFM_EW_DIV2 = 5,
    BFM_EW_ZERO_WHERE_ZERO = 6
};
int bfm_ew_unary(int op, const float* in, int64_t in_stride, float* out, int64_t out_stride, int64_t n,
                 float a, float b, bfm_stream_t stream);
int bfm_ew_binary(int op, const float* x, int64_t x_stride, const float* y, int64_t y_stride ,
                  float* out, int64_t out_stride, int64_t n, float a, bfm_stream_t stream);
int bfm_absmax_f32(const float* x, int64_t rows, int64_t len, int64_t row_stride, float* out_zeroed, bfm_stream_t stream);
int bfm_softmax_cl(const float* x, int64_t x_row_stride, int C, float* y, int64_t y_row_stride, int64_t n,
                   bfm_stream_t stream);
int bfm_argmax_lut_cl(const float* p, int64_t row_stride, int C, const int32_t* lut, int64_t* out, int64_t n,
                      bfm_stream_t stream);
int bfm_fake_cortical(const float* dist, int64_t row_stride, int n_dist, float* out, int64_t n,
                      bfm_stream_t stream);
int bfm_mask_concat2(const float* x, const float* p, int64_t n, float* out, bfm_stream_t stream);
int bfm_condition_input(const float* x, const float* p, int mode, int D, int H, int W, float* out, float* masked,
                        float* flipped, bfm_stream_t stream);
int bfm_twostage_train_input(const float* x, const float* raw0, int64_t col_offset, int64_t voxel_stride, const float* t,
                             int64_t n, float* out , float* p_out , float* masked_out ,
                             bfm_stream_t stream);

int bfm_interp3d_linear(const float* X, int nx, int ny, int nz, int C, const float* II, const float* JJ,
                        const float* KK, int64_t n, float default_value, float* out, bfm_stream_t stream);
int bfm_interp3d_nearest(const void* X, int nx, int ny, int nz, int C, const float* II, const float* JJ,
                         const float* KK, int64_t n, void* out, bfm_stream_t stream);
int bfm_deformed_atlas(const float* mask, const float* regx, const float* regy, const float* regz, const float* atlas,
                       int nx, int ny, int nz, const float* A_host, int64_t n, float* out, bfm_stream_t stream);
int bfm_deformed_atlas_tile(const float* tile_in, const float* regx, const float* regy, const float* regz,
                            const float* atlas, int nx, int ny, int nz, const float* A_host, int64_t n, float* out,
                            bfm_stream_t stream);
typedef struct { const int32_t* f; const int32_t* c; const float* wf; const float* wc; } bfm_zoom_axis_t;
int bfm_zoom_linear(const float* X, int nx, int ny, int nz, int C, const bfm_zoom_axis_t* axes , int ox, int oy,
                    int oz, float* out, bfm_stream_t stream);
int bfm_conv1d_axis(const float* in, int nx, int ny, int nz, int axis, const float* kern, int klen, float* out,
                    bfm_stream_t stream);
int bfm_grid_push3d_linear(const float* inp, int Bi, int C, int ix, int iy, int iz, const float* grid, int Bg, int nx,
                           int ny, int nz, const int* bound, int extrapolate, float* out_zeroed, bfm_stream_t stream);
int bfm_grid_grad3d_linear(const float* inp, int Bi, int C, int nx, int ny, int nz, const float* grid, int Bg, int ox,
                           int oy, int oz, const int* bound, int extrapolate, float* out, bfm_stream_t stream);

int bfm_crop3d(const float* vol, int D, int H, int W, int z0, int y0, int x0, int d, int h, int w, float* out,
               bfm_stream_t stream);

int bfm_permute_flip3d(const float* in, int nx, int ny, int nz, const int* perm ,
                       const int* flip , float* out, bfm_stream_t stream);
int bfm_bbox_nonzero(const float* in, int nx, int ny, int nz, float tol, int32_t* box ,
                     bfm_stream_t stream);
int bfm_mean_lastdim(const float* in, int64_t n, int c, float* out, bfm_stream_t stream);

int bfm_bspline3_prefilter_axis(float* vol, int nx, int ny, int nz, int axis, int bound, float pole, float gain,
                                const float* init_w, float pole_last, float init_scale, float final_scale,
                                bfm_stream_t stream);
int bfm_bspline3_resample_axis(const float* in, int nx, int ny, int nz, int axis, const float* coord, int n_out,
                               int bound, float* out, bfm_stream_t stream);

int bfm_grid_pull3d_linear(const float* inp, int Bi, int C, int nx, int ny, int nz, const float* grid, int Bg, int ox,
                           int oy, int oz, const int* bound, int extrapolate, float* out, bfm_stream_t stream);
size_t bfm_deform_grid_workspace(int sx, int sy, int sz);
int bfm_deform_grid(const float* F, int sx, int sy, int sz, const float* A_host , const float* c2_host ,
                    const int* shp_host , float* xx, float* yy, float* zz, float* minmax ,
// ... 260 lines not shown
```

Measured before the change: 210.9 million voxels/s.

## Fuse skip-conv join, activation and moment stats into upfold epilogue for last decoder levels

For the last two decoder levels, the skip-path Winograd conv now writes raw pre-activation output (and a per-class replica for uniform tiles) without applying the activation. The upfold conv then adds that skip result in its epilogue, applies the leaky activation, and writes the final output. It also reduces per-row sum, sum-of-squares, min and max via DPP and LDS for the following GroupNorm. This removes the separate accumulate/read-modify-write pass and the separate stats pass, at the cost of more LDS, register pressure and coordinate bookkeeping in the upfold kernel.

```diff
diff --git a/brainfm_amd/_lib.py b/brainfm_amd/_lib.py
--- a/brainfm_amd/_lib.py
+++ b/brainfm_amd/_lib.py
@@ -98,6 +98,8 @@
     "bfm_conv3x3x3_upfold": (_I, [_P, _I, _I, _I, _I, _P, _P, _P, _I, _P, _I, _I, _I, _P, _P]),
     "bfm_conv3x3x3_upfold_workspace": (_Z, [_I, _I, _I, _I, _I]),
     "bfm_conv3x3x3_upfold_ex": (_I, [_P, _I, _I, _I, _I, _P, _P, _P, _I, _P, _I, _I, _I, _P, _P, _Z, _P]),
+    "bfm_conv3x3x3_upfold_join_rows": (_I, [_I, _I, _I, _I, _I, _I, _I]),
+    "bfm_conv3x3x3_upfold_join": (_I, [_P, _I, _I, _I, _I, _P, _P, _P, _I, _P, _I, _I, _I, _F, _P, _P, _P, _P, _I, _P]),
     "bfm_conv3x3x3_upfold_batch_workspace": (_Z, [_I, _I, _I, _I, _I, _I]),
     "bfm_conv3x3x3_upfold_batch": (_I, [_P, _I, _I, _I, _I, _I, _P, _P, _P, _I, _P, _I, _I, _I, _P, _P, _Z, _I, _P]),
     "bfm_conv3x3x3_tap_batch_workspace": (_Z, [_I, _I, _I, _I]),
@@ -130,6 +132,7 @@
     "bfm_conv3x3x3_wino4_masked_workspace": (_Z, [_I, _I, _I, _I]),
     "bfm_conv3x3x3_wino4_uniform_scratch": (_Z, [_I]),
     "bfm_conv3x3x3_wino4_uniform": (_I, [_P, _I, _I, _I, _I, _P, _P, _P, _I, _P, _I, _I, _F, _I, _I, _P, _P, _P, _P, _P]),
+    "bfm_conv3x3x3_wino4_rest_raw": (_I, [_P, _I, _I, _I, _I, _P, _P, _P, _I, _P, _I, _I, _I, _P, _P, _P, _P]),
     "bfm_conv3x3x3_wino4": (_I, [_P, _I, _I, _I, _I, _P, _P, _P, _I, _P, _I, _I, _F, _I, _I, _P, _P, _P]),
     "bfm_conv3x3x3_wino4_batch": (_I, [_P, _I, _I, _I, _I, _I, _P, _P, _P, _I, _P, _I, _I, _F, _I, _I, _P, _P, _I, _P]),
     "bfm_conv3x3x3_wino4_masked": (_I, [_P, _I, _I, _I, _I, _P, _P, _P, _I, _P, _I, _I, _F, _I, _I, _P, _P, _P, _Z, _P]),
diff --git a/brainfm_amd/csrc/conv3d_upfold.hip b/brainfm_amd/csrc/conv3d_upfold.hip
--- a/brainfm_amd/csrc/conv3d_upfold.hip
+++ b/brainfm_amd/csrc/conv3d_upfold.hip
@@ -1,4 +1,4 @@
-#include "conv_shared.h"
+#include "wino_shared.h"
 #include <type_traits>
 
 namespace {
@@ -30,7 +30,34 @@
     int64_t slab_stride;
     int64_t sB, sO;
     int dbg_sleep;
+    float slope;
+    const unsigned char* jflags;
+    const float* jrep;
+    int jnTy, jnTx;
+    int coord_lds, fold_lds;
+    double *rsum, *rsq;
+    float *rmn, *rmx;
 };
+
+template <int CTRL>
+__device__ __forceinline__ float dpp_f(float v) {
+    return __builtin_bit_cast(float, __builtin_amdgcn_mov_dpp(__builtin_bit_cast(int, v), CTRL, 0xf, 0xf, false));
+}
+__device__ __forceinline__ float oct_sum(float v) {
+    v = v + dpp_f<0xB1>(v);
+    v = v + dpp_f<0x4E>(v);
+    return v + dpp_f<0x141>(v);
+}
+__device__ __forceinline__ float oct_min(float v) {
+    v = fminf(v, dpp_f<0xB1>(v));
+    v = fminf(v, dpp_f<0x4E>(v));
+    return fminf(v, dpp_f<0x141>(v));
+}
+__device__ __forceinline__ float oct_max(float v) {
+    v = fmaxf(v, dpp_f<0xB1>(v));
+    v = fmaxf(v, dpp_f<0x4E>(v));
+    return fmaxf(v, dpp_f<0x141>(v));
+}
 
 __device__ __forceinline__ void box_coords(const UpParams& p, int q, int& bd, int& bh, int& bw) {
     bd = q / p.BHW;
@@ -39,7 +66,7 @@
     bw = rem - bh * p.BW;
 }
 
-template <int NPASS, int ABL = 0, int NW = 8>
+template <int NPASS, int ABL = 0, int NW = 8, bool JOIN = false>
 __device__ __forceinline__ void conv_upfold_body(const UpParams& p) {
     constexpr int NTHRV = NW * 64;
     constexpr int NPL = (NPASS == 3) ? 2 : 1;
@@ -93,12 +120,20 @@
     const float dq = ldexpf(1.0f, -(aexp + p.wexp));
 
     int a_off[4];
+    unsigned jf = 0;
 #pragma unroll
     for (int mb = 0; mb < 4; ++mb) {
         int bd, bh, bw;
         const int q = mb * 32 + row_perm(l32);
         box_coords(p, q < p.BVOX ? q : 0, bd, bh, bw);
         a_off[mb] = (khalf * NPL) * p.plane_stride + (((bd + pz) * p.HT + (bh + py)) * p.WT + (bw + px)) * 16;
+        if constexpr (JOIN) {
+            if (p.jflags != nullptr) {
+                const int Z = min(2 * (z0 + bd) + pz, 2 * p.d - 1), Y = min(2 * (y0 + bh) + py, 2 * p.h - 1);
+                const int X = min(2 * (x0 + bw) + px, 2 * p.w - 1);
+                jf |= (unsigned)p.jflags[((Z >> 3) * p.jnTy + (Y >> 3)) * p.jnTx + (X >> 2)] << (8 * mb);
+            }
+        }
     }
 
     int* const rowoff = reinterpret_cast<int*>(lds + p.rowoff_lds);
@@ -107,6 +142,7 @@
         box_coords(p, tid < p.BVOX ? tid : 0, bd, bh, bw);
         const bool ok = tid < p.BVOX && z0 + bd < p.d && y0 + bh < p.h && x0 + bw < p.w;
         rowoff[tid] = ok ? (((2 * bd) * (2 * p.h) + 2 * bh) * (2 * p.w) + 2 * bw) * p.Cout : -1;
+        if constexpr (JOIN) reinterpret_cast<int*>(lds + p.coord_lds)[tid] = bd | (bh << 8) | (bw << 16);
     }
 
     constexpr int MAX_IT = 2048 / NTHRV;
@@ -261,6 +297,88 @@
         return;
     }
     const int H2 = 2 * p.h, W2 = 2 * p.w;
+    if constexpr (JOIN) {
+        const int* const rowc = reinterpret_cast<const int*>(lds + p.coord_lds);
+        float* const ob = p.out + (((int64_t)(2 * z0 + pz) * H2 + (2 * y0 + py)) * W2 + (2 * x0 + px)) * p.Cout + nt * 64 + khalf * 4;
+        float* o[4];
+        const float* sk[4];
+#pragma unroll
+        for (int mb = 0; mb < 4; ++mb) {
+            const int q = mb * 32 + row_perm(l32);
+            const int rel = rowoff[q];
+            o[mb] = nullptr;
+            sk[mb] = ob;
+            if (rel < 0) continue;
+            o[mb] = ob + (unsigned)rel;
+            sk[mb] = o[mb];
+            const int f = (int)((jf >> (8 * mb)) & 255u);
+            if (f) {
+                const int c = rowc[q];
+                const int Z = 2 * (z0 + (c & 255)) + pz, Y = 2 * (y0 + ((c >> 8) & 255)) + py, X = 2 * (x0 + (c >> 16)) + px;
+                sk[mb] = p.jrep + (size_t)((((f - 1) * 8 + (Z & 7)) * 8 + (Y & 7)) * 4 + (X & 3)) * p.Cout + nt * 64 + khalf * 4;
+            }
+        }
+        float4* const fold = reinterpret_cast<float4*>(lds + p.fold_lds);
+        const int wv = tid >> 6;
+        constexpr int JOIN_AHEAD = 3;
+        float4 s4q[8][4];
+        auto load_skip = [&](int ng) __attribute__((always_inline)) {
+#pragma unroll
+            for (int mb = 0; mb < 4; ++mb)
+                s4q[ng][mb] = *reinterpret_cast<const float4*>(sk[mb] + (ng >> 2) * 32 + (ng & 3) * 8);
+        };
+#pragma unroll
+        for (int ng = 0; ng <= JOIN_AHEAD; ++ng) load_skip(ng);
+        __builtin_amdgcn_sched_barrier(0);
+#pragma unroll
+        for (int nb = 0; nb < 2; ++nb)
+#pragma unroll
+            for (int g = 0; g < 4; ++g) {
+                float4 s4[4];
+#pragma unroll
+                for (int mb = 0; mb < 4; ++mb) s4[mb] = s4q[nb * 4 + g][mb];
+                if (nb * 4 + g + JOIN_AHEAD + 1 < 8) load_skip(nb * 4 + g + JOIN_AHEAD + 1);
+                float fs[4] = {0.f, 0.f, 0.f, 0.f}, fq[4] = {0.f, 0.f, 0.f, 0.f};
+                float fmn[4] = {INFINITY, INFINITY, INFINITY, INFINITY}, fmx[4] = {-INFINITY, -INFINITY, -INFINITY, -INFINITY};
+#pragma unroll
+                for (int mb = 0; mb < 4; ++mb) {
+                    const bool ok = o[mb] != nullptr;
+                    const float y[4] = {s4[mb].x, s4[mb].y, s4[mb].z, s4[mb].w};
+                    float r[4];
+#pragma unroll
+                    for (int j = 0; j < 4; ++j) {
+                        float v = acc[mb][nb][4 * g + j] * dq + y[j];
+                        v = v >= 0.f ? v : v * p.slope;
+                        r[j] = v;
+                        const float vs = ok ? v : 0.f, vm = ok ? v : __builtin_nanf("");
+                        fs[j] += vs; fq[j] = fmaf(vs, vs, fq[j]); fmn[j] = fminf(fmn[j], vm); fmx[j] = fmaxf(fmx[j], vm);
+                    }
+                    if (ok) *reinterpret_cast<float4*>(o[mb] + nb * 32 + g * 8) = make_float4(r[0], r[1], r[2], r[3]);
+                }
+                if (p.rsum != nullptr) {
+#pragma unroll
+                    for (int j = 0; j < 4; ++j) {
+                        const float4 part = make_float4(oct_sum(fs[j]), oct_sum(fq[j]), oct_min(fmn[j]), oct_max(fmx[j]));
+                        if ((lane & 7) == 0) fold[(wv * 4 + ((lane >> 3) & 3)) * 64 + nb * 32 + g * 8 + khalf * 4 + j] = part;
+                    }
+                }
+            }
+        if (p.rsum != nullptr) {
+            __syncthreads();
+            if (tid < 64) {
+                double Ssum = 0.0, Q = 0.0;
+                float MN = INFINITY, MX = -INFINITY;
+                for (int k = 0; k < 32; ++k) {
+                    const float4 v = fold[k * 64 + tid];
+                    Ssum += (double)v.x; Q += (double)v.y;
+                    MN = fminf(MN, v.z); MX = fmaxf(MX, v.w);
+                }
+                const size_t ro = (size_t)mt * p.Cout + nt * 64 + tid;
+                p.rsum[ro] = Ssum; p.rsq[ro] = Q; p.rmn[ro] = MN; p.rmx[ro] = MX;
+            }
+        }
+        return;
+    }
     float* const obase = p.slab ? p.slab + ((int64_t)smp * gridDim.y + blockIdx.y) * p.slab_stride : p.out + smp * p.sO;
     float* const ob = obase + (((int64_t)(2 * z0 + pz) * H2 + (2 * y0 + py)) * W2 + (2 * x0 + px)) * p.Cout + nt * 64 + khalf * 4;
 #pragma unroll
@@ -282,6 +400,8 @@
 __global__ void __launch_bounds__(NTHR, 1) conv_upfold(const UpParams p) { conv_upfold_body<NPASS, 0>(p); }
 template <int NPASS>
 __global__ void __launch_bounds__(NTHR / 2, 2) conv_upfold_h(const UpParams p) { conv_upfold_body<NPASS, 0, 4>(p); }
+template <int NPASS>
+__global__ void __launch_bounds__(NTHR, 1) conv_upfold_join(const UpParams p) { conv_upfold_body<NPASS, 0, 8, true>(p); }
 #ifdef BFM_UP_ABLATE
 template <int ABL>
 __global__ void __launch_bounds__(NTHR, 1) conv_upfold_abl(const UpParams p) { conv_upfold_body<3, ABL>(p); }
@@ -454,9 +574,47 @@
     return nsplit > 1 ? (size_t)nsplit * 8 * d * h * w * Cout * sizeof(float) : 0;
 }
 
+namespace {
+struct UpJoin {
+    float slope;
+    const unsigned char* flags;
+    const float* rep;
+    void* rows;
+    bool any_shape;
+};
+int upfold_join_rows(int CB, int d, int h, int w, int Cout, int passes, bool any_shape) {
+    if (CB <= 0 || d <= 0 || h <= 0 || w <= 0 || Cout <= 0 || CB % KC || Cout % 64 || (passes != 1 && passes != 3)) return 0;
+    if (d > 0x3fffffff || h > 0x3fffffff || w > 0x3fffffff) return 0;
+    int nsplit, per, BD, BH, BW, td, th, tw;
+    upfold_split(CB, d, h, w, Cout, nsplit, per);
+    if (nsplit > 1 && !any_shape) return 0;
+    choose_box(d, h, w, BD, BH, BW);
+    const int64_t nMt = bfm_box_count(d, h, w, BD, BH, BW);
+    if ((nMt * (Cout / 64) <= 128 && !any_shape) || nMt > 0x7fffffff) return 0;
+    if (2 * d < 8 || 2 * h < 8 || 2 * w < 4) return 0;
+    if (!bfm_wino_choose_box(2 * d, 2 * h, 2 * w, passes == 3 ? 2 : 1, td, th, tw) || td != 8 || th != 8 || tw != 4) return 0;
+    return (int)nMt;
+}
+}
+
 static int upfold_launch(const float* B, int CB, int S, int d, int h, int w, const float* scale_b, const float* shift_b,
                          const float* bound, int G, const void* wpacked, int wexp, int Cout, int passes, float* out,
-                         void* workspace, size_t workspace_bytes, bool strict, int affine_stride, bfm_stream_t stream);
+                         void* workspace, size_t workspace_bytes, bool strict, int affine_stride, bfm_stream_t stream,
+                         const UpJoin* join = nullptr);
+
+extern "C" int bfm_conv3x3x3_upfold_join_rows(int CB, int d, int h, int w, int Cout, int passes, int any_shape) {
+    return upfold_join_rows(CB, d, h, w, Cout, passes, any_shape != 0);
+}
+
+extern "C" int bfm_conv3x3x3_upfold_join(const float* B, int CB, int d, int h, int w, const float* scale_b,
+                                         const float* shift_b, const float* bound, int G, const void* wpacked, int wexp,
+                                         int Cout, int passes, float slope, float* out, const unsigned char* uniform_flags,
+                                         const void* rep_scratch, void* moment_rows, int any_shape, bfm_stream_t stream) {
+    if (!rep_scratch || (reinterpret_cast<uintptr_t>(rep_scratch) & 15)) return BFM_E_ARG;
+    const UpJoin j{slope, uniform_flags, static_cast<const float*>(rep_scratch), moment_rows, any_shape != 0};
+    return upfold_launch(B, CB, 1, d, h, w, scale_b, shift_b, bound, G, wpacked, wexp, Cout, passes, out, nullptr, 0, false, 0,
+                         stream, &j);
+}
 
 extern "C" int bfm_conv3x3x3_upfold_ex(const float* B, int CB, int d, int h, int w, const float* scale_b,
                                        const float* shift_b, const float* bound, int G, const void* wpacked, int wexp,
@@ -482,7 +640,8 @@
 
 static int upfold_launch(const float* B, int CB, int S, int d, int h, int w, const float* scale_b, const float* shift_b,
                          const float* bound, int G, const void* wpacked, int wexp, int Cout, int passes, float* out,
-                         void* workspace, size_t workspace_bytes, bool strict, int affine_stride, bfm_stream_t stream) {
+                         void* workspace, size_t workspace_bytes, bool strict, int affine_stride, bfm_stream_t stream,
+                         const UpJoin* join) {
     if (!B || CB <= 0 || d <= 0 || h <= 0 || w <= 0 || !scale_b || !shift_b || !bound || G <= 0 || !wpacked || !out)
         return BFM_E_ARG;
     if (CB % KC || Cout % 64 || Cout <= 0) return BFM_E_SHAPE;
@@ -527,6 +686,24 @@
             per = p.KCB;
         }
     }
+    if (join) {
+        if (upfold_join_rows(CB, d, h, w, Cout, passes, join->any_shape) != p.nMt) return BFM_E_SHAPE;
+        MomentRows rows;
+        if (join->rows && !rows.carve(join->rows, (size_t)p.nMt * Cout)) return BFM_E_ARG;
+        rows.into(p);
+        p.slope = join->slope; p.jflags = join->flags; p.jrep = join->rep;
+        p.jnTy = bfm_cdiv(2 * h, 8); p.jnTx = bfm_cdiv(2 * w, 4);
+        p.coord_lds = p.rowoff_lds + 128 * (int)sizeof(int);
+        p.fold_lds = p.coord_lds + 128 * (int)sizeof(int);
+        const size_t smem_j = (size_t)p.fold_lds + 8 * 4 * 64 * sizeof(float4);
+        static bool attr_j = false;
+        if (const int rc = bfm_raise_lds_limit(attr_j, {bfm_kernel(&conv_upfold_join<3>), bfm_kernel(&conv_upfold_join<1>)}, 96 * 1024))
+            return rc;
+        p.kc_per_split = p.KCB;
+        bfm_launch_by_passes(passes, conv_upfold_join<3>, conv_upfold_join<1>, dim3((unsigned)(p.nMt * p.NT)), dim3(NTHR), smem_j,
+                             bfm_s(stream), p);
+        return bfm_launch_status();
+    }
     p.kc_per_split = per;
     p.slab = nsplit > 1 ? static_cast<float*>(workspace) : nullptr;
     p.slab_stride = nout;
diff --git a/brainfm_amd/csrc/conv3d_wino4.hip b/brainfm_amd/csrc/conv3d_wino4.hip
--- a/brainfm_amd/csrc/conv3d_wino4.hip
+++ b/brainfm_amd/csrc/conv3d_wino4.hip
@@ -436,9 +436,10 @@
 template <int NPASS, int MODE, int ABL = 0>
 __device__ __forceinline__ void conv_wino4d_body(const W4Params& pin) {
     W4Params p = pin;
-    constexpr bool LIST = MODE != 0;
+    constexpr bool LIST = MODE != 0 && MODE != 5;
     constexpr bool UNI = MODE == 3;
-    constexpr bool BY_FLAG = MODE == 2 || MODE == 3;
+    constexpr bool BY_FLAG = MODE == 2 || MODE == 3 || MODE == 4;
+    constexpr bool RAW = MODE == 4 || MODE == 5;
     constexpr int NPL = (NPASS == 3) ? 2 : 1;
     constexpr int NF = 2 * NPL;
     constexpr int NWF = 3 * NPL;
@@ -486,8 +487,9 @@
     const int z0 = tz * DB_TD, y0 = ty * DB_TH, x0 = tx * 4;
     int cls = 0;
     if constexpr (BY_FLAG) cls = __builtin_amdgcn_readfirstlane((int)p.uni_flags[mt]);
-    const bool rep = MODE == 2 && cls != 0;
-    float4* const ybuf = BY_FLAG && cls ? reinterpret_cast<float4*>(p.uni_acc) + ((size_t)(cls - 1) * p.NT + nt) * (2 * 8 * NTHR) + tid
+    const bool rep = (MODE == 2 || MODE == 4) && cls != 0;
+    float* const rbuf = MODE == 4 && cls ? p.uni_acc + (size_t)(cls - 1) * (DB_TD * DB_TH * 4) * p.Cout + nt * 64 : nullptr;
+    float4* const ybuf = BY_FLAG && !RAW && cls ? reinterpret_cast<float4*>(p.uni_acc) + ((size_t)(cls - 1) * p.NT + nt) * (2 * 8 * NTHR) + tid
                                         : nullptr;
 
     float bmax = 0.f;
@@ -758,7 +760,7 @@
         const float* mc = m + col;
         if (interior) {
             float prev[8][4];
-            if (p.accum) {
+            if (!RAW && p.accum) {
 #pragma unroll
                 for (int it = 0; it < 8; ++it) {
                     const float* o = ob + (int64_t)it * p.H * p.W * p.Cout;
@@ -795,6 +797,11 @@
 #pragma unroll
                 for (int k = 0; k < 4; ++k) {
                     float r = y[k];
+                    if constexpr (RAW) {
+                        o[off_t + (unsigned)(k * p.Cout)] = r;
+                        if (MODE == 4 && rep) rbuf[((it * DB_TH + rg) * 4 + k) * p.Cout + nb * 32 + col] = r;
+                        continue;
+                    }
                     if (p.accum) r = r + prev[it][k];
                     r = r >= 0.f ? r : r * p.slope;
                     if constexpr ((ABL & 128) == 0) o[off_t + (unsigned)(k * p.Cout)] = r;
@@ -827,6 +834,11 @@
                 for (int k = 0; k < 4; ++k) {
                     if (x0 + k < p.W) {
                         float r = y[k];
+                        if constexpr (RAW) {
+                            o[off_t + (unsigned)(k * p.Cout)] = r;
+                            if (MODE == 4 && rep) rbuf[((it * DB_TH + rg) * 4 + k) * p.Cout + nb * 32 + col] = r;
+                            continue;
+                        }
                         if (p.accum) r = r + o[off_t + (unsigned)(k * p.Cout)];
                         r = r >= 0.f ? r : r * p.slope;
                         o[off_t + (unsigned)(k * p.Cout)] = r;
@@ -835,7 +847,7 @@
                 }
             }
         }
-        if (p.rsum != nullptr) {
+        if (!RAW && p.rsum != nullptr) {
             double* ls = reinterpret_cast<double*>(lds + (UNI ? (size_t)0 : (size_t)NPOS * 64 * MLD * sizeof(float)));
             double* lq = ls + NRG * 32;
             float* lmn = reinterpret_cast<float*>(lq + NRG * 32);
@@ -866,6 +878,10 @@
 __global__ void __launch_bounds__(NTHR, 2) conv_wino4d_rest(const W4Params p) { conv_wino4d_body<NPASS, 2>(p); }
 template <int NPASS>
 __global__ void __launch_bounds__(NTHR, 2) conv_wino4d_uniform(const W4Params p) { conv_wino4d_body<NPASS, 3>(p); }
+template <int NPASS>
+__global__ void __launch_bounds__(NTHR, 2) conv_wino4d_rest_raw(const W4Params p) { conv_wino4d_body<NPASS, 4>(p); }
+template <int NPASS>
+__global__ void __launch_bounds__(NTHR, 2) conv_wino4d_raw(const W4Params p) { conv_wino4d_body<NPASS, 5>(p); }
 #ifdef BFM_W4_ABLATE
 template <int ABL>
 __global__ void __launch_bounds__(NTHR, 2) conv_wino4d_abl(const W4Params p) { conv_wino4d_body<3, 0, ABL>(p); }
@@ -1011,7 +1027,13 @@
     if (smem < epi) smem = epi;
     if (smem > (dma ? 80u : 64u) * 1024) return BFM_E_SHAPE;
     const UniformFlagBuf fb{a.uniform.flags, (size_t)p.nMt};
-    if (fb.flags) {
+    if (a.uniform.raw) {
+        int bd, bh, bw;
+        if (a.mask.img || S > 1 || affine_stride > 0 || !a.uniform.scratch || a.moment_rows || p.accum) return BFM_E_ARG;
+        if (!dma || !bfm_wino_choose_box(D, H, W, npl, bd, bh, bw) || bd != p.TD || bh != p.TH || bw != p.TW) return BFM_E_SHAPE;
+        p.uni_flags = fb.flags;
+        p.uni_acc = a.uniform.scratch;
+    } else if (fb.flags) {
         int bd, bh, bw;
         if (!dma || a.mask.img || S > 1 || affine_stride > 0 || !a.uniform.scratch) return BFM_E_ARG;
         if (!bfm_wino_choose_box(D, H, W, npl, bd, bh, bw) || bd != p.TD || bh != p.TH || bw != p.TW) return BFM_E_SHAPE;
@@ -1022,7 +1044,9 @@
         static bool attr = false;
         if (const int rc = bfm_raise_lds_limit(
                 attr,
-                {bfm_kernel(&conv_wino4d_rest<3>), bfm_kernel(&conv_wino4d_rest<1>), bfm_kernel(&conv_wino4d<3>),
+                {bfm_kernel(&conv_wino4d_rest_raw<3>), bfm_kernel(&conv_wino4d_rest_raw<1>), bfm_kernel(&conv_wino4d_raw<3>),
+                 bfm_kernel(&conv_wino4d_raw<1>),
+                 bfm_kernel(&conv_wino4d_rest<3>), bfm_kernel(&conv_wino4d_rest<1>), bfm_kernel(&conv_wino4d<3>),
                  bfm_kernel(&conv_wino4d<1>), bfm_kernel(&conv_wino4d_masked<3>), bfm_kernel(&conv_wino4d_masked<1>)},
                 80 * 1024))
             return rc;
@@ -1043,6 +1067,13 @@
         else bfm_launch_by_passes(passes, conv_wino4_masked<3>, conv_wino4_masked<1>, grid, block, smem, st, p);
         return bfm_launch_status();
     }
+    if (a.uniform.raw) {
+        if (fb.flags) {
+            p.list = fb.rest_list(); p.list_n = fb.counts();
+            bfm_launch_by_passes(passes, conv_wino4d_rest_raw<3>, conv_wino4d_rest_raw<1>, grid, block, smem, st, p);
+        } else bfm_launch_by_passes(passes, conv_wino4d_raw<3>, conv_wino4d_raw<1>, grid, block, smem, st, p);
+        return bfm_launch_status();
+    }
     if (fb.flags) {
         p.list = fb.rest_list(); p.list_n = fb.counts();
         bfm_launch_by_passes(passes, conv_wino4d_rest<3>, conv_wino4d_rest<1>, grid, block, smem, st, p);
@@ -1114,3 +1145,13 @@
     a.uniform = {uniform_flags, static_cast<float*>(scratch)};
     return w4_launch(a);
 }
+
+extern "C" int bfm_conv3x3x3_wino4_rest_raw(const float* A, int CA, int D, int H, int W, const float* scale, const float* shift,
+                                            const float* bound, int G, const void* wpacked, int wexp, int Cout, int passes,
+                                            float* out, const unsigned char* uniform_flags, void* scratch, bfm_stream_t stream) {
+    if (!scratch || (reinterpret_cast<uintptr_t>(uniform_flags) & 3) || (reinterpret_cast<uintptr_t>(scratch) & 15))
+        return BFM_E_ARG;
+    WinoLaunch a{A, CA, D, H, W, scale, shift, bound, G, wpacked, wexp, Cout, 0.f, passes, 0, out, nullptr, stream};
+    a.uniform = {uniform_flags, static_cast<float*>(scratch), true};
+    return w4_launch(a);
+}
diff --git a/brainfm_amd/csrc/wino_shared.h b/brainfm_amd/csrc/wino_shared.h
--- a/brainfm_amd/csrc/wino_shared.h
+++ b/brainfm_amd/csrc/wino_shared.h
@@ -40,7 +40,7 @@
     void* moment_rows;
     bfm_stream_t stream;
     struct { const float* img = nullptr; void* ws = nullptr; } mask;
-    struct { const unsigned char* flags = nullptr; float* scratch = nullptr; } uniform;
+    struct { const unsigned char* flags = nullptr; float* scratch = nullptr; bool raw = false; } uniform;
     struct { float* out = nullptr; void* rows = nullptr; } pool;
     struct { int S = 1, affine_stride = 0; } batch;
 };
diff --git a/brainfm_amd/engine.py b/brainfm_amd/engine.py
--- a/brainfm_amd/engine.py
+++ b/brainfm_amd/engine.py
@@ -145,6 +145,7 @@
     _variants = None
     _f23_ids = None
     _same_box_cache = None
+    _join_ids = None
     _uf_cache = None
     _deep_ok = None
     _tap_cache = None
@@ -156,6 +157,7 @@
     grad_sink = None
     prof_reps = 1
     use_upfold = False
+    upfold_join = False
     upfold_min = 250
     fuse_stats = False
 
@@ -184,6 +186,7 @@
         self.force_direct = False
         self.use_upfold = os.environ.get("BFM_UPFOLD", "1") != "0"
         self.upfold_min = int(os.environ.get("BFM_UPFOLD_MIN", "250"))
+        self.upfold_join = os.environ.get("BFM_UPFOLD_JOIN", "1") != "0"
         self.fuse_stats = os.environ.get("BFM_FUSE_STATS", "1") != "0"
         self.fuse_pool = os.environ.get("BFM_FUSE_POOL", "1") != "0"
         self.stem_mc = os.environ.get("BFM_STEM_MC", "1") != "0"
@@ -787,6 +790,13 @@
             ly.skip = sk
         return ly.skip
 
+    def _join_ok(self, ly, cfg, dims, cb, lo_dims, wsu):
+        if self._join_ids is None:
+            self._join_ids = {id(d[0]) for d in self.dec[-2:]}
+        return (self.upfold_join and id(ly) in self._join_ids and cfg[6] == 4 and wsu == 0 and self._same_boxes(dims)
+                and min(dims[0], dims[1]) >= 8 and dims[2] >= 4
+                and self.lib.bfm_conv3x3x3_upfold_join_rows(cb, lo_dims[0], lo_dims[1], lo_dims[2], ly.cout, self.passes, 0) > 0)
+
     def _single_conv_upfold(self, ly, A, dims, B, lo_dims, upp, scale, shift, bound, uni_flags=None):
         D, H, W = dims
         ca, cb = A.shape[-1], B.shape[-1]
@@ -811,6 +821,34 @@
         sc_b, sh_b = scale[ca:], shift[ca:]
         nv = D * H * W
         lo = lo_dims[0] * lo_dims[1] * lo_dims[2]
+        if self._join_ok(ly, cfg, dims, cb, lo_dims, wsu):
+            rows = self._rows_buf(ly.cout, 1, self.lib.bfm_conv3x3x3_upfold_join_rows, cb, lo_dims[0], lo_dims[1], lo_dims[2],
+                                  ly.cout, self.passes, 0)
+            scratch = torch.empty(self.lib.bfm_conv3x3x3_wino4_uniform_scratch(ly.cout), dtype=torch.uint8, device=self.device)
+
+            def _launch_raw():
+                L.check(self.lib.bfm_conv3x3x3_wino4_rest_raw(L.ptr(A), ca, D, H, W, L.ptr(scale), L.ptr(shift), L.ptr(bound),
+                                                              ly.groups, L.ptr(sk.wpacked), sk.wexp, ly.cout, self.passes,
+                                                              L.ptr(out), L.ptr(uni_flags) if uni_flags is not None else None,
+                                                              L.ptr(scratch), st), "conv_wino4(rest_raw) " + ly.name)
+
+            def _launch_join():
+                L.check(self.lib.bfm_conv3x3x3_upfold_join(L.ptr(B), cb, lo_dims[0], lo_dims[1], lo_dims[2], L.ptr(sc_b),
+                                                           L.ptr(sh_b), L.ptr(bound), ly.groups, L.ptr(wup), wexp_up, ly.cout,
+                                                           self.passes, self.slope, L.ptr(out),
+                                                           L.ptr(uni_flags) if uni_flags is not None else None, L.ptr(scratch),
+                                                           L.ptr(rows[0]) if rows is not None else None, 0, st),
+                        "conv_upfold(join) " + ly.name)
+            self._bracket(_launch_raw,
+                          lambda: (2.0 * 27 * ca * ly.cout * (nv if uni_flags is None else self.uniform_voxels(uni_flags, dims)),
+                                   4.0 * (nv * ca + nv * ly.cout),
+                                   self._tag(ly) + ("sk[uniform]" if uni_flags is not None else "sk"), ca, ly.cout, dims, cfg))
+            self._bracket(_launch_join, lambda: (2.0 * 27 * cb * ly.cout * nv, 4.0 * (lo * cb + 2 * nv * ly.cout),
+                                                 self._tag(ly) + "up", cb, ly.cout, dims, (0,) * 8))
+            if rows is not None:
+                out._bfm_rows = rows
+            self._record(ly, A, B, dims, lo_dims, scale, shift, bound, out)
+            return out
 
         def _launch_up():
             L.check(self.lib.bfm_conv3x3x3_upfold_ex(L.ptr(B), cb, lo_dims[0], lo_dims[1], lo_dims[2], L.ptr(sc_b),
diff --git a/include/brainfm_hip.h b/include/brainfm_hip.h
--- a/include/brainfm_hip.h
+++ b/include/brainfm_hip.h
@@ -152,6 +152,9 @@
                                 const float* bound, int G, const void* wpacked, int wexp, int Cout, float slope, int passes,
                                 int flags, float* out, void* moment_rows, const unsigned char* uniform_flags, void* scratch,
                                 bfm_stream_t stream);
+int bfm_conv3x3x3_wino4_rest_raw(const float* A, int CA, int D, int H, int W, const float* scale, const float* shift,
+                                 const float* bound, int G, const void* wpacked, int wexp, int Cout, int passes, float* out,
+                                 const unsigned char* uniform_flags, void* scratch, bfm_stream_t stream);
 int bfm_conv3x3x3_wino4_masked(const float* A, int CA, int D, int H, int W, const float* scale, const float* shift,
                                const float* bound, int G, const void* wpacked, int wexp, int Cout, float slope, int passes,
                                int flags, float* out, const float* mask_image, void* workspace, size_t workspace_bytes,
@@ -170,6 +173,11 @@
 int bfm_conv3x3x3_upfold_ex(const float* B, int CB, int d, int h, int w, const float* scale_b, const float* shift_b,
                             const float* bound, int G, const void* wpacked, int wexp, int Cout, int passes, float* out,
                             void* workspace, size_t workspace_bytes, bfm_stream_t stream);
+int bfm_conv3x3x3_upfold_join_rows(int CB, int d, int h, int w, int Cout, int passes, int any_shape);
+int bfm_conv3x3x3_upfold_join(const float* B, int CB, int d, int h, int w, const float* scale_b, const float* shift_b,
+                              const float* bound, int G, const void* wpacked, int wexp, int Cout, int passes, float slope,
+                              float* out, const unsigned char* uniform_flags, const void* rep_scratch, void* moment_rows,
+                              int any_shape, bfm_stream_t stream);
 size_t bfm_conv3x3x3_upfold_batch_workspace(int CB, int S, int d, int h, int w, int Cout);
 int bfm_conv3x3x3_upfold_batch(const float* B, int CB, int S, int d, int h, int w, const float* scale_b,
                                const float* shift_b, const float* bound, int G, const void* wpacked, int wexp, int Cout,
```

Result: no change. 212.5 million voxels/s, median of 6 (+0.8%).
